# archibate/ptina

Measured on AMD Instinct MI355X. Metric: Msamples/sec (pixels x spp / s), 512x512x32spp cornell-monkey (978 tri), higher is better.
Workload: dtype f32; 1 GPU; s978: 978-tri synthetic cornell + bumpy sphere, 512x512, 32 spp, unidirectional MIS path tracer, depth<=5; step = 32 x render() + get_image() (resolve + D2H), exams/benchmark.py:29-36; spp=32, mode=fast, parallelism=single GPU

## Files before the change

### ptina_amd/csrc/miptina.cpp

```cpp

#include "miptina_ctx.h"
#include <chrono>

static int g_hwq = 0;
static bool g_hwq_late = false;
__attribute__((constructor)) static void mpt_want_hw_queues() {
    if (!getenv("GPU_MAX_HW_QUEUES")) {
        setenv("GPU_MAX_HW_QUEUES", "12", 0);
        const char *pre = getenv("LD_PRELOAD");
        if ((pre && strstr(pre, "rocprof")) || getenv("ROCP_TOOL_LIBRARIES")) {
            g_hwq_late = true;
            fprintf(stderr, "libmiptina: GPU_MAX_HW_QUEUES=12 requested after a preloaded profiler tool may have initialised HIP: "
                            "streams may fold onto the default 4 hardware queues (results unchanged; export the variable "
                            "before starting the profiler)\n");
        }
    }
    const char *v = getenv("GPU_MAX_HW_QUEUES");
    g_hwq = v ? atoi(v) : 0;
}

static thread_local std::string g_err;

int fail(const char *fmt, ...) {
    char buf[1024];
    va_list ap;
    va_start(ap, fmt);
    vsnprintf(buf, sizeof buf, fmt, ap);
    va_end(ap);
    g_err = buf;
    return 1;
}


extern "C" const char *mpt_last_error(void) { return g_err.c_str(); }
extern "C" int mpt_version(void) { return 100; }

extern "C" int mpt_device_count(void) {
    int n = 0;
    if (hipGetDeviceCount(&n) != hipSuccess) return 0;
    return n;
}

int use_ro(mpt_ctx *c) {
    if (!c) return fail("null context");
    HIP_TRY(hipSetDevice(c->device));
    return 0;
}

int use(mpt_ctx *c) {
    if (use_ro(c)) return 1;
    if (mpt_flush(c)) return 1;
    c->main_dirty = true;
    c->spec_valid = false;
    return 0;
}


static void default_light(mpt_ctx *c) {
    MptLight L{};
    L.color_size = { 32.f, 32.f, 32.f, 0.5f };
    L.pos_type = { 1.f, 2.f, 3.f, 0.f };
    int t = MPT_LIGHT_POINT;
    memcpy(&L.pos_type.w, &t, 4);
    c->h_lights.assign(1, L);
}

static int upload_lights(mpt_ctx *c) {
    if (!c->h_lights.empty())
        HIP_TRY(hipMemcpyAsync(c->lights, c->h_lights.data(), c->h_lights.size() * sizeof(MptLight),
                               hipMemcpyHostToDevice, c->stream));
    HIP_TRY(hipStreamSynchronize(c->stream));
    return 0;
}

static int make_render_streams(mpt_ctx *c) {
    for (int k = 0; k < MPT_MAX_PIPE; k++)
        if (!c->rstream[k]) HIP_TRY(hipStreamCreateWithFlags(&c->rstream[k], hipStreamNonBlocking));
    return 0;
}

extern "C" mpt_ctx *mpt_create(const mpt_caps *caps, int device) {
    int ndev = 0;
    hipError_t e = hipGetDeviceCount(&ndev);
    if (e != hipSuccess || ndev == 0) {
        fail("no HIP device available (%s): the MI355X path has no CPU fallback",
             e == hipSuccess ? "device count 0" : hipGetErrorString(e));
        return nullptr;
    }
    if (device < 0 || device >= ndev) { fail("device %d out of range (%d devices)", device, ndev); return nullptr; }
    mpt_ctx *c = new mpt_ctx();
    c->device = device;
    mpt_caps d = { 1 << 21, 1 << 22, 1 << 6, 1 << 6, 1 << 6, 1 << 21, 3 };
    c->caps = caps ? *caps : d;
    if (c->caps.max_lights > MPT_MAX_LIGHTS) c->caps.max_lights = MPT_MAX_LIGHTS;
    if (c->caps.max_filmpasses < 3) c->caps.max_filmpasses = 3;
    auto bail = [&](const char *what) -> mpt_ctx * {
        std::string m = g_err;
        fail("mpt_create: %s: %s", what, m.c_str());
        delete c;
        return nullptr;
    };
    if (hipSetDevice(device) != hipSuccess) return bail("hipSetDevice");
    if (hipStreamCreateWithFlags(&c->stream, hipStreamNonBlocking) != hipSuccess) return bail("stream");
    if (dev_alloc(&c->mats, (size_t)c->caps.max_materials + 1)) return bail("materials");
    if (dev_alloc(&c->images, c->caps.max_textures)) return bail("images");
    if (dev_alloc(&c->lights, MPT_MAX_LIGHTS)) return bail("lights");
    if (dev_alloc(&c->d_counters, MPT_COUNTER_WORDS)) return bail("counters");
    if (dev_alloc(&c->d_scratch, 2)) return bail("scratch");
    if (dev_alloc(&c->d_work, MPT_QUEUE_WORDS)) return bail("work counters");
    for (int k = 0; k < MPT_MAX_PIPE; k++) {
        if (hipEventCreateWithFlags(&c->ev_sobol2[k], hipEventDisableTiming) != hipSuccess) return bail("event");
        if (hipEventCreateWithFlags(&c->ev_render[k], hipEventDisableTiming) != hipSuccess) return bail("event");
        if (hipEventCreateWithFlags(&c->ev_free[k], hipEventDisableTiming) != hipSuccess) return bail("event");
        if (dev_alloc(&c->d_work2[k], MPT_QUEUE_WORDS)) return bail("work counters");
        hipMemsetAsync(c->d_work2[k], 0, MPT_QUEUE_WORDS * sizeof(unsigned int), c->stream);
    }
    if (hipStreamCreateWithFlags(&c->aux, hipStreamNonBlocking) != hipSuccess) return bail("aux stream");
    if (hipEventCreateWithFlags(&c->ev_main, hipEventDisableTiming) != hipSuccess) return bail("event");
    if (hipEventCreateWithFlags(&c->ev_film, hipEventDisableTiming) != hipSuccess) return bail("event");
    {
        hipDeviceProp_t prop;
        if (hipGetDeviceProperties(&prop, device) == hipSuccess) {
            if (prop.multiProcessorCount > 0) c->num_cus = prop.multiProcessorCount;
            c->clock_khz = prop.clockRate;
        }
    }
    if (make_render_streams(c)) return bail("render streams");
    {
        void *dp = nullptr;
        if (hipHostMalloc((void **)&c->h_watchdog, sizeof(unsigned int), hipHostMallocMapped) != hipSuccess ||
            hipHostGetDevicePointer(&dp, c->h_watchdog, 0) != hipSuccess) return bail("pinned watchdog flag");
        *c->h_watchdog = 0;
        c->d_watchdog = (unsigned int *)dp;
        void *dm = nullptr;
        if (hipHostMalloc((void **)&c->h_sahmeta, 32 * sizeof(int), hipHostMallocMapped) != hipSuccess ||
            hipHostGetDevicePointer(&dm, c->h_sahmeta, 0) != hipSuccess) return bail("pinned build mailbox");
        c->d_sahmeta = (int *)dm;
        memset(c->h_sahmeta, 0, 32 * sizeof(int));
    }
    hipMemsetAsync(c->d_counters, 0, MPT_COUNTER_WORDS * sizeof(unsigned long long), c->stream);
    hipMemsetAsync(c->d_work, 0, MPT_QUEUE_WORDS * sizeof(unsigned int), c->stream);
    {
        std::vector<MptMaterial> z((size_t)c->caps.max_materials + 1);
        for (auto &m : z) { memset(&m, 0, sizeof m); for (int k = 0; k < 12; k++) m.tex[k] = -1; }
        const float dflt[14] = { 0.8f, 0.8f, 0.8f, 0.0f, 0.4f, 0.5f, 0.4f, 0.0f, 0.0f, 0.4f, 0.0f, 0.5f, 0.0f, 1.45f };
        memcpy(z.back().p, dflt, sizeof dflt);
        hipMemcpyAsync(c->mats, z.data(), z.size() * sizeof(MptMaterial), hipMemcpyHostToDevice, c->stream);
        mpt_launch_derive_materials(c->mats, (int)z.size(), c->stream);
        hipStreamSynchronize(c->stream);
    }
    for (int i = 0; i < 16; i++) c->v2w[i] = c->w2v[i] = (i % 5 == 0) ? 1.f : 0.f;
    default_light(c);
    if (upload_lights(c)) return bail("lights upload");
    return c;
}

extern "C" void mpt_destroy(mpt_ctx *c) {
    if (!c) return;
    hipSetDevice(c->device);
    for (int k = 0; k < MPT_MAX_PIPE; k++) if (c->rstream[k]) hipStreamSynchronize(c->rstream[k]);
    if (c->aux) { hipStreamSynchronize(c->aux); }
    hipStreamSynchronize(c->stream);
    mpt_comm_release(c);
    if (c->aux) hipStreamDestroy(c->aux);
    if (c->probe_stream) hipStreamDestroy(c->probe_stream);
    if (c->stress_stream) { hipStreamSynchronize(c->stress_stream); hipStreamDestroy(c->stress_stream); }
    hipFree(c->stress_buf);
    for (int k = 0; k < MPT_MAX_PIPE; k++) {
        if (c->rstream[k]) hipStreamDestroy(c->rstream[k]);
        if (c->ev_render[k]) hipEventDestroy(c->ev_render[k]);
        if (c->ev_free[k]) hipEventDestroy(c->ev_free[k]);
        if (c->ev_sobol2[k]) hipEventDestroy(c->ev_sobol2[k]);
        hipFree(c->partial2[k]); hipFree(c->sP2[k]); hipFree(c->d_work2[k]);
    }
    if (c->ev_main) hipEventDestroy(c->ev_main);
    if (c->ev_film) hipEventDestroy(c->ev_film);
    for (auto &pr : c->events) { hipEventDestroy(pr.first); hipEventDestroy(pr.second); }
    for (auto &ev : c->event_pool) hipEventDestroy(ev);
    for (auto &ev : c->mlt_events) hipEventDestroy(ev);
    for (auto &ev : c->brute_events) hipEventDestroy(ev);
    hipFree(c->mlt_X); hipFree(c->mlt_L); hipFree(c->mlt_bit); hipFree(c->mlt_keys); hipFree(c->mlt_keys2);
    hipFree(c->mlt_vals); hipFree(c->mlt_vals2); hipFree(c->mlt_tmp); hipFree(c->mlt_runs);
    for (int p = 0; p < 3; p++) hipFree(c->film[p]);
    hipFree(c->resolved); hipFree(c->exported);
    hipFree(c->snode); hipFree(c->fnode); hipFree(c->tgeo); hipFree(c->tshade); hipFree(c->wnode); hipFree(c->qnode); hipFree(c->tfast);
    for (int k = 0; k < MPT_MAX_PIPE; k++) hipFree(c->stack_spill2[k]);
    hipFree(c->mats); hipFree(c->images); hipFree(c->texels); hipFree(c->lights);
    hipFree(c->sV); hipFree(c->sX); hipFree(c->sX_spec); hipFree(c->sP);
    hipFree(c->gather_buf); hipFree(c->d_pieces); hipFree(c->sah_ws);
    hipFree(c->wb_bin_of); hipFree(c->wb_ncount); hipFree(c->wb_offset); hipFree(c->wb_scan); hipFree(c->wb_area);
    hipFree(c->d_counters); hipFree(c->d_scratch); hipFree(c->d_work); hipFree(c->d_timeline);
    if (c->h_watchdog) hipHostFree(c->h_watchdog);
    if (c->h_sahmeta) hipHostFree(c->h_sahmeta);
    if (c->h_stage) hipHostFree(c->h_stage);
    hipFree(c->d_verts); hipFree(c->d_mtlids); hipFree(c->d_cen); hipFree(c->d_bounds); hipFree(c->d_depth);
    hipFree(c->d_keys_in); hipFree(c->d_keys_out); hipFree(c->d_sort_tmp);
    hipFree(c->d_child); hipFree(c->d_parent); hipFree(c->d_leaf); hipFree(c->d_mc);
    hipFree(c->d_bmin); hipFree(c->d_bmax); hipFree(c->d_arrive);
    hipStreamDestroy(c->stream);
    delete c;
}

static std::mutex g_host_mu;
static std::map<uintptr_t, size_t> g_host_bufs;

extern "C" void *mpt_host_alloc(size_t bytes) {
    void *p = nullptr;
    if (hipHostMalloc(&p, std::max<size_t>(bytes, 1), hipHostMallocDefault) != hipSuccess) {
        fail("hipHostMalloc(%zu) failed", bytes);
        return nullptr;
    }
    std::lock_guard<std::mutex> lk(g_host_mu);
    g_host_bufs[(uintptr_t)p] = bytes;
    return p;
}

extern "C" void mpt_host_free(void *p) {
    if (!p) return;
    {
        std::lock_guard<std::mutex> lk(g_host_mu);
        g_host_bufs.erase((uintptr_t)p);
    }
    hipHostFree(p);
}

static bool is_locked_range(const void *p, size_t bytes) {
    std::lock_guard<std::mutex> lk(g_host_mu);
    auto it = g_host_bufs.upper_bound((uintptr_t)p);
    if (it == g_host_bufs.begin()) return false;
    --it;
    return (uintptr_t)p + bytes <= it->first + it->second;
}

static int read_back(mpt_ctx *c, void *out, const void *dev, size_t bytes) {
    if (is_locked_range(out, bytes)) {
        HIP_TRY(hipMemcpyAsync(out, dev, bytes, hipMemcpyDeviceToHost, c->stream));
        HIP_TRY(hipStreamSynchronize(c->stream));
        return 0;
    }
    if (bytes > c->h_stage_bytes) {
        if (c->h_stage) hipHostFree(c->h_stage);
        c->h_stage = nullptr; c->h_stage_bytes = 0;
        HIP_TRY(hipHostMalloc(&c->h_stage, bytes, hipHostMallocDefault));
        c->h_stage_bytes = bytes;
    }
    HIP_TRY(hipMemcpyAsync(c->h_stage, dev, bytes, hipMemcpyDeviceToHost, c->stream));
    HIP_TRY(hipStreamSynchronize(c->stream));
    memcpy(out, c->h_stage, bytes);
    return 0;
}

extern "C" int mpt_set_option(mpt_ctx *c, const char *key, int value) {
    if (use(c)) return 1;
    std::string k = key ? key : "";
    if (k == "mode") {
        if (value != MPT_MODE_FAST && value != MPT_MODE_STRICT) return fail("mode must be 0 (fast) or 1 (strict)");
        c->mode = value;
    } else if (k == "batch") {
        if (value < 1 || value > MPT_MAX_BATCH) return fail("batch must be in 1..%d", MPT_MAX_BATCH);
        c->batch = value;
    } else if (k == "chunk") {
        if (value < 0) return fail("chunk must be >= 0");
        c->chunk = value;
    } else if (k == "count") {
        c->count = value ? 1 : 0;
    } else if (k == "lds") {
        c->use_lds = value ? 1 : 0;
    } else if (k == "lds_wide") {
        if (value != 0 && value != 1) return fail("lds_wide must be 0 or 1");
        c->lds_wide = value;
    } else if (k == "zero_copy") {
        c->zero_copy = value ? 1 : 0;
    } else if (k == "skip_dark") {
        if (value < -1 || value > 1) return fail("skip_dark must be -1 (auto), 0 or 1");
        c->skip_dark = value;
    } else if (k == "spin_us") {
        if (value < 0) return fail("spin_us must be >= 0");
        c->spin_us = value;
    } else if (k == "finalise") {
        if (value < 0 || value > 2) return fail("finalise must be 0 (combine pass), 1 (tail finalisation) or 2 (the same without the early image: A/B)");
        c->finalise = value;
    } else if (k == "launch_seq") {
        if (value < 0) return fail("launch_seq must be >= 0");
        if (mpt_flush(c)) return 1;
        c->launch_seq = (unsigned)value;
        c->tag_epoch = 0xffffffffu;
    } else if (k == "timeline") {
        c->timeline = value ? 1 : 0;
    } else if (k == "pipe_depth") {
        if (value != 0 && (value < 2 || value > MPT_MAX_PIPE)) return fail("pipe_depth must be 0 (auto) or 2..%d", MPT_MAX_PIPE);
        c->pipe_depth = value;
    } else if (k == "grid_div") {
        if (value < 0 || value > 8) return fail("grid_div must be 0 (auto) or 1..8");
        c->grid_div = value;
    } else if (k == "lds_block") {
        if (value != 0 && value != 256 && value != 512 && value != 768 && value != 1024)
            return fail("lds_block must be 0 (auto), 256, 512, 768 or 1024");
        c->lds_block = value;
    } else if (k == "reserve_cus") {
        if (value < 0 || value >= c->num_cus) return fail("reserve_cus must be in 0..%d", c->num_cus - 1);
        c->reserve_cus = value;
    } else if (k == "wide") {
        c->use_wide = value ? 1 : 0;
    } else if (k == "sah_exact_max") {
        if (value < 2) return fail("sah_exact_max must be >= 2");
        c->sah_exact_max = value; c->tree_valid = false;
    } else if (k == "sah_build") {
        if (value < -1 || value > 1) return fail("sah_build must be -1 (auto), 0 (host) or 1 (device)");
        if (value != c->sah_build) { c->sah_build = value; c->tree_valid = false; }
    } else if (k == "wide_build") {
        if ((value ? 1 : 0) != c->wide_build) { c->wide_build = value ? 1 : 0; c->tree_valid = false; }
    } else if (k == "wide_quant") {
        c->use_quant = value ? 1 : 0;
    } else if (k == "tree") {
        if (value != 0 && value != 1) return fail("tree must be 0 (LBVH) or 1 (SAH)");
        if (value != c->tree_kind) { c->tree_kind = value; c->tree_valid = false; }
    } else if (k == "tile_w_shift" || k == "tile_h_shift") {
        if (value < 0 || value > 3) return fail("%s must be in 0..3", k.c_str());
        (k == "tile_w_shift" ? c->tile_w_shift : c->tile_h_shift) = value;
    } else if (k == "gpu_build") {
        if ((value ? 1 : 0) != c->gpu_build) { c->gpu_build = value ? 1 : 0; c->tree_valid = false; }
    } else if (k == "sah_inject_fail") {
        c->sah_inject_fail = value != 0; c->tree_valid = false;
    } else if (k == "build_phases") {
        c->build_phases = value ? 1 : 0;
    } else if (k == "lane_hist") {
        c->lane_hist = value ? 1 : 0;
    } else if (k == "sah_max") {
        c->sah_max = value; c->tree_valid = false;
    } else {
        return fail("unknown option '%s'", k.c_str());
    }
    return 0;
}

extern "C" int mpt_get_option(mpt_ctx *c, const char *key, int *value) {
    if (!c || !value) return fail("null argument");
    std::string k = key ? key : "";
    if (k == "mode") *value = c->mode;
    else if (k == "batch") *value = c->batch;
    else if (k == "chunk") *value = c->chunk;
    else if (k == "count") *value = c->count;
    else if (k == "tree_depth") *value = c->tree_depth;
    else if (k == "fast_depth") *value = c->fast_depth;
    else if (k == "tree") *value = c->tree_kind;
    else if (k == "gpu_build") *value = c->gpu_build;
    else if (k == "pending") *value = c->pending;
    else if (k == "lds") *value = c->use_lds;
    else if (k == "lds_wide") *value = c->lds_wide;
    else if (k == "lds_block") *value = c->lds_block;
    else if (k == "zero_copy") *value = c->zero_copy;
    else if (k == "spin_us") *value = c->spin_us;
    else if (k == "finalise") *value = c->finalise;
    else if (k == "last_finalised") *value = c->last_finalised;
    else if (k == "launch_seq") *value = (int)(c->launch_seq & 0x7fffffffu);
    else if (k == "tag_wraps") *value = (int)c->tag_wraps;
    else if (k == "skip_dark") *value = c->skip_dark;
    else if (k == "pipe_depth") *value = c->pipe_depth;
    else if (k == "grid_div") *value = c->grid_div;
    else if (k == "cur_depth") *value = c->cur_depth;
    else if (k == "cur_div") *value = c->cur_div;
    else if (k == "last_div") *value = c->last_div;
    else if (k == "last_kernel") *value = c->last_kernel;
    else if (k == "num_cus") *value = c->num_cus;
    else if (k == "reserve_cus") *value = c->reserve_cus;
    else if (k == "wide") *value = c->use_wide;
    else if (k == "wide_quant") *value = c->use_quant;
    else if (k == "wide_build") *value = c->wide_build;
    else if (k == "sah_build") *value = c->sah_build;
    else if (k == "sah_fallback") *value = c->sah_fallback;
    else if (k == "build_phases") *value = c->build_phases;
    else if (k == "lane_hist") *value = c->lane_hist;
    else if (k == "sah_levels") *value = c->sah_stats.levels;
    else if (k == "sah_kelems") *value = (int)(c->sah_stats.elems / 1000);
    else if (k == "sah_chunks") *value = (int)c->sah_stats.chunks;
    else if (k == "sah_segments") *value = (int)c->sah_stats.segments;
    else if (k == "sah_part_kwords") *value = (int)(c->sah_stats.part_words / 1000);
    else if (k == "sah_tasks_small") *value = c->sah_stats.tasks_small;
    else if (k == "sah_tasks_big") *value = c->sah_stats.tasks_big;
    else if (k == "sah_t_sort_k") *value = c->sah_stats.t_sort_k;
    else if (k == "sah_t_loop_k") *value = c->sah_stats.t_loop_k;
    else if (k == "sah_t_max_k") *value = c->sah_stats.t_max_k;
    else if (k == "sah_task_levels") *value = c->sah_stats.task_levels;
    else if (k == "sah_task_levels_max") *value = c->sah_stats.task_levels_max;
    else if (k.rfind("build_phase_us_", 0) == 0 && k.size() == 16 && k[15] >= '0' && k[15] <= '5') *value = (int)(c->build_phase_us[k[15] - '0'] + 0.5);
    else if (k == "wide_nodes") *value = c->wide_nodes;
    else if (k == "wide_stack") *value = c->wide_stack;
    else if (k == "wide_ratio_permille") *value = (int)(c->wide_ratio * 1000.f + 0.5f);
    else if (k == "wide_depth") *value = c->wide_depth;
    else if (k == "nranks") *value = c->nranks;
    else if (k == "rank") *value = c->rank;
    else if (k == "device") *value = c->device;
    else if (k == "clock_khz") *value = c->clock_khz;
    else if (k == "hw_queues") *value = g_hwq_late ? -g_hwq : g_hwq;
    else return fail("unknown option '%s'", k.c_str());
    return 0;
}

extern "C" int mpt_set_size(mpt_ctx *c, int nx, int ny) {
    if (use(c)) return 1;
    if (nx <= 0 || ny <= 0) return fail("film size must be positive, got %dx%d", nx, ny);
    size_t npix = (size_t)nx * ny;
    if (npix > (size_t)c->caps.max_filmsize)
        return fail("film %dx%d exceeds max_filmsize=%d (init_things(max_filmsize=...))", nx, ny, c->caps.max_filmsize);
    if (npix > c->film_cap) {
        HIP_TRY(hipStreamSynchronize(c->stream));
        for (int p = 0; p < 3; p++) { hipFree(c->film[p]); c->film[p] = nullptr; }
        hipFree(c->resolved); c->resolved = nullptr;
        hipFree(c->exported); c->exported = nullptr;
        for (int p = 0; p < 3; p++) {
            if (dev_alloc(&c->film[p], npix)) return 1;
            HIP_TRY(hipMemsetAsync(c->film[p], 0, npix * sizeof(MptVec4), c->stream));
        }
        if (dev_alloc(&c->resolved, npix)) return 1;
        if (dev_alloc(&c->exported, npix * 3)) return 1;
        c->film_cap = npix;
    }
    c->nx = nx; c->ny = ny; c->x0 = 0; c->x1 = nx; c->stripe_w = 0; c->stripe_idx = 0; c->stripe_mod = 1;
    c->film_version++;
    return 0;
}

extern "C" int mpt_get_size(mpt_ctx *c, int *nx, int *ny) {
    if (!c) return fail("null context");
    if (nx) *nx = c->nx;
    if (ny) *ny = c->ny;
    return 0;
}

extern "C" int mpt_set_slab(mpt_ctx *c, int x0, int x1) {
    if (use(c)) return 1;
    if (x0 < 0 || x1 > c->nx || x0 > x1) return fail("slab [%d,%d) outside film width %d", x0, x1, c->nx);
    c->x0 = x0; c->x1 = x1;
    c->stripe_w = 0; c->stripe_idx = 0; c->stripe_mod = 1;
    return 0;
}

extern "C" int mpt_set_stripes(mpt_ctx *c, int width, int index, int modulo) {
    if (use(c)) return 1;
    if (c->nx <= 0) return fail("film size not set: call set_size() first");
    if (width <= 0 || width % MPT_TILE != 0) return fail("stripe width must be a positive multiple of %d", MPT_TILE);
    if (modulo < 1 || index < 0 || index >= modulo) return fail("stripe index %d outside [0, %d)", index, modulo);
    if ((long long)width * modulo > (1 << 30)) return fail("stripe pitch too large");
    c->stripe_w = width; c->stripe_idx = index; c->stripe_mod = modulo;
    c->x0 = std::min((long long)index * width, (long long)c->nx); c->x1 = c->nx;
    return 0;
}

static void share_extent(const mpt_ctx *c, int tile, long long *cols, int *tile_cols) {
    long long n = 0; int t = 0;
    if (c->stripe_w == 0) {
        n = c->x1 - c->x0; t = (c->x1 - c->x0 + tile - 1) / tile;
    } else {
        for (long long x = (long long)c->stripe_idx * c->stripe_w; x < c->nx; x += (long long)c->stripe_w * c->stripe_mod) {
            int w = (int)std::min<long long>(c->stripe_w, c->nx - x);
            n += w; t += (w + tile - 1) / tile;
        }
    }
    if (cols) *cols = n;
    if (tile_cols) *tile_cols = t;
}

extern "C" int mpt_load_model(mpt_ctx *c, const float *verts, const int32_t *mtlids, int n) {
    if (use(c)) return 1;
    if (n < 0 || (n > 0 && !verts)) return fail("bad model arguments");
    if (n >= c->caps.max_faces) return fail("too many faces");
    c->nfaces = n;
    c->verts.assign(verts, verts + (size_t)n * 24);
    if (mtlids) c->mtlids.assign(mtlids, mtlids + n);
    else c->mtlids.assign(n, -1);
    c->max_mtlid = -1;
    for (int i = 0; i < n; i++) {
        if (c->mtlids[i] < -1 || c->mtlids[i] >= c->caps.max_materials)
            return fail("material id %d of face %d outside [-1, %d)", c->mtlids[i], i, c->caps.max_materials);
        c->max_mtlid = std::max(c->max_mtlid, (int)c->mtlids[i]);
    }
    {
        double lo[3] = { 1e300, 1e300, 1e300 }, hi[3] = { -1e300, -1e300, -1e300 };
        for (size_t v = 0; v < (size_t)n * 3; v++)
            for (int k = 0; k < 3; k++) {
                const double x = c->verts[v * 8 + k];
                if (x < lo[k]) lo[k] = x;
                if (x > hi[k]) hi[k] = x;
            }
        double r2 = 0;
        for (int k = 0; k < 3; k++) { c->scene_cen[k] = n ? 0.5 * (lo[k] + hi[k]) : 0.0; r2 += n ? 0.25 * (hi[k] - lo[k]) * (hi[k] - lo[k]) : 0.0; }
        c->scene_rad = std::sqrt(r2);
        if (!std::isfinite(c->scene_rad)) c->scene_rad = 1e30;
    }
    c->tree_valid = false;
    c->d_model_stale = true;
    return 0;
}

extern "C" int mpt_load_materials(mpt_ctx *c, const float *fac, const int32_t *tex, int m) {
    if (use(c)) return 1;
    if (m < 0 || m > c->caps.max_materials) return fail("%d materials exceed max_materials=%d", m, c->caps.max_materials);
    std::vector<MptMaterial> h(std::max(m, 1));
    int max_tex = -1;
    for (int i = 0; i < m; i++) {
        MptMaterial &M = h[i];
        memset(&M, 0, sizeof M);
        const float *f = fac + (size_t)i * 48;
        M.p[0] = f[0]; M.p[1] = f[1]; M.p[2] = f[2];
        for (int k = 1; k < 12; k++) M.p[2 + k] = f[k * 4];
        M.any_tex = 0;
        for (int k = 0; k < 12; k++) {
            int t = tex ? tex[(size_t)i * 12 + k] : -1;
            if (t < -1 || t >= c->caps.max_textures) return fail("texture id %d outside [-1, %d)", t, c->caps.max_textures);
            M.tex[k] = t;
            if (t != -1) M.any_tex = 1;
            max_tex = std::max(max_tex, t);
        }
    }
    c->max_mat_tex = max_tex;
    c->nmats = m;
    if (m) HIP_TRY(hipMemcpyAsync(c->mats, h.data(), (size_t)m * sizeof(MptMaterial), hipMemcpyHostToDevice, c->stream));
    HIP_TRY(mpt_launch_derive_materials(c->mats, m, c->stream));
    HIP_TRY(hipStreamSynchronize(c->stream));
    return 0;
}

extern "C" int mpt_reset_images(mpt_ctx *c) {
    if (use(c)) return 1;
    c->h_images.clear();
    c->texels_used = 0;
    return 0;
}

extern "C" int mpt_load_image(mpt_ctx *c, const float *rgba, int nx, int ny, int *id) {
    if (use(c)) return 1;
    if ((int)c->h_images.size() >= c->caps.max_textures) return fail("Out of ID!");
    size_t need = (size_t)nx * ny;
    if (c->texels_used + need > (size_t)c->caps.max_texels) return fail("Out of memory!");
    if (!c->texels) { if (dev_alloc(&c->texels, (size_t)c->caps.max_texels)) return 1; }
    HIP_TRY(hipMemcpyAsync(c->texels + c->texels_used, rgba, need * sizeof(MptVec4), hipMemcpyHostToDevice, c->stream));
    MptImage im = { nx, ny, (int32_t)c->texels_used, 0 };
    c->h_images.push_back(im);
    c->texels_used += need;
    HIP_TRY(hipMemcpyAsync(c->images, c->h_images.data(), c->h_images.size() * sizeof(MptImage),
                           hipMemcpyHostToDevice, c->stream));
    HIP_TRY(hipStreamSynchronize(c->stream));
    if (id) *id = (int)c->h_images.size() - 1;
    return 0;
}

extern "C" int mpt_set_camera(mpt_ctx *c, const float v2w[16], const float w2v[16]) {
    if (use(c)) return 1;
    memcpy(c->v2w, v2w, sizeof c->v2w);
    if (w2v) memcpy(c->w2v, w2v, sizeof c->w2v);
    return 0;
}

extern "C" int mpt_clear_lights(mpt_ctx *c) {
    if (use(c)) return 1;
    c->h_lights.clear();
    return 0;
}

extern "C" int mpt_add_light(mpt_ctx *c, int type, const float color[3], const float pos[3], const float axes[9],
                             float size, int *index) {
    if (use(c)) return 1;
    if (type != MPT_LIGHT_POINT && type != MPT_LIGHT_AREA) return fail("unknown light type %d", type);
    if ((int)c->h_lights.size() >= c->caps.max_lights) return fail("too many lights (max_lights=%d)", c->caps.max_lights);
    MptLight L{};
    L.color_size = { color[0], color[1], color[2], size };
    L.pos_type = { pos[0], pos[1], pos[2], 0.f };
    memcpy(&L.pos_type.w, &type, 4);
    L.ax0 = { axes[0], axes[1], axes[2], 0.f };
    L.ax1 = { axes[3], axes[4], axes[5], 0.f };
    L.ax2 = { axes[6], axes[7], axes[8], 0.f };
    c->h_lights.push_back(L);
    if (index) *index = (int)c->h_lights.size() - 1;
    return upload_lights(c);
}

extern "C" int mpt_set_world_light(mpt_ctx *c, const float fac[4], int tex) {
    if (use(c)) return 1;
    memcpy(c->world_fac, fac, sizeof c->world_fac);
    c->world_tex = tex;
    return 0;
}

extern "C" int mpt_sobol_init(mpt_ctx *c, const int32_t *V, int rows, int dim) {
    if (use(c)) return 1;
    if (rows < 2 || dim < 1 || !V) return fail("bad sobol grid %dx%d", rows, dim);
    HIP_TRY(hipStreamSynchronize(c->stream));
    hipFree(c->sV); hipFree(c->sX); hipFree(c->sX_spec); hipFree(c->sP);
    c->sV = c->sX = c->sX_spec = nullptr; c->sP = nullptr;
    HIP_TRY(hipStreamSynchronize(c->aux));
    for (int k = 0; k < MPT_MAX_PIPE; k++) { HIP_TRY(hipStreamSynchronize(c->rstream[k])); hipFree(c->sP2[k]); c->sP2[k] = nullptr; }
    if (dev_alloc(&c->sV, (size_t)rows * dim) || dev_alloc(&c->sX, (size_t)dim) || dev_alloc(&c->sX_spec, (size_t)dim) ||
        dev_alloc(&c->sP, (size_t)MPT_MAX_BATCH * dim)) return 1;
    for (int k = 0; k < MPT_MAX_PIPE; k++)
        if (dev_alloc(&c->sP2[k], (size_t)MPT_MAX_BATCH * dim)) return 1;
    HIP_TRY(hipMemcpyAsync(c->sV, V, (size_t)rows * dim * sizeof(int32_t), hipMemcpyHostToDevice, c->stream));
    HIP_TRY(hipMemsetAsync(c->sX, 0, (size_t)dim * sizeof(int), c->stream));
    HIP_TRY(hipStreamSynchronize(c->stream));
    c->sdim = dim; c->srows = rows; c->stime = 0;
    return 0;
}

static int sobol_advance(mpt_ctx *c, int count, int keep, hipStream_t stream = nullptr, float *P = nullptr) {
    if (!stream) stream = c->stream;
    if (!P) P = c->sP;
    while (count > 0) {
        int step = count;
        int k = std::min(keep, step);
        HIP_TRY(mpt_launch_sobol_update(c->sX, c->sX, c->sV, P, c->sdim, c->srows, c->stime, step, k, 1, stream));
        c->stime = (int32_t)((uint32_t)c->stime + (uint32_t)step);
        count -= step;
    }
    return 0;
}

extern "C" int mpt_sobol_reset(mpt_ctx *c, int skip) {
    if (use(c)) return 1;
    if (!c->sV) return fail("sobol sampler not initialised");
    c->stime = 0;
    HIP_TRY(hipMemsetAsync(c->sX, 0, (size_t)c->sdim * sizeof(int), c->stream));
    return sobol_advance(c, skip, 0);
}

extern "C" int mpt_sobol_update(mpt_ctx *c, int count) {
    if (use(c)) return 1;
    if (!c->sV) return fail("sobol sampler not initialised");
    return sobol_advance(c, count, 0);
}

extern "C" int mpt_sobol_get(mpt_ctx *c, int32_t *X, float *P, int32_t *time) {
    if (use(c)) return 1;
    if (!c->sV) return fail("sobol sampler not initialised");
    std::vector<int32_t> x(c->sdim);
    HIP_TRY(hipMemcpyAsync(x.data(), c->sX, (size_t)c->sdim * sizeof(int32_t), hipMemcpyDeviceToHost, c->stream));
    HIP_TRY(hipStreamSynchronize(c->stream));
    if (X) memcpy(X, x.data(), (size_t)c->sdim * sizeof(int32_t));
    if (P)
        for (int j = 0; j < c->sdim; j++) {
            float ret = 0.f, term = 0.5f;
            for (uint32_t v = (uint32_t)x[j]; v; v <<= 1, term *= 0.5f)
                if (v & 0x80000000u) ret += term;
            P[j] = ret;
        }
    if (time) *time = c->stime;
    return 0;
}

static int fill_scene_params(mpt_ctx *c, MptRenderParams &p) {
    p.nlights = (int)c->h_lights.size(); p.world_tex = c->world_tex;
    memcpy(p.world_fac, c->world_fac, sizeof p.world_fac);
    memcpy(p.v2w, c->v2w, sizeof p.v2w);
    p.default_mtl = c->caps.max_materials;
    p.mats = c->mats; p.lights = c->lights; p.images = c->images; p.texels = c->texels;
    if (p.world_tex != -1 && (p.world_tex < 0 || p.world_tex >= (int)c->h_images.size()))
        return fail("world light texture %d is not a loaded image", p.world_tex);
    return 0;
}

static int fill_params(mpt_ctx *c, MptRenderParams &p, int nframes) {
    if (c->nx <= 0) return fail("film size not set: call set_size() first");
    if (!c->sV) return fail("sobol sampler not initialised");
    if (!c->tree_valid) return fail("BVH not built: call build_tree() after load_model()");
    if ((long long)nframes * c->sdim >= (1ll << 30) || nframes >= (1 << 24) || c->sdim >= (1 << 24))
        return fail("%d frames of %d Sobol dimensions in one launch exceed the kernels' 32-bit row offsets", nframes, c->sdim);
    if (c->nfaces >= (1 << 26)) return fail("%d faces exceed the kernels' 32-bit record offsets", c->nfaces);
    memset(&p, 0, sizeof p);
    p.nx = c->nx; p.ny = c->ny; p.x0 = c->x0; p.x1 = c->x1;
    p.nframes = nframes; p.n = c->nfaces;
// ... 73 lines not shown
        if (c->main_dirty) {
            HIP_TRY(hipEventRecord(c->ev_main, c->stream));
            c->main_dirty = false;
        }
        HIP_TRY(hipStreamWaitEvent(ss, c->ev_main, 0));
        HIP_TRY(hipStreamWaitEvent(ss, c->ev_render[k], 0));
        HIP_TRY(hipStreamWaitEvent(rs, c->ev_main, 0));
        p.P = c->sP2[k];
    }
    const bool use_spec = fast && p.ntiles != 0 && c->spec_valid && c->spec_slot == k && c->spec_B == B &&
                          c->spec_time == c->stime;
    c->spec_valid = false;
    if (p.ntiles == 0) {
        if (sobol_advance(c, B, 0, ss, fast ? c->sP2[k] : nullptr)) return 1;
        if (fast) { HIP_TRY(hipEventRecord(c->ev_sobol2[k], ss)); HIP_TRY(hipStreamWaitEvent(c->stream, c->ev_sobol2[k], 0)); }
        return 0;
    }
    if (use_spec) {
        std::swap(c->sX, c->sX_spec);
        c->stime = (int32_t)((uint32_t)c->stime + (uint32_t)B);
    } else if (sobol_advance(c, B, B, ss, fast ? c->sP2[k] : nullptr)) return 1;

    const int stack = ((c->mode == MPT_MODE_STRICT ? c->tree_depth : c->fast_depth) + 2 <= 32) ? 32 : 64;
    const int lds_stack = c->fast_depth + 1;
    const size_t lds_bytes = ((((size_t)(c->nfaces - 1) * MPT_LDS_NODE_STRIDE + 15) >> 4) + (size_t)c->nfaces * 3 + (size_t)(c->caps.max_materials + 1) * 6) * sizeof(MptVec4) +
                             (((size_t)c->nfaces + 15) & ~(size_t)15) + (size_t)lds_stack * 1024 * sizeof(short);
    const int lds4_nmats = c->max_mtlid + 1;
    const size_t lds4_bytes = ((size_t)c->wide_nodes * (MPT_LDS4_NODE_STRIDE / 16) + ((size_t)c->nfaces + 1) * 3 + (size_t)(lds4_nmats + 1) * 6) * sizeof(MptVec4) +
                              (((size_t)c->nfaces + 15) & ~(size_t)15) + (size_t)c->wide_stack * 1024 * sizeof(short);
    const bool lds4_kernel = fast && c->use_lds && c->lds_wide && c->use_wide && c->wide_nodes > 0 && c->wide_stack > 0 && c->wnode &&
                             c->nfaces >= 2 && c->nfaces < 4095 && lds4_nmats < 255 && lds4_bytes <= 160 * 1024 &&
                             (size_t)c->wide_nodes * MPT_LDS4_NODE_STRIDE < 65536;
    const bool lds_kernel = lds4_kernel ||
                            (fast && c->use_lds && c->nfaces >= 2 && c->nfaces < 32768 && c->caps.max_materials < 256 &&
                             lds_bytes <= 160 * 1024 &&
                             (size_t)(c->nfaces - 1) * (MPT_LDS_NODE_STRIDE / 8) < 32768);
    p.lds_nmats = lds4_nmats;
    int chunk = B, nchunks = 1;
    const int tw = 1 << c->tile_w_shift, th = 1 << c->tile_h_shift;
    int tile_cols = 0;
    share_extent(c, tw, nullptr, &tile_cols);
    const int tiles8 = tile_cols * ((c->ny + th - 1) / th);
    if (fast) {
        chunk = c->chunk;
        if (chunk <= 0) {
            chunk = 1;
        }
        chunk = std::min(chunk, B);
        nchunks = (B + chunk - 1) / chunk;
    }
    p.chunk = chunk; p.nchunks = nchunks;
    p.nitems = tiles8 * nchunks;
    p.tile_w_shift = c->tile_w_shift; p.tile_h_shift = c->tile_h_shift;
    if (fast) {
        const int ccols = tile_cols * tw;
        p.partial_stride = ccols * c->ny;
        size_t need = (size_t)B * (size_t)ccols * c->ny;
        bool zeroed = false;
        for (int q = 0; q < c->cur_depth; q++)
            if (need > c->partial2_cap[q]) {
                HIP_TRY(hipDeviceSynchronize());
                hipFree(c->partial2[q]); c->partial2[q] = nullptr; c->partial2_cap[q] = 0;
                if (dev_alloc(&c->partial2[q], need)) return 1;
                c->partial2_cap[q] = need;
                HIP_TRY(hipMemsetAsync(c->partial2[q], 0, need * sizeof(MptVec4), c->stream));
                zeroed = true;
            }
        if (zeroed) HIP_TRY(hipStreamSynchronize(c->stream));
        p.partial = c->partial2[k];
        p.work_counter = c->d_work2[k];
        if (!use_spec) {
            HIP_TRY(hipMemsetAsync(c->d_work2[k], 0, MPT_QUEUE_WORDS * sizeof(unsigned int), ss));
            HIP_TRY(hipEventRecord(c->ev_sobol2[k], ss));
        }
        HIP_TRY(hipStreamWaitEvent(rs, c->ev_sobol2[k], 0));
        HIP_TRY(hipStreamWaitEvent(rs, c->ev_free[k], 0));
    }
    const int reserve = std::max(c->reserve_cus, 0);
    const int usable_cus = std::max(c->num_cus - reserve, 1);
    int launch_div = std::max(c->cur_div, 1);
    bool ring_idle = fast;
    if (fast && ((launch_div > 1 && c->grid_div <= 0) || c->finalise)) {
        for (int q = 0; q < c->cur_depth && ring_idle; q++) {
            hipError_t st = hipEventQuery(c->ev_render[q]);
            if (st == hipErrorNotReady) ring_idle = false;
            else if (st != hipSuccess) HIP_TRY(st);
        }
    }
    if (fast && launch_div > 1 && c->grid_div <= 0 && ring_idle) launch_div = 1;
    c->last_div = launch_div;
    const int launch_cus = std::max(usable_cus / launch_div, 1);
    const bool wide_pays = c->use_wide != 0;
    const bool wide_kernel = fast && !lds_kernel && wide_pays && c->wide_nodes > 0;
    int wide_blocks = 0;
    if (wide_kernel) {
        HIP_TRY(mpt_wide_blocks(launch_cus, c->count, c->use_quant, &wide_blocks));
        const size_t need_spill = (size_t)wide_blocks * MPT_BLOCK * 128;
        for (int q = 0; q < c->cur_depth; q++)
            if (need_spill > c->stack_spill2_cap[q]) {
                HIP_TRY(hipDeviceSynchronize());
                hipFree(c->stack_spill2[q]); c->stack_spill2[q] = nullptr; c->stack_spill2_cap[q] = 0;
                if (dev_alloc(&c->stack_spill2[q], need_spill)) return 1;
                c->stack_spill2_cap[q] = need_spill;
            }
        p.stack_spill = c->stack_spill2[k];
    }
    int lds_block_used = c->lds_block ? c->lds_block : 1024;
    if (lds_kernel && !lds4_kernel && c->lds_block == 0 &&
        ((long long)p.nitems * chunk << (c->tile_w_shift + c->tile_h_shift)) < 6ll * launch_cus * 1024) lds_block_used = 768;
    p.timeline = nullptr;
    if (c->timeline && lds_kernel) {
        const int block = lds_block_used;
        const int waves = launch_cus * (block / 64);
        if (waves != c->timeline_waves) {
            HIP_TRY(hipDeviceSynchronize());
            hipFree(c->d_timeline); c->d_timeline = nullptr;
            if (dev_alloc(&c->d_timeline, (size_t)waves * MPT_TIMELINE_WORDS)) return 1;
            HIP_TRY(hipMemsetAsync(c->d_timeline, 0, (size_t)waves * MPT_TIMELINE_WORDS * sizeof(unsigned long long), c->stream));
            HIP_TRY(hipStreamSynchronize(c->stream));
            c->timeline_waves = waves;
        }
        p.timeline = c->d_timeline;
    }
    const bool fin = fast && c->finalise && ring_idle && p.nitems > 0;
    c->launch_seq++;
    p.fin_counter = nullptr; p.image_out = nullptr; p.slab_tag = MPT_TAG_COMBINE;
    c->film_version++;
    if (fin) {
        const unsigned phase = c->launch_seq % (unsigned)MPT_TAG_PERIOD, epoch = c->launch_seq / (unsigned)MPT_TAG_PERIOD;
        if (epoch != c->tag_epoch) {
            c->tag_epoch = epoch;
            HIP_TRY(hipStreamSynchronize(c->stream));
            for (int q = 0; q < MPT_MAX_PIPE; q++)
                if (c->partial2[q]) HIP_TRY(hipMemsetAsync(c->partial2[q], 0, c->partial2_cap[q] * sizeof(MptVec4), rs));
            HIP_TRY(hipStreamSynchronize(rs));
            c->tag_wraps++;
        }
        p.fin_counter = c->d_work2[k] + 8 * MPT_QUEUE_STRIDE;
        p.slab_tag = (unsigned)MPT_TAG_FIRST + phase;
        const hipError_t main_busy = hipStreamQuery(c->stream);
        if (main_busy == hipErrorNotReady) {
            HIP_TRY(hipEventRecord(c->ev_film, c->stream));
            HIP_TRY(hipStreamWaitEvent(rs, c->ev_film, 0));
        } else if (main_busy != hipSuccess) HIP_TRY(main_busy);
        const size_t img_bytes = (size_t)c->nx * c->ny * sizeof(MptVec4);
        void *mapped = nullptr;
        if (c->hint_image && c->finalise == 1 && c->zero_copy && c->x0 == 0 && c->x1 == c->nx && c->stripe_w == 0 && is_locked_range(c->hint_image, img_bytes) &&
            hipHostGetDevicePointer(&mapped, c->hint_image, 0) == hipSuccess && mapped) {
            p.image_out = (MptVec4 *)mapped;
            c->early_ptr = c->hint_image; c->early_version = c->film_version; c->early_stream = rs;
        }
    }
    c->last_finalised = fin ? 1 : 0;
    hipEvent_t e0 = get_event(c), e1 = get_event(c);
    HIP_TRY(hipEventRecord(e0, rs));
    if (!fast) HIP_TRY(mpt_launch_render_strict(&p, p.ntiles, stack, c->count, rs));
    else if (lds4_kernel) HIP_TRY(mpt_launch_render_lds4(&p, launch_cus, lds_block_used, lds4_bytes, c->count, rs));
    else if (lds_kernel) HIP_TRY(mpt_launch_render_lds(&p, launch_cus, lds_block_used, lds_bytes, c->count, rs));
    else if (wide_kernel) HIP_TRY(mpt_launch_render_wide(&p, wide_blocks, c->count, c->use_quant, rs));
    else HIP_TRY(mpt_launch_render_fast(&p, launch_cus, stack, c->count, rs));
    c->last_kernel = lds4_kernel ? 5 : lds_kernel ? 1 : wide_kernel ? 2 : 0;
    HIP_TRY(hipEventRecord(e1, rs));
    c->events.push_back({ e0, e1 });
    if (c->events.size() > 4096) {
        for (size_t q = 0; q < 2048; q++) { c->event_pool.push_back(c->events[q].first); c->event_pool.push_back(c->events[q].second); }
        c->events.erase(c->events.begin(), c->events.begin() + 2048);
    }
    if (fast) {
        HIP_TRY(hipEventRecord(c->ev_render[k], rs));
        HIP_TRY(hipStreamWaitEvent(c->stream, c->ev_render[k], 0));
        if (!fin)
            HIP_TRY(mpt_launch_combine(c->film[0], c->partial2[k], c->ny, c->x0, c->x1, p.stripe_w, p.stripe_pitch,
                                       p.partial_stride / std::max(c->ny, 1), B, c->stream));
        HIP_TRY(hipEventRecord(c->ev_free[k], c->stream));
        const int k2 = c->flip % c->cur_depth;
        if (k2 != k) {
            HIP_TRY(hipStreamWaitEvent(ss, c->ev_render[k2], 0));
            HIP_TRY(mpt_launch_sobol_update(c->sX, c->sX_spec, c->sV, c->sP2[k2], c->sdim, c->srows, c->stime, B, B, 1, ss));
            HIP_TRY(hipMemsetAsync(c->d_work2[k2], 0, MPT_QUEUE_WORDS * sizeof(unsigned int), ss));
            HIP_TRY(hipEventRecord(c->ev_sobol2[k2], ss));
            c->spec_valid = true; c->spec_slot = k2; c->spec_B = B; c->spec_time = c->stime;
        }
    }
    return 0;
}

extern "C" int mpt_render(mpt_ctx *c, int nframes) {
    if (!c) return fail("null context");
    if (nframes < 0) return fail("nframes must be >= 0");
    if (c->nx <= 0) return fail("film size not set: call set_size() first");
    if (!c->sV) return fail("sobol sampler not initialised");
    if (!c->tree_valid) return fail("BVH not built: call build_tree() after load_model()");
    if (c->mlt_pending && mlt_flush(c)) return 1;
    while (nframes > 0) {
        int room = c->batch - c->pending;
        int take = std::min(room, nframes);
        c->pending += take;
        nframes -= take;
        if (c->pending >= c->batch && mpt_flush(c)) return 1;
    }
    return 0;
}

extern "C" int mpt_render_preview(mpt_ctx *c, int nframes) {
    if (use(c)) return 1;
    while (nframes > 0) {
        int B = std::min(nframes, MPT_MAX_BATCH);
        MptRenderParams p;
        if (fill_params(c, p, B)) return 1;
        if (sobol_advance(c, B, B)) return 1;
        p.chunk = B; p.nchunks = 1;
        const int stack = ((c->mode == MPT_MODE_STRICT ? c->tree_depth : c->fast_depth) + 2 <= 32) ? 32 : 64;
        if (p.ntiles) {
            if (c->mode == MPT_MODE_STRICT) HIP_TRY(mpt_launch_preview_strict(&p, p.ntiles, stack, c->stream));
            else HIP_TRY(mpt_launch_preview_fast(&p, p.ntiles, stack, c->stream));
        }
        nframes -= B;
    }
    return 0;
}

enum { MPT_MLT_SLAB_RECORDS = 1 << 24 };

static int mlt_check(mpt_ctx *c) {
    if (c->mlt_n <= 0) return fail("Metropolis engine not reset: call mpt_mlt_reset first");
    return 0;
}

static int mlt_stack(const mpt_ctx *c) {
    return ((c->mode == MPT_MODE_STRICT ? c->tree_depth : c->fast_depth) + 2 <= 32) ? 32 : 64;
}

static int mlt_flush(mpt_ctx *c) {
    int n = c->mlt_pending;
    c->mlt_pending = 0;
    if (n <= 0) return 0;
    HIP_TRY(hipSetDevice(c->device));
    MptRenderParams p;
    if (fill_params(c, p, 1)) return 1;
    const int nch = c->mlt_n;
    const int kmax = std::max(1, (int)(MPT_MLT_SLAB_RECORDS / nch));
    const int K0 = std::min(n, kmax);
    const size_t recs = (size_t)K0 * nch, npix = (size_t)c->nx * c->ny;
    if (recs > c->mlt_cap || npix > c->mlt_runs_cap) {
        HIP_TRY(hipStreamSynchronize(c->stream));
        const size_t cap = std::max(recs, c->mlt_cap), rcap = std::max(npix, c->mlt_runs_cap);
        size_t tmp = 0;
        HIP_TRY(mpt_mlt_sort_bytes((int)cap, (int)rcap, &tmp));
        hipFree(c->mlt_keys); hipFree(c->mlt_keys2); hipFree(c->mlt_vals); hipFree(c->mlt_vals2); hipFree(c->mlt_tmp); hipFree(c->mlt_runs);
        c->mlt_keys = c->mlt_keys2 = nullptr; c->mlt_vals = c->mlt_vals2 = nullptr; c->mlt_tmp = nullptr; c->mlt_runs = nullptr;
        c->mlt_cap = c->mlt_runs_cap = 0;
        HIP_TRY(hipMalloc(&c->mlt_keys, cap * sizeof(uint32_t)));
        HIP_TRY(hipMalloc(&c->mlt_keys2, cap * sizeof(uint32_t)));
        HIP_TRY(hipMalloc(&c->mlt_vals, cap * sizeof(MptVec4)));
        HIP_TRY(hipMalloc(&c->mlt_vals2, cap * sizeof(MptVec4)));
        HIP_TRY(hipMalloc(&c->mlt_tmp, std::max(tmp, (size_t)16)));
        HIP_TRY(hipMalloc(&c->mlt_runs, rcap * 2 * sizeof(uint32_t)));
        c->mlt_cap = cap; c->mlt_runs_cap = rcap; c->mlt_tmp_bytes = std::max(tmp, (size_t)16);
    }
    const int stack = mlt_stack(c);
    while (n > 0) {
        const int K = std::min(n, kmax);
        MptMltArgs a;
        a.X = c->mlt_X; a.L = c->mlt_L; a.bit = c->mlt_bit; a.keys = c->mlt_keys; a.vals = c->mlt_vals;
        a.nchains = nch; a.t0 = c->mlt_iter; a.K = K; a.seed = c->mlt_seed; a.lsp = c->mlt_lsp; a.sigma = c->mlt_sigma;
        hipEvent_t e0 = get_event(c), e1 = get_event(c), e2 = get_event(c);
        HIP_TRY(hipEventRecord(e0, c->stream));
        if (c->mode == MPT_MODE_STRICT) HIP_TRY(mpt_launch_mlt_chain_strict(&p, &a, stack, c->stream));
        else HIP_TRY(mpt_launch_mlt_chain_fast(&p, &a, stack, c->stream));
        HIP_TRY(hipEventRecord(e1, c->stream));
        HIP_TRY(mpt_launch_mlt_splat(c->film[0], c->mlt_keys, c->mlt_vals, c->mlt_keys2, c->mlt_vals2, c->mlt_tmp, c->mlt_tmp_bytes,
                                     c->mlt_runs, K * nch, (int)npix, c->stream));
        HIP_TRY(hipEventRecord(e2, c->stream));
        c->mlt_events.push_back(e0); c->mlt_events.push_back(e1); c->mlt_events.push_back(e2);
        if (c->mlt_events.size() > 3 * 4096) {
            for (size_t q = 0; q < 3 * 2048; q++) c->event_pool.push_back(c->mlt_events[q]);
            c->mlt_events.erase(c->mlt_events.begin(), c->mlt_events.begin() + 3 * 2048);
        }
        c->mlt_iter += K;
        n -= K;
    }
    c->film_version++;
    c->main_dirty = true;
    return 0;
}

extern "C" int mpt_mlt_reset(mpt_ctx *c, int nchains, uint32_t seed) {
    if (use(c)) return 1;
    if (nchains <= 0 || nchains > (1 << 24)) return fail("nchains %d outside [1, 2^24]", nchains);
    if (nchains != c->mlt_n) {
        HIP_TRY(hipStreamSynchronize(c->stream));
        hipFree(c->mlt_X); hipFree(c->mlt_L); hipFree(c->mlt_bit);
        c->mlt_X = c->mlt_L = nullptr; c->mlt_bit = nullptr; c->mlt_n = 0;
        HIP_TRY(hipMalloc(&c->mlt_X, (size_t)nchains * 2 * 32 * sizeof(float)));
        HIP_TRY(hipMalloc(&c->mlt_L, (size_t)nchains * 3 * sizeof(float)));
        HIP_TRY(hipMalloc(&c->mlt_bit, (size_t)nchains * sizeof(int32_t)));
        c->mlt_n = nchains;
    }
    c->mlt_seed = seed; c->mlt_iter = 0; c->mlt_pending = 0;
    HIP_TRY(mpt_launch_mlt_reset(c->mlt_X, c->mlt_L, c->mlt_bit, nchains, seed, c->stream));
    return 0;
}

extern "C" int mpt_mlt_set_param(mpt_ctx *c, float lsp, float sigma) {
    if (use(c)) return 1;
    c->mlt_lsp = lsp; c->mlt_sigma = sigma;
    return 0;
}

extern "C" int mpt_mlt_render(mpt_ctx *c, int iterations) {
    if (!c) return fail("null context");
    if (iterations < 0) return fail("iterations must be >= 0");
    if (mlt_check(c)) return 1;
// ... 392 lines not shown
```

### ptina_amd/csrc/miptina_ctx.h

```cpp
#pragma once

#include "../../include/miptina.h"
#include "mpt_types.h"
#include <hip/hip_runtime_api.h>
#include <rccl/rccl.h>
#include <dlfcn.h>
#include <algorithm>
#include <cmath>
#include <cstdarg>
#include <cstdio>
#include <chrono>
#include <cstring>
#include <map>
#include <mutex>
#include <string>
#include <vector>

MPT_KERNEL_API hipError_t mpt_launch_render_fast(const MptRenderParams *, int grid, int stack, int count, hipStream_t);
MPT_KERNEL_API hipError_t mpt_launch_render_strict(const MptRenderParams *, int grid, int stack, int count, hipStream_t);
MPT_KERNEL_API hipError_t mpt_launch_derive_materials(MptMaterial *mats, int count, hipStream_t);
MPT_KERNEL_API hipError_t mpt_launch_derive_tfast(const MptVec4 *tgeo, MptVec4 *tfast, int n, hipStream_t);
MPT_KERNEL_API hipError_t mpt_wide_blocks(int grid, int count, int quant, int *blocks);
MPT_KERNEL_API hipError_t mpt_launch_render_wide(const MptRenderParams *, int blocks, int count, int quant, hipStream_t);
MPT_KERNEL_API hipError_t mpt_launch_render_lds(const MptRenderParams *, int grid, int block, size_t lds_bytes, int count, hipStream_t);
MPT_KERNEL_API hipError_t mpt_launch_render_lds4(const MptRenderParams *, int grid, int block, size_t lds_bytes, int count, hipStream_t);
MPT_KERNEL_API hipError_t mpt_launch_mlt_chain_fast(const MptRenderParams *, const MptMltArgs *, int stack, hipStream_t);
MPT_KERNEL_API hipError_t mpt_launch_mlt_chain_strict(const MptRenderParams *, const MptMltArgs *, int stack, hipStream_t);
MPT_KERNEL_API hipError_t mpt_launch_mlt_trace_fast(const MptRenderParams *, const float *X, float *rgb, int n, int stack, hipStream_t);
MPT_KERNEL_API hipError_t mpt_launch_mlt_trace_strict(const MptRenderParams *, const float *X, float *rgb, int n, int stack, hipStream_t);
MPT_KERNEL_API hipError_t mpt_launch_mlt_reset(float *X, float *L, int *bit, int nchains, unsigned seed, hipStream_t);
MPT_KERNEL_API hipError_t mpt_mlt_sort_bytes(int n, int npix, size_t *bytes);
MPT_KERNEL_API hipError_t mpt_launch_mlt_splat(MptVec4 *film, const unsigned *keys, const MptVec4 *vals, unsigned *keys2, MptVec4 *vals2,
                                               void *tmp, size_t tmp_bytes, unsigned *runs, int n, int npix, hipStream_t);
MPT_KERNEL_API hipError_t mpt_launch_brute_fast(const MptRenderParams *, int grid, int stack, hipStream_t);
MPT_KERNEL_API hipError_t mpt_launch_brute_strict(const MptRenderParams *, int grid, int stack, hipStream_t);
MPT_KERNEL_API hipError_t mpt_launch_preview_fast(const MptRenderParams *, int grid, int stack, hipStream_t);
MPT_KERNEL_API hipError_t mpt_launch_preview_strict(const MptRenderParams *, int grid, int stack, hipStream_t);
MPT_KERNEL_API hipError_t mpt_launch_sobol_update(const int *X, int *Xout, const int *V, float *P, int dim, int rows, int time0,
                                              int count, int keep, int write_x, hipStream_t stream);
MPT_KERNEL_API hipError_t mpt_launch_combine(MptVec4 *film, const MptVec4 *partial, int ny, int x0, int x1,
                                         int stripe_w, int stripe_pitch, int ccols, int nframes, hipStream_t);
MPT_KERNEL_API hipError_t mpt_launch_resolve(const MptVec4 *film, MptVec4 *out, size_t npix, hipStream_t);
MPT_KERNEL_API hipError_t mpt_launch_probe(double *out, int threads, size_t lds_bytes, hipStream_t);
MPT_KERNEL_API hipError_t mpt_launch_unit_eval_fast(const MptRenderParams *, int kind, const float *in, int in_cols, float *out, int out_cols, int n, hipStream_t);
MPT_KERNEL_API hipError_t mpt_launch_unit_eval_strict(const MptRenderParams *, int kind, const float *in, int in_cols, float *out, int out_cols, int n, hipStream_t);
MPT_KERNEL_API hipError_t mpt_launch_copy_pieces(const MptVec4 *src, MptVec4 *dst, const MptPiece *tab, int npieces,
                                             long long max_count, hipStream_t);
MPT_KERNEL_API hipError_t mpt_launch_export(const MptVec4 *film, float *out, int nx, int ny, hipStream_t);

struct MptLbvhBuffers {
    const float *verts; const int *mtlids; int n;
    float *cen; int *bounds;
    unsigned long long *keys_in, *keys_out;
    void *sort_tmp; size_t sort_tmp_bytes;
    int *child, *parent, *leaf, *mc;
    float *bmin, *bmax;
    unsigned *arrive;
    int *depth;
    MptVec4 *snode, *fnode, *tgeo, *tshade;
};
MPT_KERNEL_API size_t mpt_sah_seg_capacity(int n);
MPT_KERNEL_API size_t mpt_sah_chunk_capacity(int n);
MPT_KERNEL_API size_t mpt_sah_task_capacity(int n);
MPT_KERNEL_API size_t mpt_sah_part_words(int n);
MPT_KERNEL_API size_t mpt_sah_segbin_words(int n);
MPT_KERNEL_API size_t mpt_sah_level_words(int n, size_t nseg, int *nb_out);
MPT_KERNEL_API int mpt_sah_task_max(void);
MPT_KERNEL_API hipError_t mpt_sah_build(const MptSahBuffers *B, int *depth, hipStream_t stream);
MPT_KERNEL_API hipError_t mpt_wide_scan_bytes(int ni, size_t *bytes);
MPT_KERNEL_API hipError_t mpt_wide_build(const MptVec4 *fnode, int n, MptVec4 *wnode, MptVec4 *qnode, int *bin_of, int *ncount,
                                     int *offset, void *scan_tmp, size_t scan_bytes, double *d_area, int *nwide, int *depth,
                                     double area[2], hipStream_t stream, volatile int *mail_host, int *mail_dev);
MPT_KERNEL_API hipError_t mpt_lbvh_sort_bytes(int n, size_t *bytes);
MPT_KERNEL_API hipError_t mpt_lbvh_build(const MptLbvhBuffers *b, hipStream_t stream);

#define MPT_INTERNAL __attribute__((visibility("hidden")))
MPT_INTERNAL int fail(const char *fmt, ...);

#define HIP_TRY(expr)                                                                     \
    do {                                                                                  \
        hipError_t e_ = (expr);                                                           \
        if (e_ != hipSuccess) return fail("%s failed: %s", #expr, hipGetErrorString(e_)); \
    } while (0)

enum { MPT_MAX_PIPE = 6 };

struct mpt_ctx {
    int device = 0;
    hipStream_t stream = nullptr;
    mpt_caps caps{};

    int mode = MPT_MODE_FAST, batch = 32, chunk = 0, count = 0, use_lds = 1, lds_block = 0, zero_copy = 1;
    int lds_wide = 1;
    int skip_dark = -1;
    int max_mtlid = -1;
    int num_cus = 256;
    int clock_khz = 0;
    int tile_w_shift = 3, tile_h_shift = 3;
    int last_div = 1;
    int last_kernel = 0;

    int nx = 0, ny = 0, x0 = 0, x1 = 0;
    int stripe_w = 0, stripe_idx = 0, stripe_mod = 1;
    MptVec4 *film[3] = { nullptr, nullptr, nullptr };
    size_t film_cap = 0;
    MptVec4 *resolved = nullptr;
    float *exported = nullptr;

    int nfaces = 0;
    std::vector<float> verts;
    double scene_cen[3] = { 0, 0, 0 }, scene_rad = 0;
    std::vector<int32_t> mtlids;
    bool tree_valid = false;
    int tree_depth = 0;
    int fast_depth = 0;
    int tree_kind = 1;
    int gpu_build = 1;
    int sah_max = 1 << 22;
    bool host_tree_valid = false;
    float *d_verts = nullptr; int *d_mtlids = nullptr; size_t d_model_cap = 0;
    float *d_cen = nullptr; int *d_bounds = nullptr; int *d_depth = nullptr;
    unsigned long long *d_keys_in = nullptr, *d_keys_out = nullptr;
    void *d_sort_tmp = nullptr; size_t d_sort_bytes = 0;
    int *d_child = nullptr, *d_parent = nullptr, *d_leaf = nullptr, *d_mc = nullptr;
    float *d_bmin = nullptr, *d_bmax = nullptr;
    unsigned *d_arrive = nullptr;
    size_t d_build_cap = 0;
    std::vector<int32_t> h_child, h_leaf, h_mc;
    std::vector<float> h_bmin, h_bmax;
    MptVec4 *snode = nullptr, *fnode = nullptr, *tgeo = nullptr, *tshade = nullptr;
    MptVec4 *tfast = nullptr; size_t tfast_cap = 0;
    MptVec4 *qnode = nullptr; size_t qnode_cap = 0;
    int use_quant = 1;
    MptVec4 *wnode = nullptr; size_t wnode_cap = 0;
    int wide_nodes = 0, wide_depth = 0;
    int wide_stack = 0;
    float wide_ratio = 1.f;
    int sah_exact_max = 8192;
    int sah_inject_fail = 0;
    int *h_sahmeta = nullptr, *d_sahmeta = nullptr;
    MptSahStats sah_stats{};
    bool d_model_stale = true;
    int lane_hist = 0;
    int build_phases = 0;
    double build_phase_us[6] = { 0, 0, 0, 0, 0, 0 };
    int sah_fallback = 0;
    int sah_build = -1;
    void *sah_ws = nullptr; size_t sah_ws_bytes = 0;
    int wide_build = 1;
    int *wb_bin_of = nullptr, *wb_ncount = nullptr, *wb_offset = nullptr; void *wb_scan = nullptr; size_t wb_scan_bytes = 0;
    double *wb_area = nullptr; size_t wb_cap = 0;
    int use_wide = 1;
    int *stack_spill2[MPT_MAX_PIPE] = {}; size_t stack_spill2_cap[MPT_MAX_PIPE] = {};
    size_t node_cap = 0, tri_cap = 0;

    MptMaterial *mats = nullptr;
    int nmats = 0;
    int max_mat_tex = -1;
    MptImage *images = nullptr;
    std::vector<MptImage> h_images;
    MptVec4 *texels = nullptr;
    size_t texels_used = 0;
    MptLight *lights = nullptr;
    std::vector<MptLight> h_lights;
    float world_fac[4] = { 0.1f, 0.1f, 0.1f, 0.1f };
    int world_tex = -1;
    float v2w[16], w2v[16];

    int sdim = 0, srows = 0;
    int32_t stime = 0;
    int *sV = nullptr, *sX = nullptr;
    int *sX_spec = nullptr;
    float *sP = nullptr;

    int mlt_n = 0, mlt_iter = 0, mlt_pending = 0;
    uint32_t mlt_seed = 0;
    float mlt_lsp = 0.25f, mlt_sigma = 0.01f;
    float *mlt_X = nullptr, *mlt_L = nullptr;
    int32_t *mlt_bit = nullptr;
    size_t mlt_cap = 0, mlt_tmp_bytes = 0, mlt_runs_cap = 0;
    uint32_t *mlt_keys = nullptr, *mlt_keys2 = nullptr;
    MptVec4 *mlt_vals = nullptr, *mlt_vals2 = nullptr;
    void *mlt_tmp = nullptr;
    uint32_t *mlt_runs = nullptr;
    std::vector<hipEvent_t> mlt_events;
    std::vector<hipEvent_t> brute_events;
    int pending = 0;

    hipStream_t rstream[MPT_MAX_PIPE] = {};
    hipEvent_t ev_render[MPT_MAX_PIPE] = {};
    hipEvent_t ev_free[MPT_MAX_PIPE] = {};
    hipStream_t probe_stream = nullptr;
    hipStream_t stress_stream = nullptr;
    char *stress_buf = nullptr;
    size_t stress_bytes = 0;
    hipStream_t aux = nullptr;
    hipEvent_t ev_sobol2[MPT_MAX_PIPE] = {};
    int pipe_depth = 0;
    int reserve_cus = 0;
    int grid_div = 0;
    int cur_depth = 2, cur_div = 1;
    hipEvent_t ev_film = nullptr;
    int finalise = 1;
    int spin_us = 20000;
    unsigned launch_seq = 0;
    unsigned tag_epoch = 0;
    unsigned tag_wraps = 0;
    unsigned long long film_version = 0;
    float *hint_image = nullptr;
    float *early_ptr = nullptr;
    hipStream_t early_stream = nullptr;
    unsigned long long early_version = 0;
    int last_finalised = 0;
    hipEvent_t ev_main = nullptr;
    bool main_dirty = true;
    int flip = 0;
    bool spec_valid = false;
    int spec_slot = -1, spec_B = 0;
    int32_t spec_time = 0;
    MptVec4 *partial2[MPT_MAX_PIPE] = {};
    size_t partial2_cap[MPT_MAX_PIPE] = {};
    float *sP2[MPT_MAX_PIPE] = {};
    unsigned int *d_work2[MPT_MAX_PIPE] = {};

    int timeline = 0;
    unsigned long long *d_timeline = nullptr;
    int timeline_waves = 0;
    unsigned long long *d_counters = nullptr;
    unsigned int *d_work = nullptr;
    unsigned int *h_watchdog = nullptr, *d_watchdog = nullptr;
    void *h_stage = nullptr; size_t h_stage_bytes = 0;
    std::vector<std::pair<hipEvent_t, hipEvent_t>> events;
    std::vector<hipEvent_t> event_pool;

    ncclComm_t comm = nullptr;
    int nranks = 1, rank = 0;
    double *d_scratch = nullptr;
    MptVec4 *gather_buf = nullptr; size_t gather_cap = 0;
    MptPiece *d_pieces = nullptr; size_t pieces_cap = 0;
    int plan_key[6] = { -1, -1, -1, -1, -1, -1 };
    int plan_npieces = 0; long long plan_max_count = 0;
};

MPT_INTERNAL int use_ro(mpt_ctx *c);
MPT_INTERNAL int use(mpt_ctx *c);
MPT_INTERNAL int check_pass(mpt_ctx *c, int pass);
MPT_INTERNAL int check_watchdog(mpt_ctx *c);

template <class T>
static int dev_alloc(T **p, size_t count) {
    HIP_TRY(hipMalloc((void **)p, std::max<size_t>(count, 1) * sizeof(T)));
    return 0;
}

MPT_INTERNAL void mpt_comm_release(mpt_ctx *c);
```

### ptina_amd/csrc/pt_device.h

```cpp
#pragma once

#include <hip/hip_runtime.h>
#include "mpt_types.h"

#ifndef MPT_STRICT
#define MPT_STRICT 0
#endif

#define MPT_EPS 1e-6f
#define MPT_INF 1e6f
#define MPT_PI 3.14159265358979323846f
#define MPT_TAU 6.28318530717958647692f
#define MPT_INV_PI 0.31830988618379067154f

#define DEV __device__ __forceinline__

#if MPT_STRICT
DEV float m_div(float a, float b) { return a / b; }
DEV float m_rcp(float a) { return 1.0f / a; }
DEV float m_sqrt(float a) { return sqrtf(a); }
DEV float m_rnorm(float sumsq) { return 1.0f / sqrtf(sumsq); }
DEV void m_sincos_turn(float p, float *s, float *c) { *c = cosf(p * MPT_TAU); *s = sinf(p * MPT_TAU); }
DEV float m_pow5(float x) { return powf(x, 5.0f); }
DEV float m_pow(float a, float b) { return powf(a, b); }
DEV float m_log(float a) { return logf(a); }
#else
DEV float m_div(float a, float b) { return a * __builtin_amdgcn_rcpf(b); }
DEV float m_rcp(float a) { return __builtin_amdgcn_rcpf(a); }
DEV float m_sqrt(float a) { return __builtin_amdgcn_sqrtf(a); }
DEV float m_rnorm(float sumsq) { return __builtin_amdgcn_rsqf(sumsq); }
DEV void m_sincos_turn(float p, float *s, float *c) { *c = __builtin_amdgcn_cosf(p); *s = __builtin_amdgcn_sinf(p); }
DEV float m_pow5(float x) { float x2 = x * x; return x2 * x2 * x; }
DEV float m_pow(float a, float b) { return __builtin_amdgcn_exp2f(b * __builtin_amdgcn_logf(a)); }
DEV float m_log(float a) { return __builtin_amdgcn_logf(a) * 0.69314718055994530942f; }
#endif

struct V3 { float x, y, z; };
DEV V3 v3(float x, float y, float z) { V3 r; r.x = x; r.y = y; r.z = z; return r; }
DEV V3 v3s(float s) { return v3(s, s, s); }
DEV V3 operator+(V3 a, V3 b) { return v3(a.x + b.x, a.y + b.y, a.z + b.z); }
DEV V3 operator-(V3 a, V3 b) { return v3(a.x - b.x, a.y - b.y, a.z - b.z); }
DEV V3 operator*(V3 a, V3 b) { return v3(a.x * b.x, a.y * b.y, a.z * b.z); }
DEV V3 operator*(V3 a, float s) { return v3(a.x * s, a.y * s, a.z * s); }
DEV V3 operator-(V3 a) { return v3(-a.x, -a.y, -a.z); }
DEV V3 vdivs(V3 a, float s) { return v3(m_div(a.x, s), m_div(a.y, s), m_div(a.z, s)); }
DEV float dot(V3 a, V3 b) { return a.x * b.x + a.y * b.y + a.z * b.z; }
DEV V3 cross(V3 a, V3 b) { return v3(a.y * b.z - a.z * b.y, a.z * b.x - a.x * b.z, a.x * b.y - a.y * b.x); }
DEV float norm_sqr(V3 a) { return a.x * a.x + a.y * a.y + a.z * a.z; }
DEV V3 normalized(V3 a) { return a * m_rnorm(norm_sqr(a)); }
DEV V3 normalized_unfused(V3 a) {
#pragma clang fp contract(off)
    const float xx = a.x * a.x, yy = a.y * a.y, zz = a.z * a.z;
    const float s = xx + yy + zz;
    return a * m_rnorm(s);
}
#if MPT_STRICT
DEV float vavg(V3 a) { return m_div(a.x + a.y + a.z, 3.0f); }
#else
DEV float vavg(V3 a) { return (a.x + a.y + a.z) * 0.33333334f; }
#endif
DEV bool any_gt0(V3 a) { return a.x > 0.0f || a.y > 0.0f || a.z > 0.0f; }
DEV bool any_ne0(V3 a) { return a.x != 0.0f || a.y != 0.0f || a.z != 0.0f; }
DEV float clampf(float x, float lo, float hi) { return fminf(hi, fmaxf(lo, x)); }
DEV float dot_or_zero(V3 a, V3 b) { return fmaxf(0.0f, dot(a, b)); }
DEV float lerpf(float f, float src, float dst) { return src * (1.0f - f) + dst * f; }
DEV V3 lerpv(float f, V3 src, V3 dst) { return src * (1.0f - f) + dst * f; }
DEV V3 reflectv(V3 I, V3 N) { return I - N * (2.0f * dot(N, I)); }

DEV bool refractv(V3 I, V3 N, float eta, V3 *T) {
    bool has_r = false;
    *T = v3s(0.0f);
    float NoI = dot(N, I);
    float discr = 1.0f - eta * eta * (1.0f - NoI * NoI);
    if (discr > 0.0f) {
        has_r = true;
        *T = normalized(I * eta - N * (eta * NoI + m_sqrt(discr)));
    }
    return has_r;
}

DEV V3 spherical(float h, float p) {
    float s, c;
    m_sincos_turn(p, &s, &c);
    float r = m_sqrt(fmaxf(0.0f, 1.0f - h * h));
    return v3(r * c, r * s, h);
}

struct TanSpace { V3 tan, bitan, nrm; };
DEV TanSpace tanspace(V3 nrm) {
    TanSpace t;
    V3 up = v3(233.0f, 666.0f, 512.0f);
    t.bitan = normalized(cross(nrm, up));
    t.tan = cross(t.bitan, nrm);
    t.nrm = nrm;
    return t;
}
DEV V3 tanspace_mul(const TanSpace &t, V3 v) {
    return v3(t.tan.x * v.x + t.bitan.x * v.y + t.nrm.x * v.z,
              t.tan.y * v.x + t.bitan.y * v.y + t.nrm.y * v.z,
              t.tan.z * v.x + t.bitan.z * v.y + t.nrm.z * v.z);
}

DEV int wanghash(int x) {
    unsigned v = (unsigned)x;
    v = (v ^ 61u) ^ (v >> 16);
    v *= 9u;
    v ^= v << 4;
    v *= 0x27d4eb2du;
    v ^= v >> 15;
    return (int)v;
}
DEV int wanghash2(int x, int y) { return wanghash(y ^ wanghash(x)); }

struct Rng { const float *P; int i; int dim; };
DEV float rng_random(Rng &r) {
    int k = r.i % r.dim;
    if (k < 0) k += r.dim;
    float v = r.P[k];
    r.i = (int)((unsigned)r.i + 1u);
    return v;
}
DEV V3 random3(Rng &r) { float a = rng_random(r), b = rng_random(r), c = rng_random(r); return v3(a, b, c); }

struct Cnt { unsigned rays, n_box, n_tri, n_shade, n_draws, bounces, n_node, samples, it_node, it_leaf, it_shade, it_new;
             unsigned pl_local, pl_batches, pl_batch_lanes, pl_prim, pl_tidle, pl_sidle, pl_trips, pl_taken; };

struct Hit { int hit; float depth; int index; float u, v; };

DEV V3 ld3(const MptVec4 &a) { return v3(a.x, a.y, a.z); }

DEV bool tri_test(MptVec4 g0, MptVec4 g1, MptVec4 g2, MptVec4 g3, V3 ro, V3 rd, float *depth, float *s_, float *t_) {
    V3 v0 = ld3(g0), u = ld3(g1), v = ld3(g2), norm = ld3(g3);
    float D = g0.w, uu = g1.w, uv = g2.w, vv = g3.w;
    float b = dot(norm, rd);
#if !MPT_STRICT
    {
        V3 w0 = ro - v0;
        float a = -dot(norm, w0);
        float r = m_div(a, b);
        V3 ip = ro + rd * r;
        V3 w = ip - v0;
        float wu = dot(w, u);
        float wv = dot(w, v);
        float rD = m_rcp(D);
        float s = (uv * wv - vv * wu) * rD;
        float t = (uv * wu - uu * wv) * rD;
        bool ok = fabsf(b) >= MPT_EPS && r > 0.0f && 0.0f <= s && s <= 1.0f && 0.0f <= t && s + t <= 1.0f;
        *depth = r; *s_ = s; *t_ = t;
        return ok;
    }
#else
    bool hit = false;
    if (fabsf(b) >= MPT_EPS) {
        V3 w0 = ro - v0;
        float a = -dot(norm, w0);
        float r = m_div(a, b);
// ... 382 lines not shown
            bool swap = tn1 < tn0;
            st.push(swap ? id0 : id1);
            curr = swap ? id1 : id0;
        } else if (h0) {
            curr = id0;
        } else if (h1) {
            curr = id1;
        } else {
            if (st.sp == 0) break;
            curr = st.pop();
        }
    }
    return ret;
}

template <class SCENE, class STACK>
struct Tracer {
    SCENE sc;
    STACK st;
    int n;
    template <bool COUNT>
    DEV Hit closest(V3 ro, V3 rd, int avoid, Cnt &cnt) const {
        Hit h = bvh_walk<false, COUNT>(sc, n, st, ro, rd, avoid, MPT_INF, cnt);
        if (!h.hit) h.depth = MPT_INF;
        return h;
    }
    template <bool COUNT>
    DEV bool occluded(V3 ro, V3 rd, int avoid, float dis, Cnt &cnt) const {
        return bvh_walk<true, COUNT>(sc, n, st, ro, rd, avoid, dis, cnt).hit != 0;
    }
};
#endif

DEV float sphere_intersect(V3 pos, float rad2, V3 ro, V3 rd) {
    float ret = 0.0f;
    V3 op = pos - ro;
    float b = dot(op, rd);
    float det = b * b + rad2 - norm_sqr(op);
    if (det >= 0.0f) {
        det = m_sqrt(det);
        float t = b - det;
        if (t > MPT_EPS) {
            ret = t;
        } else {
            t = b + det;
            if (t > MPT_EPS) ret = t;
        }
    }
    return ret;
}

DEV bool area_intersect(V3 pos, V3 dirx, V3 diry, V3 ro, V3 rd, float *depth, float *u_ = nullptr, float *v_ = nullptr) {
    bool hit = false;
    V3 nrm = normalized(cross(dirx, diry));
    float NoD = dot(nrm, rd);
    if (NoD > MPT_EPS) {
        float t = m_div(dot(nrm, pos - ro), NoD);
        V3 hitdisp = ro + rd * t - pos;
        float u = m_div(dot(hitdisp, dirx), norm_sqr(dirx));
        float v = m_div(dot(hitdisp, diry), norm_sqr(diry));
        *depth = t;
        if (u_) *u_ = u;
        if (v_) *v_ = v;
        if (-1.0f < u && u < 1.0f && -1.0f < v && v < 1.0f) hit = true;
    }
    return hit;
}

DEV int pymod(int a, int b) { int r = a % b; return r < 0 ? r + b : r; }

DEV MptVec4 image_texel(const MptRenderParams &p, MptImage im, int x, int y) {
    x = pymod(x, im.nx);
    y = pymod(y, im.ny);
    return p.texels[(size_t)im.base + (size_t)x * im.ny + y];
}

DEV MptVec4 image_sample(const MptRenderParams &p, int id, float x, float y) {
    MptImage im = p.images[id];
    float px = x * (float)(im.nx - 1), py = y * (float)(im.ny - 1);
    float fx = floorf(px), fy = floorf(py);
    int Ix = (int)fx, Iy = (int)fy;
    float x0 = px - fx, x1 = py - fy;
    float y0 = 1.0f - x0, y1 = 1.0f - x1;
    MptVec4 t11 = image_texel(p, im, Ix + 1, Iy + 1), t10 = image_texel(p, im, Ix + 1, Iy);
    MptVec4 t00 = image_texel(p, im, Ix, Iy), t01 = image_texel(p, im, Ix, Iy + 1);
    MptVec4 r;
    r.x = t11.x * x0 * x1 + t10.x * x0 * y1 + t00.x * y0 * y1 + t01.x * y0 * x1;
    r.y = t11.y * x0 * x1 + t10.y * x0 * y1 + t00.y * y0 * y1 + t01.y * y0 * x1;
    r.z = t11.z * x0 * x1 + t10.z * x0 * y1 + t00.z * y0 * y1 + t01.z * y0 * x1;
    r.w = t11.w * x0 * x1 + t10.w * x0 * y1 + t00.w * y0 * y1 + t01.w * y0 * x1;
    return r;
}

DEV float schlickFresnel(float cost) { return m_pow5(clampf(1.0f - cost, 0.0f, 1.0f)); }

DEV float dielectricFresnel(float etai, float etao, float cosi) {
    float sini = m_sqrt(fmaxf(0.0f, 1.0f - cosi * cosi));
    float sint = m_div(etao, etai) * sini;
    float ret = 1.0f;
    if (sint < 1.0f) {
        float cost = m_sqrt(fmaxf(0.0f, 1.0f - sint * sint));
        float a1 = etai * cosi, a2 = etao * cost;
        float b1 = etao * cosi, b2 = etai * cost;
        float para = m_div(a1 - a2, a1 + a2);
        float perp = m_div(b1 - b2, b1 + b2);
        ret = 0.5f * (para * para + perp * perp);
    }
    return ret;
}

DEV float GTR1(float cosh_, float alpha) {
    float alpha2 = alpha * alpha;
    float t = 1.0f + (alpha2 - 1.0f) * (cosh_ * cosh_);
    return m_div(alpha2 - 1.0f, MPT_PI * m_log(alpha2) * t);
}
DEV float GTR2(float cosh_, float alpha) {
    float alpha2 = alpha * alpha;
    float t = 1.0f + (alpha2 - 1.0f) * (cosh_ * cosh_);
    return m_div(alpha2, MPT_PI * (t * t));
}
DEV float smithGGX(float cosi, float alpha) {
    float a = alpha * alpha;
    float b = cosi * cosi;
    return m_rcp(cosi + m_sqrt(a + b - a * b));
}
DEV V3 sample_GTR1(float u, float v, float alpha) {
    u = m_div(m_sqrt(m_pow(alpha, 2.0f - 2.0f * u) - 1.0f), alpha * alpha - 1.0f);
    return spherical(u, v);
}
DEV V3 sample_GTR2(float u, float v, float alpha) {
    u = m_sqrt(m_div(1.0f - u, 1.0f - u * (1.0f - alpha * alpha)));
    return spherical(u, v);
}

struct Disney {
    V3 basecolor;
    float metallic, roughness, specular, specularTint, subsurface, sheen, sheenTint, clearcoat,
        clearcoatGloss, transmission, ior;
    V3 speccolor, sheencolor;
    float alpha, clearcoatAlpha;
};

DEV void disney_init(Disney &m) {
    V3 tint = v3s(1.0f);
    float lum = dot(m.basecolor, v3(0.3f, 0.6f, 0.1f));
    if (lum > MPT_EPS) tint = vdivs(m.basecolor, lum);
    m.speccolor = lerpv(m.metallic, lerpv(m.specularTint, v3s(1.0f), tint) * (m.specular * 0.08f), m.basecolor);
    m.sheencolor = lerpv(m.sheenTint, v3s(1.0f), tint);
    m.alpha = fmaxf(0.001f, m.roughness * m.roughness);
    m.clearcoatAlpha = lerpf(m.clearcoatGloss, 0.1f, 0.001f);
}

#if !MPT_STRICT
DEV void material_from(const MptRenderParams &p, const MptMaterial *mt, MptVec4 q0, MptVec4 q1, MptVec4 q2, MptVec4 q3,
                       MptVec4 d0, MptVec4 d1, float tu, float tv, Disney &m) {
    float v[14] = { q0.x, q0.y, q0.z, q0.w, q1.x, q1.y, q1.z, q1.w, q2.x, q2.y, q2.z, q2.w, q3.x, q3.y };
    const bool textured = __float_as_int(q3.z) != 0;
    if (textured) {
#pragma unroll 1
        for (int k = 0; k < 12; k++) {
            int texid = mt->tex[k];
            if (texid != -1) {
                MptVec4 t = image_sample(p, texid, tu, tv);
                if (k == 0) { v[0] *= t.x; v[1] *= t.y; v[2] *= t.z; }
                else {
                    switch (k) {
                    case 1: v[3] *= t.x; break; case 2: v[4] *= t.x; break; case 3: v[5] *= t.x; break;
                    case 4: v[6] *= t.x; break; case 5: v[7] *= t.x; break; case 6: v[8] *= t.x; break;
                    case 7: v[9] *= t.x; break; case 8: v[10] *= t.x; break; case 9: v[11] *= t.x; break;
                    case 10: v[12] *= t.x; break; default: v[13] *= t.x; break;
                    }
                }
            }
        }
    }
    m.basecolor = v3(v[0], v[1], v[2]);
    m.metallic = v[3]; m.roughness = v[4]; m.specular = v[5]; m.specularTint = v[6];
    m.subsurface = v[7]; m.sheen = v[8]; m.sheenTint = v[9]; m.clearcoat = v[10];
    m.clearcoatGloss = v[11]; m.transmission = v[12]; m.ior = v[13];
    if (textured) disney_init(m);
    else {
        m.speccolor = v3(d0.x, d0.y, d0.z); m.sheencolor = v3(d0.w, d1.x, d1.y);
        m.alpha = d1.z; m.clearcoatAlpha = d1.w;
    }
}
DEV void material_get(const MptRenderParams &p, int mtlid, float tu, float tv, Disney &m) {
    const MptMaterial *mt = p.mats + (mtlid == -1 ? p.default_mtl : mtlid);
    const MptVec4 *q = (const MptVec4 *)mt;
    material_from(p, mt, q[0], q[1], q[2], q[3], q[8], q[9], tu, tv, m);
}
#else
DEV void material_get(const MptRenderParams &p, int mtlid, float tu, float tv, Disney &m) {
    if (mtlid == -1) {
        m.basecolor = v3s(0.8f);
        m.metallic = 0.0f; m.roughness = 0.4f; m.specular = 0.5f; m.specularTint = 0.4f;
        m.subsurface = 0.0f; m.sheen = 0.0f; m.sheenTint = 0.4f; m.clearcoat = 0.0f;
        m.clearcoatGloss = 0.5f; m.transmission = 0.0f; m.ior = 1.45f;
    } else {
        const MptVec4 *q = (const MptVec4 *)(p.mats + mtlid);
        MptVec4 q0 = q[0], q1 = q[1], q2 = q[2], q3 = q[3];
        float v[14] = { q0.x, q0.y, q0.z, q0.w, q1.x, q1.y, q1.z, q1.w, q2.x, q2.y, q2.z, q2.w, q3.x, q3.y };
        const MptMaterial *mt = p.mats + mtlid;
        if (mt->any_tex) {
#pragma unroll 1
            for (int k = 0; k < 12; k++) {
                int texid = mt->tex[k];
                if (texid != -1) {
                    MptVec4 t = image_sample(p, texid, tu, tv);
                    if (k == 0) { v[0] *= t.x; v[1] *= t.y; v[2] *= t.z; }
                    else {
                        switch (k) {
                        case 1: v[3] *= t.x; break; case 2: v[4] *= t.x; break; case 3: v[5] *= t.x; break;
                        case 4: v[6] *= t.x; break; case 5: v[7] *= t.x; break; case 6: v[8] *= t.x; break;
                        case 7: v[9] *= t.x; break; case 8: v[10] *= t.x; break; case 9: v[11] *= t.x; break;
                        case 10: v[12] *= t.x; break; default: v[13] *= t.x; break;
                        }
                    }
                }
            }
        }
        m.basecolor = v3(v[0], v[1], v[2]);
        m.metallic = v[3]; m.roughness = v[4]; m.specular = v[5]; m.specularTint = v[6];
        m.subsurface = v[7]; m.sheen = v[8]; m.sheenTint = v[9]; m.clearcoat = v[10];
        m.clearcoatGloss = v[11]; m.transmission = v[12]; m.ior = v[13];
    }
    disney_init(m);
}
#endif

DEV V3 disney_brdf(const Disney &m, V3 normal, float sign, V3 indir, V3 outdir) {
    float etai = 1.0f, etao = m.ior;
    if (sign < 0.0f) { etai = m.ior; etao = 1.0f; }

    V3 halfdir = normalized(indir + outdir);
    float cosi = dot(indir, normal);
    float coso = dot(outdir, normal);
    float cosh_ = dot_or_zero(halfdir, normal);
    float cosoh = dot_or_zero(halfdir, outdir);

    V3 result = v3s(0.0f);
    if (coso < 0.0f) {
        if (cosi >= 0.0f) {
            float Ds = GTR2(cosh_, m.alpha);
            float fdf = dielectricFresnel(etao, etai, cosoh);
            V3 transmit = m.basecolor * MPT_INV_PI * (1.0f - fdf) * Ds;
            result = transmit * (1.0f - m.metallic) * m.transmission;
        }
    } else {
        float Fi = schlickFresnel(cosi);
        float Fo = schlickFresnel(coso);
        float Fd90 = 0.5f + 2.0f * (cosoh * cosoh) * m.roughness;
        float Fd = lerpf(Fi, 1.0f, Fd90) * lerpf(Fo, 1.0f, Fd90);

        float Fss90 = (cosoh * cosoh) * m.roughness;
        float Fss = lerpf(Fi, 1.0f, Fss90) * lerpf(Fo, 1.0f, Fss90);
        float ss = 1.25f * (Fss * (m_rcp(cosi + coso) - 0.5f) + 0.5f);

        float Foh = schlickFresnel(cosoh);
        V3 Fsheen = m.sheencolor * (Foh * m.sheen);

        float Ds = GTR2(cosh_, m.alpha);
        V3 Fs = lerpv(Foh, m.speccolor, v3s(1.0f));
        float Gs = smithGGX(cosi, m.alpha) * smithGGX(coso, m.alpha);
        V3 diffuse = m.basecolor * (MPT_INV_PI * lerpf(m.subsurface, Fd, ss)) + Fsheen;
#if MPT_STRICT
        float fdf = dielectricFresnel(etao, etai, cosoh);
        float Dr = GTR1(cosh_, m.clearcoatAlpha);
        float Gr = smithGGX(cosi, 0.25f) * smithGGX(coso, 0.25f);
        float Fr = lerpf(Foh, 0.04f, 1.0f);
        V3 specular = Fs * Gs * Ds + v3s(0.25f * m.clearcoat * Gr * Fr * Dr);
        V3 transmit = m.basecolor * (MPT_INV_PI * fdf * Ds);
#else
        float coat = 0.0f;
        if (m.clearcoat != 0.0f) {
            float Dr = GTR1(cosh_, m.clearcoatAlpha);
            float Gr = smithGGX(cosi, 0.25f) * smithGGX(coso, 0.25f);
            float Fr = lerpf(Foh, 0.04f, 1.0f);
            coat = 0.25f * m.clearcoat * Gr * Fr * Dr;
        }
        V3 specular = Fs * Gs * Ds + v3s(coat);
        V3 transmit = v3s(0.0f);
        if (m.transmission != 0.0f) transmit = m.basecolor * (MPT_INV_PI * dielectricFresnel(etao, etai, cosoh) * Ds);
#endif

        result = diffuse * (1.0f - m.metallic) * (1.0f - m.transmission);
        result = result + transmit * (1.0f - m.metallic) * m.transmission;
        result = result + specular * (1.0f - m.transmission);
    }
    return result;
}

struct BsdfSample { V3 outdir; float pdf; V3 color; };

struct Choice {
    float pdf, w;
    DEV bool operator()(float r) {
        bool ret;
        if (w < r) {
            w = m_div(w, r);
            pdf *= r;
            ret = true;
        } else {
            w = m_div(w - r, 1.0f - r);
            pdf *= 1.0f - r;
            ret = false;
        }
        return ret;
    }
};

DEV BsdfSample disney_bounce(const Disney &m, V3 normal, float sign, V3 indir, V3 samp) {
    BsdfSample result;
    result.outdir = v3s(0.0f); result.pdf = 0.0f; result.color = v3s(0.0f);

    float etai = 1.0f, etao = m.ior;
    if (sign < 0.0f) { etai = m.ior; etao = 1.0f; }
#if MPT_STRICT
    float eta = m_div(etai, etao);
#endif

    float cosi = dot(indir, normal);
    float Fi = schlickFresnel(cosi);
    V3 Fs = lerpv(Fi, m.speccolor, v3s(1.0f));

    const TanSpace ts = tanspace(normal);
    Choice choice; choice.pdf = 1.0f; choice.w = samp.z;
    float specrate = lerpf(m.transmission, lerpf(m.metallic, vavg(Fs), 1.0f), 1.0f);
    float coatrate = 0.04f * m.clearcoat;

    specrate = lerpf(specrate, 0.1f, 1.0f);
    if (coatrate != 0.0f) coatrate = lerpf(coatrate, 0.1f, 1.0f);

#if MPT_STRICT
    const bool coat = choice(coatrate);
    if (coat) {
        float alpha = m.clearcoatAlpha;
        V3 halfdir = tanspace_mul(ts, sample_GTR1(samp.x, samp.y, alpha));
        V3 outdir = reflectv(-indir, halfdir);

        float coso = dot(outdir, normal);
        float cosh_ = dot_or_zero(halfdir, normal);
        float cosoh = dot_or_zero(halfdir, outdir);
        if (cosoh > 0.0f) {
            float Dr = GTR1(cosh_, alpha);
            float Foh = schlickFresnel(cosoh);
            float Fr = lerpf(Foh, 0.04f, 1.0f);

            result.outdir = outdir;
            float partial = m_div(m.clearcoat * Fr * coso, cosoh);
            result.pdf = Dr * partial;
            result.color = v3s(m_div(partial, choice.pdf));
        }
    } else if (choice(specrate)) {
        float alpha = m.alpha;
        V3 halfdir = tanspace_mul(ts, sample_GTR2(samp.x, samp.y, alpha));
        V3 outdir = reflectv(-indir, halfdir);

        float coso = dot_or_zero(outdir, normal);
        float cosh_ = dot_or_zero(halfdir, normal);
        float cosoh = dot_or_zero(halfdir, outdir);
        if (cosoh > 0.0f && coso > 0.0f && cosh_ > 0.0f) {
            float Ds = GTR2(cosh_, alpha);

            if (choice(m.transmission)) {
                float fdf = dielectricFresnel(etao, etai, cosoh);
                float reflrate = lerpf(fdf, 0.2f, 1.0f);

                if (choice(reflrate)) {
                    result.outdir = outdir;
                    result.pdf = Ds * fdf;
                    result.color = vdivs(m.basecolor * fdf * m.transmission, choice.pdf);
                } else {
                    V3 T;
                    if (refractv(-indir, halfdir, eta, &T)) {
                        result.outdir = T;
                        result.pdf = Ds * (1.0f - fdf);
                        result.color = vdivs(m.basecolor * (1.0f - fdf) * m.transmission, choice.pdf);
                    }
                }
            } else {
                float Foh = schlickFresnel(cosoh);
                V3 Fs2 = lerpv(Foh, m.speccolor, v3s(1.0f));

                result.outdir = outdir;
                float partial = m_div(0.5f, cosoh * smithGGX(coso, alpha));
                result.pdf = Ds * vavg(Fs2) * partial;
                result.color = vdivs(Fs2 * partial * (1.0f - m.transmission), choice.pdf);
            }
        }
    } else {
        V3 outdir = tanspace_mul(ts, spherical(m_sqrt(samp.x), samp.y));

        V3 halfdir = normalized(indir + outdir);
        float cosi2 = cosi;
        float coso = dot(outdir, normal);
        float cosoh = dot_or_zero(halfdir, outdir);

        float Fi2 = Fi;
        float Fo = schlickFresnel(coso);
        float Fd90 = 0.5f + 2.0f * (cosoh * cosoh) * m.roughness;
        float Fd = lerpf(Fi2, 1.0f, Fd90) * lerpf(Fo, 1.0f, Fd90);

        float Fss90 = (cosoh * cosoh) * m.roughness;
        float Fss = lerpf(Fi2, 1.0f, Fss90) * lerpf(Fo, 1.0f, Fss90);
        float ss = 1.25f * (Fss * (m_rcp(cosi2 + coso) - 0.5f) + 0.5f);

        float Foh = schlickFresnel(cosoh);
        V3 Fsheen = m.sheencolor * (Foh * m.sheen);

        V3 diffuse = m.basecolor * (MPT_INV_PI * lerpf(m.subsurface, Fd, ss)) + Fsheen;

        result.outdir = outdir;
        result.pdf = MPT_INV_PI;
        result.color = vdivs(diffuse * MPT_PI * (1.0f - m.metallic) * (1.0f - m.transmission), choice.pdf);
    }
#else
    const bool coat = coatrate != 0.0f && choice(coatrate);
    const bool spec = !coat && choice(specrate);
    float hz;
    if (coat) {
        float a = m.clearcoatAlpha;
        hz = m_div(m_sqrt(m_pow(a, 2.0f - 2.0f * samp.x) - 1.0f), a * a - 1.0f);
    } else if (spec) {
        hz = m_sqrt(m_div(1.0f - samp.x, 1.0f - samp.x * (1.0f - m.alpha * m.alpha)));
    } else {
        hz = m_sqrt(samp.x);
    }
    const V3 sdir = tanspace_mul(ts, spherical(hz, samp.y));
    V3 halfdir, outdir;
    if (coat || spec) { halfdir = sdir; outdir = reflectv(-indir, halfdir); }
    else { outdir = sdir; halfdir = normalized(indir + outdir); }
    const float coso_raw = dot(outdir, normal);
    const float cosh_ = dot_or_zero(halfdir, normal);
    const float cosoh = dot_or_zero(halfdir, outdir);
    const float Foh = schlickFresnel(cosoh);
    if (coat) {
        if (cosoh > 0.0f) {
            float Dr = GTR1(cosh_, m.clearcoatAlpha);
            float Fr = lerpf(Foh, 0.04f, 1.0f);
            result.outdir = outdir;
            float partial = m_div(m.clearcoat * Fr * coso_raw, cosoh);
            result.pdf = Dr * partial;
            result.color = v3s(m_div(partial, choice.pdf));
        }
    } else if (spec) {
        const float coso = fmaxf(0.0f, coso_raw);
        if (cosoh > 0.0f && coso > 0.0f && cosh_ > 0.0f) {
            float Ds = GTR2(cosh_, m.alpha);
            if (choice(m.transmission)) {
                float fdf = dielectricFresnel(etao, etai, cosoh);
                float reflrate = lerpf(fdf, 0.2f, 1.0f);
                if (choice(reflrate)) {
                    result.outdir = outdir;
                    result.pdf = Ds * fdf;
                    result.color = vdivs(m.basecolor * fdf * m.transmission, choice.pdf);
                } else {
                    V3 T;
                    const float eta = m_div(etai, etao);
                    if (refractv(-indir, halfdir, eta, &T)) {
                        result.outdir = T;
                        result.pdf = Ds * (1.0f - fdf);
                        result.color = vdivs(m.basecolor * (1.0f - fdf) * m.transmission, choice.pdf);
                    }
                }
            } else {
                V3 Fs2 = lerpv(Foh, m.speccolor, v3s(1.0f));
                result.outdir = outdir;
                float partial = m_div(0.5f, cosoh * smithGGX(coso, m.alpha));
                result.pdf = Ds * vavg(Fs2) * partial;
                result.color = vdivs(Fs2 * partial * (1.0f - m.transmission), choice.pdf);
            }
        }
    } else {
        const float coso = coso_raw;
        float Fo = schlickFresnel(coso);
        float Fd90 = 0.5f + 2.0f * (cosoh * cosoh) * m.roughness;
        float Fd = lerpf(Fi, 1.0f, Fd90) * lerpf(Fo, 1.0f, Fd90);
        float Fss90 = (cosoh * cosoh) * m.roughness;
        float Fss = lerpf(Fi, 1.0f, Fss90) * lerpf(Fo, 1.0f, Fss90);
        float ss = 1.25f * (Fss * (m_rcp(cosi + coso) - 0.5f) + 0.5f);
        V3 Fsheen = m.sheencolor * (Foh * m.sheen);
        V3 diffuse = m.basecolor * (MPT_INV_PI * lerpf(m.subsurface, Fd, ss)) + Fsheen;
        result.outdir = outdir;
        result.pdf = MPT_INV_PI;
        result.color = vdivs(diffuse * MPT_PI * (1.0f - m.metallic) * (1.0f - m.transmission), choice.pdf);
    }
#endif
    return result;
}

DEV float power_heuristic(float a, float b) {
    a = clampf(a, MPT_EPS, MPT_INF); a = a * a;
    b = clampf(b, MPT_EPS, MPT_INF); b = b * b;
    return m_div(a, a + b);
}

#if !MPT_STRICT && defined(__HIP_DEVICE_COMPILE__)
typedef const __attribute__((address_space(4))) MptLight *LightPtr;
DEV LightPtr lights_const(const MptLight *g) {
    LightPtr q = (LightPtr)(const void *)g;
    asm("" : "+s"(q));
    return q;
}
#define MPT_LIGHTS(p) lights_const((p).lights)
#else
#define MPT_LIGHTS(p) ((p).lights)
#endif
DEV V3 axes_mul(const MptLight &L, V3 v) {
    return v3(L.ax0.x * v.x + L.ax0.y * v.y + L.ax0.z * v.z,
              L.ax1.x * v.x + L.ax1.y * v.y + L.ax1.z * v.z,
              L.ax2.x * v.x + L.ax2.y * v.y + L.ax2.z * v.z);
}

struct LightHit { bool hit; float dis, pdf; V3 color; };

DEV LightHit lights_hit(const MptRenderParams &p, V3 ro, V3 rd) {
    LightHit ret; ret.hit = false; ret.dis = MPT_INF; ret.pdf = 0.0f; ret.color = v3s(0.0f);
    for (int i = 0; i < p.nlights; i++) {
        MptLight L = MPT_LIGHTS(p)[i];
        int type = __float_as_int(L.pos_type.w);
        V3 pos = ld3(L.pos_type);
        float size = L.color_size.w;
        float t = 0.0f, area = 0.0f;
        if (type == 1) {
            t = sphere_intersect(pos, size * size, ro, rd);
            area = MPT_PI * (size * size);
        } else if (type == 2) {
            V3 dirx = axes_mul(L, v3(size, 0.0f, 0.0f));
            V3 diry = axes_mul(L, v3(0.0f, size, 0.0f));
            float d;
            if (area_intersect(pos, dirx, diry, ro, rd, &d)) {
                t = d;
                area = 4.0f * (size * size);
            }
        }
        if (0.0f < t && t < ret.dis) {
            ret.dis = t;
            ret.pdf = m_div(ret.dis * ret.dis, area);
            ret.color = ld3(L.color_size);
            ret.hit = true;
            break;
        }
    }
    return ret;
}

struct LightSample { float dis; V3 dir; float pdf; V3 color; };

DEV LightSample light_sample_one(const MptLight &L, V3 hitpos, V3 samp) {
    LightSample ret;
    int type = __float_as_int(L.pos_type.w);
    V3 color = ld3(L.color_size);
    V3 pos = ld3(L.pos_type);
    float size = L.color_size.w;

    V3 litpos = v3s(MPT_INF);
    V3 norm = v3s(0.0f);
    float area = 0.0f;
    if (type == 1) {
        V3 disp = spherical(samp.x, samp.y);
        litpos = pos + disp * size;
        area = MPT_PI * (size * size);
    } else if (type == 2) {
        V3 disp = axes_mul(L, v3(samp.x * 2.0f - 1.0f, samp.y * 2.0f - 1.0f, 0.0f));
        norm = axes_mul(L, v3(0.0f, 0.0f, 1.0f));
        litpos = pos + disp * size;
        area = 4.0f * (size * size);
    }
    V3 toli = litpos - hitpos;
    float d2 = norm_sqr(toli);
#if MPT_STRICT
    float dis = sqrtf(d2);
    V3 dir = vdivs(toli, dis);
    float pdf = dis * dis / area;
#else
    float rdis = __builtin_amdgcn_rsqf(d2);
    float dis = d2 * rdis;
    V3 dir = toli * rdis;
    float pdf = dis * dis * __builtin_amdgcn_rcpf(area);
#endif
    color = vdivs(color, pdf);
    if (any_ne0(norm)) color = color * dot_or_zero(norm, dir);
    ret.dis = dis; ret.dir = dir; ret.pdf = pdf; ret.color = color;
    return ret;
}

DEV LightSample lights_sample(const MptRenderParams &p, V3 hitpos, V3 samp) {
    LightSample ret; ret.dis = MPT_INF; ret.dir = v3s(0.0f); ret.pdf = 0.0f; ret.color = v3s(0.0f);
#if !MPT_STRICT
    if (p.nlights == 1) {
        const MptLight L = MPT_LIGHTS(p)[0];
        return light_sample_one(L, hitpos, samp);
    }
#endif
    if (p.nlights != 0) {
        int i = (int)floorf(samp.z * (float)p.nlights);
        i = min(max(i, 0), min(p.nlights, MPT_MAX_LIGHTS - 1));
        const MptLight L = MPT_LIGHTS(p)[i];
        ret = light_sample_one(L, hitpos, samp);
    }
    return ret;
}

DEV void dir2tex(V3 dir, float *s, float *t) {
    V3 dn = normalized(dir);
    *s = atan2f(dn.z, dn.x) / MPT_PI * 0.5f + 0.5f;
    *t = atan2f(dn.y, sqrtf(dn.x * dn.x + dn.z * dn.z)) / MPT_PI + 0.5f;
}

DEV V3 world_at(const MptRenderParams &p, V3 dir) {
    V3 fac = v3(p.world_fac[0], p.world_fac[1], p.world_fac[2]);
    if (p.world_tex != -1) {
        V3 d2 = v3(dir.x, dir.z, -dir.y);
        float s, t;
        dir2tex(d2, &s, &t);
        MptVec4 tx = image_sample(p, p.world_tex, s, t);
        fac = fac * v3(tx.x, tx.y, tx.z);
    }
    return fac;
}

DEV void camera_generate(const MptRenderParams &p, float x, float y, V3 *ro, V3 *rd) {
    const float *M = p.v2w;
    float a0 = M[0] * x + M[1] * y + M[2] * -1.0f + M[3] * 1.0f;
    float a1 = M[4] * x + M[5] * y + M[6] * -1.0f + M[7] * 1.0f;
    float a2 = M[8] * x + M[9] * y + M[10] * -1.0f + M[11] * 1.0f;
    float a3 = M[12] * x + M[13] * y + M[14] * -1.0f + M[15] * 1.0f;
    float b0 = M[0] * x + M[1] * y + M[2] * 1.0f + M[3] * 1.0f;
    float b1 = M[4] * x + M[5] * y + M[6] * 1.0f + M[7] * 1.0f;
    float b2 = M[8] * x + M[9] * y + M[10] * 1.0f + M[11] * 1.0f;
    float b3 = M[12] * x + M[13] * y + M[14] * 1.0f + M[15] * 1.0f;
    V3 o = v3(m_div(a0, a3), m_div(a1, a3), m_div(a2, a3));
    V3 o1 = v3(m_div(b0, b3), m_div(b1, b3), m_div(b2, b3));
    *ro = o;
    *rd = normalized(o1 - o);
}

DEV void face_shading(MptVec4 s0, MptVec4 s1, MptVec4 s2, MptVec4 s3, float u, float v, V3 *nrm, float *tu, float *tv) {
    float wx = 1.0f - u - v, wy = u, wz = v;
    V3 vn0 = v3(s0.x, s0.y, s0.z), vn1 = v3(s0.w, s1.x, s1.y), vn2 = v3(s1.z, s1.w, s2.x);
    *nrm = normalized(vn0 * wx + vn1 * wy + vn2 * wz);
    *tu = wx * s2.y + wy * s2.w + wz * s3.y;
    *tv = wx * s2.z + wy * s3.x + wz * s3.z;
}

DEV void get_geometries(const MptRenderParams &p, const Hit &hit, V3 ro, V3 rd, V3 *hitpos, V3 *normal, Disney &mat) {
    const MptVec4 *s = p.tshade + (size_t)hit.index * 4;
    MptVec4 s0 = s[0], s1 = s[1], s2 = s[2], s3 = s[3];
    V3 nrm; float tu, tv;
    face_shading(s0, s1, s2, s3, hit.u, hit.v, &nrm, &tu, &tv);
    *hitpos = ro + rd * hit.depth;
    float sign = -dot(rd, nrm);
    if (sign < 0.0f) nrm = -nrm;
    *normal = nrm;
    material_get(p, __float_as_int(s3.w), tu, tv, mat);
}

#if !MPT_STRICT
struct ShadeRec { MptVec4 s0, s1, s2, s3; };
template <bool OFF32>
DEV ShadeRec shade_rec_load(const MptRenderParams &p, int slot) {
    const MptVec4 *s = OFF32 ? (const MptVec4 *)((const char *)p.tshade + ((unsigned)slot << 6)) : p.tshade + (size_t)slot * 4;
    ShadeRec r; r.s0 = s[0]; r.s1 = s[1]; r.s2 = s[2]; r.s3 = s[3];
    return r;
}
template <class SCENE>
DEV void get_geometries_rec(const MptRenderParams &p, const SCENE &sc, const ShadeRec &r, const Hit &hit, V3 ro, V3 rd,
                            V3 *hitpos, V3 *normal, Disney &mat) {
    const MptVec4 s0 = r.s0, s1 = r.s1, s2 = r.s2, s3 = r.s3;
    V3 nrm; float tu, tv;
    face_shading(s0, s1, s2, s3, hit.u, hit.v, &nrm, &tu, &tv);
    *hitpos = ro + rd * hit.depth;
    float sign = -dot(rd, nrm);
    if (sign < 0.0f) nrm = -nrm;
    *normal = nrm;
    if constexpr (SCENE::LDS_MATS) {
        const int rec = sc.mtl[hit.index];
        LdsVec4Ptr q = sc.mats + rec * MPT_LDS_MAT_VEC4;
        MptVec4 q0 = lds_ld(q), q1 = lds_ld(q + 1), q2 = lds_ld(q + 2), q3 = lds_ld(q + 3), d0 = lds_ld(q + 4), d1 = lds_ld(q + 5);
        material_from(p, p.mats + (rec == sc.mat_last ? sc.mat_default : rec), q0, q1, q2, q3, d0, d1, tu, tv, mat);
    } else {
        material_get(p, __float_as_int(s3.w), tu, tv, mat);
    }
}
#endif
```

### ptina_amd/csrc/render_kernel.hip

```cpp

#include "pt_device.h"
#include "film_ops.h"
#include <atomic>

#if MPT_STRICT
#define MPT_SUFFIX(x) x##_strict
#else
#define MPT_SUFFIX(x) x##_fast
#endif

#include "path_common.h"

template <bool COUNT>
DEV void flush_counters(const MptRenderParams &p, const Cnt &c) {
    if (!COUNT) return;
    unsigned v[20] = { c.samples, c.rays, c.n_box, c.n_tri, c.n_shade, c.n_draws, c.bounces, c.n_node,
                       c.it_node, c.it_leaf, c.it_shade, c.it_new,
                       c.pl_local, c.pl_batches, c.pl_batch_lanes, c.pl_prim, c.pl_tidle, c.pl_sidle, c.pl_trips, c.pl_taken };
#pragma unroll
    for (int k = 0; k < 20; k++) {
        unsigned x = v[k];
#pragma unroll
        for (int off = 32; off > 0; off >>= 1) x += __shfl_xor(x, off);
        if ((threadIdx.x & 63) == 0 && x) atomicAdd(p.counters + k, (unsigned long long)x);
// ... 202 lines not shown
    asm("v_min3_f32 %0, %1, %2, %3" : "=v"(r) : "v"(a), "v"(b), "v"(m));
    return r;
}
DEV float exit_min(float a, float b, float c, float tbest) { return exit_min_asm(a, b, c, tbest); }

template <bool COUNT, class SCENE, class STACK>
DEV void stage_node4(const SCENE &sc, STACK &stk, LaneState &L, Cnt &cnt) {
    int id0, id1, id2, id3;
    float t0, t1, t2, t3;
    bool h0, h1, h2, h3;
    if (COUNT) { cnt.n_node++; cnt.n_box += 4; }
    int spec = 0;
    if constexpr (STACK::SP_ADDR) spec = STACK::ld(L.sp - STACK::SP_STEP + STACK::SP_BIAS);
    if constexpr (SCENE::QUANT) {
        MptVec4 ra, rb, rc, idv;
        sc.node4q(L.curr, ra, rb, rc, idv);
        id0 = __float_as_int(idv.x); id1 = __float_as_int(idv.y); id2 = __float_as_int(idv.z); id3 = __float_as_int(idv.w);
        const float sx = ra.w * L.inv.x, sy = rb.x * L.inv.y, sz = rb.y * L.inv.z;
        const float bx = __builtin_fmaf(ra.x, L.inv.x, -L.oinv.x), by = __builtin_fmaf(ra.y, L.inv.y, -L.oinv.y),
                    bz = __builtin_fmaf(ra.z, L.inv.z, -L.oinv.z);
        const unsigned lox = (unsigned)__float_as_int(rb.z), hix = (unsigned)__float_as_int(rb.w);
        const unsigned loy = (unsigned)__float_as_int(rc.x), hiy = (unsigned)__float_as_int(rc.y);
        const unsigned loz = (unsigned)__float_as_int(rc.z), hiz = (unsigned)__float_as_int(rc.w);
        const bool dnx = __float_as_int(L.inv.x) < 0, dny = __float_as_int(L.inv.y) < 0, dnz = __float_as_int(L.inv.z) < 0;
        const unsigned nxq = dnx ? hix : lox, fxq = dnx ? lox : hix;
        const unsigned nyq = dny ? hiy : loy, fyq = dny ? loy : hiy;
        const unsigned nzq = dnz ? hiz : loz, fzq = dnz ? loz : hiz;
#define MPT_UB(w, c) ((float)(((w) >> (8 * (c))) & 0xffu))
#define MPT_QSLAB(c, tn, h)                                                                                            \
        tn = fmaxf(fmaxf(__builtin_fmaf(MPT_UB(nxq, c), sx, bx), __builtin_fmaf(MPT_UB(nyq, c), sy, by)),               \
                   fmaxf(__builtin_fmaf(MPT_UB(nzq, c), sz, bz), 0.0f));                                                 \
        h = tn <= fminf(fminf(__builtin_fmaf(MPT_UB(fxq, c), sx, bx), __builtin_fmaf(MPT_UB(fyq, c), sy, by)),          \
                        fminf(__builtin_fmaf(MPT_UB(fzq, c), sz, bz), L.tbest));
        MPT_QSLAB(0, t0, h0) MPT_QSLAB(1, t1, h1) MPT_QSLAB(2, t2, h2) MPT_QSLAB(3, t3, h3)
#undef MPT_QSLAB
#undef MPT_UB
    } else {
        MptVec4 nx, fx, ny, fy, nz, fz, idv;
        sc.node4(L.curr, __float_as_int(L.inv.x) < 0 ? 16 : 0, __float_as_int(L.inv.y) < 0 ? 16 : 0, __float_as_int(L.inv.z) < 0 ? 16 : 0,
                 nx, fx, ny, fy, nz, fz, idv);
        id0 = __float_as_int(idv.x); id1 = __float_as_int(idv.y); id2 = __float_as_int(idv.z); id3 = __float_as_int(idv.w);
#define MPT_SLAB(c, tn, h)                                                                                              \
        tn = fmaxf(fmaxf(__builtin_fmaf(nx.c, L.inv.x, -L.oinv.x), __builtin_fmaf(ny.c, L.inv.y, -L.oinv.y)),            \
                   STACK::T_SCALED ? __builtin_amdgcn_fmed3f(__builtin_fmaf(nz.c, L.inv.z, -L.oinv.z), 0.0f, 1.0f)       \
                                   : fmaxf(__builtin_fmaf(nz.c, L.inv.z, -L.oinv.z), 0.0f));                             \
        h = tn <= exit_min(__builtin_fmaf(fx.c, L.inv.x, -L.oinv.x), __builtin_fmaf(fy.c, L.inv.y, -L.oinv.y),          \
                           __builtin_fmaf(fz.c, L.inv.z, -L.oinv.z), L.tbest);
        MPT_SLAB(x, t0, h0) MPT_SLAB(y, t1, h1) MPT_SLAB(z, t2, h2) MPT_SLAB(w, t3, h3)
#undef MPT_SLAB
    }
    const unsigned MISS = 0xffffffffu;
    unsigned k0, k1, k2, k3;
    if constexpr (sizeof(typename STACK::entry_t) == 2) {
        k0 = h0 ? __builtin_amdgcn_perm((unsigned)__float_as_int(t0), (unsigned)id0, 0x07060100u) : MISS;
        k1 = h1 ? __builtin_amdgcn_perm((unsigned)__float_as_int(t1), (unsigned)id1, 0x07060100u) : MISS;
        k2 = h2 ? __builtin_amdgcn_perm((unsigned)__float_as_int(t2), (unsigned)id2, 0x07060100u) : MISS;
        k3 = h3 ? __builtin_amdgcn_perm((unsigned)__float_as_int(t3), (unsigned)id3, 0x07060100u) : MISS;
        const unsigned a0 = min(k0, k1), a1 = max(k0, k1), b0 = min(k2, k3), b1 = max(k2, k3);
        const unsigned m0 = max(a0, b0), m1 = min(a1, b1);
        k0 = min(a0, b0); k3 = max(a1, b1); k1 = min(m0, m1); k2 = max(m0, m1);
        id0 = STACK::ODD_IDS ? (int)(k0 & 0xffffu) : (int)(short)(k0 & 0xffffu);
        id1 = (int)k1; id2 = (int)k2; id3 = (int)k3;
    } else {
        k0 = h0 ? (unsigned)__float_as_int(t0) : MISS;
        k1 = h1 ? (unsigned)__float_as_int(t1) : MISS;
        k2 = h2 ? (unsigned)__float_as_int(t2) : MISS;
        k3 = h3 ? (unsigned)__float_as_int(t3) : MISS;
#define MPT_CSWAP(ka, ia, kb, ib) { bool sw = kb < ka; unsigned tk = sw ? kb : ka; kb = sw ? ka : kb; ka = tk; \
                                    int ti_ = sw ? ib : ia; ib = sw ? ia : ib; ia = ti_; }
        MPT_CSWAP(k0, id0, k1, id1) MPT_CSWAP(k2, id2, k3, id3) MPT_CSWAP(k0, id0, k2, id2) MPT_CSWAP(k1, id1, k3, id3)
        MPT_CSWAP(k1, id1, k2, id2)
#undef MPT_CSWAP
    }
    int next = id0;
    if (STACK::NO_SPILL || __ballot(L.sp > STACK::CAP - 3) == 0ull) {
        typedef typename STACK::entry_t entry_t;
        int sp = L.sp;
        if constexpr (STACK::SP_ADDR) {
            STACK::st(sp + STACK::SP_BIAS, id3); sp += k3 != MISS ? STACK::SP_STEP : 0;
            STACK::st(sp + STACK::SP_BIAS, id2); sp += k2 != MISS ? STACK::SP_STEP : 0;
            STACK::st(sp + STACK::SP_BIAS, id1); sp += k1 != MISS ? STACK::SP_STEP : 0;
            if (k0 == MISS) { sp -= STACK::SP_STEP; next = spec; }
        } else {
            stk.base[sp * STACK::STRIDE] = (entry_t)id3; sp += k3 != MISS ? 1 : 0;
            stk.base[sp * STACK::STRIDE] = (entry_t)id2; sp += k2 != MISS ? 1 : 0;
            stk.base[sp * STACK::STRIDE] = (entry_t)id1; sp += k1 != MISS ? 1 : 0;
            if (k0 == MISS) { sp--; next = (int)stk.base[sp * STACK::STRIDE]; }
        }
        L.sp = sp;
    } else {
        stk.sp = L.sp;
        if (k3 != MISS) stk.push(id3);
        if (k2 != MISS) stk.push(id2);
        if (k1 != MISS) stk.push(id1);
        if (k0 == MISS) next = stk.pop();
        L.sp = stk.sp;
    }
    L.curr = next;
    L.st = classify<STACK>(next);
}

template <bool COUNT, class SCENE, class STACK>
DEV void stage_leaf(const SCENE &sc, STACK &stk, LaneState &L, Cnt &cnt) {
    int slot = SCENE::ODD_IDS ? L.curr : ~L.curr;
    bool stop = false;
    if (COUNT) cnt.n_tri += (SCENE::AVOID_IN_LEAF && L.curr == L.navoid) ? 0u : 1u;
    int spec = 0;
    if constexpr (STACK::SP_ADDR) spec = STACK::ld(L.sp - STACK::SP_STEP + STACK::SP_BIAS);
    else if constexpr (STACK::PEEK) spec = stk.peek(L.sp - 1);
    MptVec4 g0, g1, g2;
    sc.tri(slot, g0, g1, g2);
    float dd, su, sv;
    bool hit = tri_test_fast(g0, g1, g2, L.to, L.td, &dd, &su, &sv);
    if constexpr (STACK::T_SCALED) dd *= stk.ts;
    if constexpr (SCENE::AVOID_IN_LEAF) hit = hit && L.curr != L.navoid;
    if constexpr (STACK::ONE_TEST) {
        if (hit && dd < L.tbest) {
            L.tbest = dd; L.hidx = slot; L.hu = su; L.hv = sv;
            stop = L.shadow != 0;
        }
    } else if (hit) {
        if (L.shadow) {
            if (dd <= L.tbest) { L.hidx = slot; stop = true; }
        } else if (dd < L.tbest) {
            L.tbest = dd; L.hidx = slot; L.hu = su; L.hv = sv;
        }
    }
    int next;
    if constexpr (STACK::PEEK) {
#if MPT_X_LEAFPAIRS
        if (COUNT) { cnt.pl_trips++; if (classify<STACK>(spec) == ST_LEAF && !stop) cnt.pl_local++; }
#endif
        next = spec; L.sp = L.sp - (STACK::SP_ADDR ? STACK::SP_STEP : 1);
    } else {
        stk.sp = L.sp;
        next = stk.pop();
        L.sp = stk.sp;
    }
    L.curr = next;
    L.st = stop ? ST_DONE : classify<STACK>(next);
}

enum { SH_END = 0, SH_BOUNCE = 1, SH_SHADOW = 2 };
#if MPT_X_STAMPS == 2
#define MPT_SEG_BEGIN unsigned long long seg_t = 0; if (COUNT) { __builtin_amdgcn_sched_barrier(0); seg_t = __builtin_amdgcn_s_memtime(); __builtin_amdgcn_sched_barrier(0); }
#define MPT_SEG(field) if (COUNT) { __builtin_amdgcn_sched_barrier(0); const unsigned long long seg_n = __builtin_amdgcn_s_memtime(); \
        const unsigned long long seg_m = __ballot(true); \
        const bool seg_first = __builtin_amdgcn_mbcnt_hi((unsigned)(seg_m >> 32), __builtin_amdgcn_mbcnt_lo((unsigned)seg_m, 0u)) == 0; \
        cnt.field += seg_first ? (unsigned)((seg_n - seg_t) >> 4) : 0u; seg_t = seg_n; __builtin_amdgcn_sched_barrier(0); }
#else
#define MPT_SEG_BEGIN
#define MPT_SEG(field)
#endif
template <bool COUNT, class SCENE>
DEV int shade_core(const MptRenderParams &p, const SCENE &sc, LaneState &L, Cnt &cnt, V3 &hitpos, V3 &sdir, float &sdis) {
    V3 ro = L.to, rd = L.prd;
    const bool was_hit = L.hidx >= 0;
    float hdepth = was_hit ? (SCENE::T_SCALED ? L.tbest * p.t_unscale : L.tbest) : MPT_INF;
    ShadeRec rec;
    float u[6];
    if constexpr (!SCENE::LDS_MATS) { rec = ShadeRec{}; for (int k = 0; k < 6; k++) u[k] = 0.0f; }
    MPT_SEG_BEGIN
    const int hslot = SCENE::ODD_IDS ? (L.hidx >> 4) : L.hidx;
    if (was_hit) {
        rec = shade_rec_load<SCENE::LDS_MATS>(p, hslot);
        lane_draws<6, SCENE::LDS_MATS>(p, L, u);
    }
    MPT_SEG(pl_trips)
    LightHit lit = lights_hit(p, ro, rd);
    if (lit.hit && (!was_hit || lit.dis < hdepth)) {
        float mis = power_heuristic(L.last_brdf_pdf, lit.pdf);
        L.result = L.result + L.throughput * (lit.color * mis);
    }
    hitpos = ro; sdir = v3s(0.0f); sdis = 0.0f;
    MPT_SEG(pl_local)
    if (!was_hit) {
        L.result = L.result + L.throughput * world_at(p, rd);
        L.depth = 5;
        return SH_END;
    }
    L.navoid = SCENE::ODD_IDS ? L.hidx : ~L.hidx;
    Hit hit; hit.hit = 1; hit.depth = hdepth; hit.index = hslot; hit.u = L.hu; hit.v = L.hv;
    V3 normal; Disney mat;
    get_geometries_rec(p, sc, rec, hit, ro, rd, &hitpos, &normal, mat);
    if (COUNT) { cnt.n_shade++; cnt.n_draws += 6; }
    float sign = -dot(rd, normal);
    if (sign < 0.0f) normal = -normal;
    MPT_SEG(pl_batches)

    LightSample li = lights_sample(p, hitpos, v3(u[0], u[1], u[2]));
    bool want_shadow = any_gt0(li.color);
    MPT_SEG(pl_batch_lanes)
    L.direct = v3s(0.0f);
    if (want_shadow) {
        V3 brdf_clr = disney_brdf(mat, normal, sign, -rd, li.dir);
        float brdf_pdf = vavg(brdf_clr);
        float mis = power_heuristic(li.pdf, brdf_pdf);
        V3 direct_li = li.color * mis * brdf_clr * dot_or_zero(normal, li.dir);
        L.direct = L.throughput * direct_li;
    }
    MPT_SEG(pl_prim)
    BsdfSample brdf = disney_bounce(mat, normal, sign, -rd, v3(u[3], u[4], u[5]));
    L.throughput = L.throughput * brdf.color;
    L.prd = brdf.outdir;
    L.last_brdf_pdf = brdf.pdf;
    MPT_SEG(pl_tidle)
    if (want_shadow && p.n >= 2 && (p.skip_dark == 0 || any_ne0(L.direct))) {
        sdir = li.dir; sdis = li.dis;
        return SH_SHADOW;
    }
    if (want_shadow && p.n < 2) { L.result = L.result + L.direct; if (COUNT) cnt.rays++; }
    return SH_BOUNCE;
}

struct PrimaryPool {
    V3 ro, rd;
    int rng_i, rng_k;
};
DEV void pool_prepare(const MptRenderParams &p, PrimaryPool &pp, bool inside, int i, int j, int frame) {
    pp.ro = v3s(0.0f); pp.rd = v3s(0.0f); pp.rng_i = 0; pp.rng_k = -1;
    if (inside) {
        LaneState T;
        T.frame = frame;
        T.rng_i = wanghash2(i, j);
        T.rng_k = reduce_mod_dim(T.rng_i, p.sobol_dim, p.sobol_inv_dim);
        float jit[2];
        lane_draws<2>(p, T, jit);
        float x = m_div((float)i + jit[0], (float)p.nx) * 2.0f - 1.0f;
        float y = m_div((float)j + jit[1], (float)p.ny) * 2.0f - 1.0f;
        camera_generate(p, x, y, &pp.ro, &pp.rd);
        pp.rng_i = T.rng_i; pp.rng_k = T.rng_k;
    }
}
DEV float lane_from(float v, int byte_lane) { return __int_as_float(__builtin_amdgcn_ds_bpermute(byte_lane, __float_as_int(v))); }
DEV int lane_from(int v, int byte_lane) { return __builtin_amdgcn_ds_bpermute(byte_lane, v); }

#ifndef MPT_PREF_NODE
#define MPT_PREF_NODE 1
#define MPT_PREF_LEAF 1
#endif
#ifndef MPT_LEAVE_A
#define MPT_LEAVE_A 2
#define MPT_LEAVE_B 1
#endif
#if MPT_X_STAMPS
#define MPT_STAMP_BEGIN unsigned long long stamp_t0 = 0; if (COUNT) { __builtin_amdgcn_sched_barrier(0); stamp_t0 = __builtin_amdgcn_s_memtime(); __builtin_amdgcn_sched_barrier(0); }
#define MPT_STAMP_END(acc) if (COUNT) { __builtin_amdgcn_sched_barrier(0); acc += __builtin_amdgcn_s_memtime() - stamp_t0; __builtin_amdgcn_sched_barrier(0); }
#else
#define MPT_STAMP_BEGIN
#define MPT_STAMP_END(acc)
#endif
DEV void lane_hist_add(const MptRenderParams &p, int stage, bool part, int depth, int shadow) {
    unsigned long long *h = p.counters + MPT_HIST_BASE;
    const bool l0 = (threadIdx.x & 63) == 0;
    const int n = (int)__builtin_popcountll(__ballot(part));
    if (l0) atomicAdd(h + stage * 65 + n, 1ull);
    for (int d = 0; d < 6; d++)
        for (int k = 0; k < 2; k++) {
            const int c = (int)__builtin_popcountll(__ballot(part && min(depth, 5) == d && (shadow != 0) == (k != 0)));
            if (l0 && c) atomicAdd(h + 3 * 65 + (stage * 6 + d) * 2 + k, (unsigned long long)c);
        }
}
DEV void node_id_hist_add(const MptRenderParams &p, bool part, int id) {
    unsigned long long *h = p.counters + MPT_HIST_BASE + 3 * 65 + 3 * 6 * 2;
    const int b = id <= 0 ? 0 : 32 - __builtin_clz((unsigned)id);
    for (int k = 0; k < 24; k++) {
        const int c = (int)__builtin_popcountll(__ballot(part && b == k));
        if ((threadIdx.x & 63) == 0 && c) atomicAdd(h + k, (unsigned long long)c);
    }
}
DEV int wave_count(bool pred) { return (int)__builtin_popcountll(__ballot(pred)); }
DEV int wave_count32(bool pred) {
    unsigned long long m = __ballot(pred);
    int n;
    asm("s_bcnt1_i32_b64 %0, %1" : "=s"(n) : "s"(m) : "scc");
    return n;
}

struct WorkQueue {
    unsigned int *ctr;
    int nitems, q0, qoff;
    DEV int pull() {
        const int lane = threadIdx.x & 63;
        while (qoff < 8) {
            int q = (q0 + qoff) & 7;
            int lo = (int)(((long long)nitems * q) >> 3), hi = (int)(((long long)nitems * (q + 1)) >> 3);
            int k = 0;
            if (lane == 0) k = (int)atomicAdd(ctr + q * MPT_QUEUE_STRIDE, 1u);
            k = __builtin_amdgcn_readfirstlane(k);
            if (lo + k < hi) return lo + k;
            qoff++;
        }
        return -1;
    }
};

template <bool COUNT, class SCENE, class STACK>
DEV void trace_stream(const MptRenderParams &p, const SCENE &sc, STACK stk, WorkQueue wq, Cnt &cnt,
                      unsigned long long *tl = nullptr) {
    const int tws = p.tile_w_shift, ths = p.tile_h_shift, tps = tws + ths;
    const int t8y = (p.ny + (1 << ths) - 1) >> ths;
    int S = 0, next = 0;
    int ti = 0, tj = 0, f0 = 0, tx_cur = 0;
    int ndead = 0;
    int deferred = 0;
    bool more = true;
    PrimaryPool pool;
    pool.ro = v3s(0.0f); pool.rd = v3s(0.0f); pool.rng_i = 0; pool.rng_k = -1;
    int pool_base = -64;
#if MPT_X_TIMELINE2
    int tl_items = 0, tl_passes = 0;
    unsigned long long tl_lastpull = 0;
#endif
#if MPT_X_STAMPS
    unsigned long long acc_node = 0, acc_leaf = 0, acc_sdone = 0, acc_shade = 0, acc_new = 0;
    const unsigned long long stamp_start = __builtin_amdgcn_s_memtime();
#endif
    LaneState L;
    L.st = ST_NEW;
    L.sp = 0; L.curr = 0; L.shadow = 0;
    L.result = v3s(0.0f); L.throughput = v3s(0.0f); L.prd = v3s(0.0f); L.direct = v3s(0.0f);
    L.to = v3s(0.0f); L.td = v3s(0.0f); L.inv = v3s(0.0f); L.oinv = v3s(0.0f);
    L.offx = 0; L.offy = 0; L.offz = 0;
    L.tbest = 0.0f; L.hidx = -1; L.hu = 0.0f; L.hv = 0.0f; L.last_brdf_pdf = 0.0f;
    L.navoid = 0; L.depth = 0; L.rng_i = 0; L.rng_k = 0; L.pix = 0; L.frame = 0;
    for (unsigned guard = 0;; guard++) {
        if (guard > (1u << 26)) {
            if ((threadIdx.x & 63) == 0) __hip_atomic_store(p.watchdog, 1u, __ATOMIC_RELAXED, __HIP_MEMORY_SCOPE_SYSTEM);
            break;
        }
        for (;;) {
            const int cn = wave_count32(L.st == ST_NODE);
            const int cl = wave_count32(L.st == ST_LEAF);
            const int trav = cn + cl;
            if (trav == 0) break;
            if (trav * MPT_LEAVE_A < (64 - ndead - trav - deferred) * MPT_LEAVE_B) break;
            MPT_STAMP_BEGIN
#if MPT_X_PAIRS
            const unsigned long long mn = __ballot(L.st == ST_NODE), ml = __ballot(L.st == ST_LEAF);
            if (COUNT && (threadIdx.x & 63) == 0) {
                if (cn * MPT_PREF_NODE >= cl * MPT_PREF_LEAF) { cnt.pl_local += (unsigned)__builtin_popcount((unsigned)mn | (unsigned)(mn >> 32)); cnt.pl_prim += (unsigned)__builtin_popcountll(mn); cnt.pl_trips++; }
                else { cnt.pl_batches += (unsigned)__builtin_popcount((unsigned)ml | (unsigned)(ml >> 32)); cnt.pl_tidle += (unsigned)__builtin_popcountll(ml); cnt.pl_taken++; }
            }
#endif
            if (cn * MPT_PREF_NODE >= cl * MPT_PREF_LEAF) {
                if (COUNT && (threadIdx.x & 63) == 0) cnt.it_node++;
                if (COUNT && p.lane_hist) lane_hist_add(p, 0, L.st == ST_NODE, L.depth, L.shadow);
                if constexpr (!STACK::ODD_IDS) { if (COUNT && p.lane_hist) node_id_hist_add(p, L.st == ST_NODE, L.curr); }
                if (L.st == ST_NODE) {
                    if constexpr (SCENE::WIDE) stage_node4<COUNT>(sc, stk, L, cnt);
                    else stage_node<COUNT>(sc, stk, L, cnt);
                }
#pragma unroll
                for (int rep = 0; rep < SCENE::NODE_REP; rep++) {
                    if (__ballot(L.st == ST_NODE) == 0ull) break;
                    if (COUNT && (threadIdx.x & 63) == 0) cnt.it_node++;
                    if (COUNT && p.lane_hist) lane_hist_add(p, 0, L.st == ST_NODE, L.depth, L.shadow);
                    if constexpr (!STACK::ODD_IDS) { if (COUNT && p.lane_hist) node_id_hist_add(p, L.st == ST_NODE, L.curr); }
                    if (L.st == ST_NODE) {
                        if constexpr (SCENE::WIDE) stage_node4<COUNT>(sc, stk, L, cnt);
                        else stage_node<COUNT>(sc, stk, L, cnt);
                    }
                }
                MPT_STAMP_END(acc_node)
            } else {
                if (COUNT && (threadIdx.x & 63) == 0) cnt.it_leaf++;
                if (COUNT && p.lane_hist) lane_hist_add(p, 1, L.st == ST_LEAF, L.depth, L.shadow);
                if (L.st == ST_LEAF) stage_leaf<COUNT>(sc, stk, L, cnt);
#pragma unroll
                for (int rep = 0; rep < SCENE::LEAF_REP; rep++) {
                    if (__ballot(L.st == ST_LEAF) == 0ull) break;
                    if (COUNT && (threadIdx.x & 63) == 0) cnt.it_leaf++;
                    if (COUNT && p.lane_hist) lane_hist_add(p, 1, L.st == ST_LEAF, L.depth, L.shadow);
                    if (L.st == ST_LEAF) stage_leaf<COUNT>(sc, stk, L, cnt);
                }
                MPT_STAMP_END(acc_leaf)
            }
        }
        bool shade_now = wave_count(L.st == ST_DONE && !L.shadow) != 0;
        if constexpr (SCENE::SHADE_MIN > 0) {
            const int ns = wave_count(L.st == ST_DONE && !L.shadow);
            const int ntrav = wave_count(L.st == ST_NODE || L.st == ST_LEAF);
            shade_now = ns != 0 && (ns >= SCENE::SHADE_MIN || ns * 2 >= 64 - ndead || ntrav == 0);
            deferred = shade_now ? 0 : ns;
        }
        if (shade_now) {
#if MPT_X_PAIRS
            const unsigned long long ms = __ballot(L.st == ST_DONE && !L.shadow);
            if (COUNT && (threadIdx.x & 63) == 0) {
                cnt.pl_batch_lanes += (unsigned)__builtin_popcount((unsigned)ms | (unsigned)(ms >> 32)); cnt.pl_sidle += (unsigned)__builtin_popcountll(ms);
            }
#endif
            if (COUNT && (threadIdx.x & 63) == 0) cnt.it_shade++;
            if (COUNT && p.lane_hist) lane_hist_add(p, 2, L.st == ST_DONE && !L.shadow, L.depth, 0);
            MPT_STAMP_BEGIN
            if (L.st == ST_DONE && !L.shadow) {
                V3 hitpos, sdir;
                float sdis;
                const int nk = shade_core<COUNT>(p, sc, L, cnt, hitpos, sdir, sdis);
                L.to = hitpos;
                if (nk == SH_SHADOW) { L.td = sdir; L.tbest = sdis; L.st = ST_SHADOW; }
                else L.st = ST_BOUNCE;
            }
            MPT_STAMP_END(acc_shade)
        }
        {
            MPT_STAMP_BEGIN
            if (L.st == ST_DONE && L.shadow) {
                if (L.hidx < 0) L.result = L.result + L.direct;
                L.st = ST_BOUNCE;
            }
            if (L.st == ST_BOUNCE && !path_continues(L)) lane_store_sample(p, L);
            MPT_STAMP_END(acc_sdone)
        }
        MPT_STAMP_BEGIN
        unsigned long long m_new = __ballot(L.st == ST_NEW);
        if (m_new != 0ull) {
            if (next >= S && more) {
#if MPT_X_STAMPS == 3
                const unsigned long long tp0 = __builtin_amdgcn_s_memtime();
#endif
                int item = wq.pull();
#if MPT_X_STAMPS == 3
                if (COUNT && (threadIdx.x & 63) == 0) cnt.pl_local += (unsigned)((__builtin_amdgcn_s_memtime() - tp0) >> 4);
#endif
                if (item < 0) {
                    more = false;
                    if (tl && (threadIdx.x & 63) == 0) {
                        tl[2] = wall_clock64();
#if MPT_X_TIMELINE2
                        tl[4] = tl_lastpull; tl[5] = (unsigned long long)tl_items;
                        tl[6] = (unsigned long long)(64 - (int)__builtin_popcountll(m_new));
#endif
                    }
                } else {
#if MPT_X_TIMELINE2
                    tl_items++; tl_lastpull = wall_clock64();
#endif
                    int tile = item / p.nchunks, chunk = item - tile * p.nchunks;
                    int tx = tile / t8y, ty = tile - tx * t8y;
                    int tps_x = p.stripe_w >> tws, st = tx / tps_x;
                    ti = p.x0 + st * p.stripe_pitch + ((tx - st * tps_x) << tws); tj = ty << ths; tx_cur = tx;
                    f0 = chunk * p.chunk;
                    S = (min(f0 + p.chunk, p.nframes) - f0) << tps;
                    next = 0; pool_base = -64;
                }
            }
            if (next < S) {
                if (COUNT && (threadIdx.x & 63) == 0) cnt.it_new++;
                const int lane = threadIdx.x & 63;
                if (next >= pool_base + 64) {
                    pool_base = next;
                    const int smp = pool_base + lane;
                    const int q = smp & ((1 << tps) - 1);
                    const int i = ti + (q >> ths), j = tj + (q & ((1 << ths) - 1));
#if MPT_X_STAMPS == 3
                    __builtin_amdgcn_sched_barrier(0);
                    const unsigned long long tq0 = __builtin_amdgcn_s_memtime();
#endif
                    pool_prepare(p, pool, smp < S && i < p.x1 && j < p.ny, i, j, f0 + (smp >> tps));
#if MPT_X_STAMPS == 3
                    {
                        float sink = pool.rd.x + pool.ro.x;
                        asm volatile("" :: "v"(sink));
                        __builtin_amdgcn_sched_barrier(0);
                        if (COUNT && (threadIdx.x & 63) == 0) cnt.pl_batches += (unsigned)((__builtin_amdgcn_s_memtime() - tq0) >> 4);
                    }
#endif
                }
                const int rank = __builtin_amdgcn_mbcnt_hi((unsigned)(m_new >> 32), __builtin_amdgcn_mbcnt_lo((unsigned)m_new, 0u));
                const int smp = next + rank;
                const int pool_end = min(S, pool_base + 64);
                const int src = ((smp - pool_base) & 63) << 2;
                V3 ro = v3(lane_from(pool.ro.x, src), lane_from(pool.ro.y, src), lane_from(pool.ro.z, src));
                V3 rd = v3(lane_from(pool.rd.x, src), lane_from(pool.rd.y, src), lane_from(pool.rd.z, src));
                const int rng_i = lane_from(pool.rng_i, src), rng_k = lane_from(pool.rng_k, src);
                if (L.st == ST_NEW && smp < pool_end && rng_k >= 0) {
                    const int q = smp & ((1 << tps) - 1);
                    L.frame = f0 + (smp >> tps);
                    L.pix = ((tx_cur << tws) + (q >> ths)) * p.ny + (tj + (q & ((1 << ths) - 1)));
                    L.rng_i = rng_i; L.rng_k = rng_k; L.prd = rd;
                    L.navoid = 0; L.depth = 0;
                    L.result = v3s(0.0f); L.throughput = v3s(1.0f); L.last_brdf_pdf = 0.0f;
                    if (COUNT) { cnt.samples++; cnt.n_draws += 2; }
                    L.to = ro;
                    L.st = ST_BOUNCE;
                    if (!path_continues(L)) lane_store_sample(p, L);
                }
                next = min(next + (int)__builtin_popcountll(m_new), pool_end);
            } else if (!more) {
                if (L.st == ST_NEW) L.st = ST_DEAD;
                ndead += (int)__builtin_popcountll(m_new);
            }
        }
        MPT_STAMP_END(acc_new)
        {
            MPT_STAMP_BEGIN
            if (L.st == ST_BOUNCE || L.st == ST_SHADOW) lane_begin_ray<COUNT>(p, L, stk, cnt);
            MPT_STAMP_END(acc_sdone)
        }
#if MPT_X_TIMELINE2
        if (!more) tl_passes++;
        if (ndead == 64 && tl && (threadIdx.x & 63) == 0) tl[7] = (unsigned long long)tl_passes;
#endif
        if (ndead == 64) break;
    }
#if MPT_X_STAMPS
    if (COUNT) {
        const bool l0 = (threadIdx.x & 63) == 0;
        const unsigned long long total = __builtin_amdgcn_s_memtime() - stamp_start;
        cnt.n_box = l0 ? (unsigned)(acc_node >> 8) : 0u; cnt.n_tri = l0 ? (unsigned)(acc_leaf >> 8) : 0u;
        cnt.n_draws = l0 ? (unsigned)(acc_sdone >> 8) : 0u; cnt.n_shade = l0 ? (unsigned)(acc_shade >> 8) : 0u;
        cnt.bounces = l0 ? (unsigned)(acc_new >> 8) : 0u; cnt.n_node = l0 ? (unsigned)(total >> 8) : 0u;
    }
#endif
}

DEV mpt_u4 slab_load_sc1(const MptVec4 *frame_base, unsigned frame_bytes, unsigned byte_off) {
    const __amdgpu_buffer_rsrc_t rsrc = __builtin_amdgcn_make_buffer_rsrc((void *)frame_base, (short)0, (int)frame_bytes, 0x00020000);
#ifndef MPT_FIN_AUX
#define MPT_FIN_AUX 16
#endif
    return __builtin_amdgcn_raw_buffer_load_b128(rsrc, (int)byte_off, 0, MPT_FIN_AUX);
}

#ifndef MPT_FIN_SLEEP
#define MPT_FIN_SLEEP 32
#endif
#ifndef MPT_FIN_GROUP_LDS
#define MPT_FIN_GROUP_LDS 8
#define MPT_FIN_GROUP_GATHER 6
#endif
struct FinArgs {
    MptVec4 *partial, *film0, *image_out;
    unsigned int *fin_counter, *watchdog;
    int tile_w_shift, tile_h_shift, ny, nitems, nchunks, nframes, partial_stride, stripe_w, stripe_pitch, x0, x1;
    unsigned slab_tag;
};
DEV int uniform_i(int v) { return __builtin_amdgcn_readfirstlane(v); }
template <class T> DEV T *uniform_p(T *ptr) {
    const unsigned long long v = (unsigned long long)ptr;
    const unsigned lo = (unsigned)__builtin_amdgcn_readfirstlane((int)(unsigned)v), hi = (unsigned)__builtin_amdgcn_readfirstlane((int)(unsigned)(v >> 32));
    return (T *)(((unsigned long long)hi << 32) | lo);
}
template <int GROUP>
__device__ __attribute__((noinline)) int finalise_tiles_impl(
        MptVec4 *a_partial, MptVec4 *a_film0, MptVec4 *a_image_out, unsigned int *a_fin_counter, unsigned int *a_watchdog,
        int a_tws, int a_ths, int a_ny, int a_nitems, int a_nchunks, int a_nframes, int a_partial_stride, int a_stripe_w,
        int a_stripe_pitch, int a_x0, int a_x1, unsigned a_slab_tag) {
    FinArgs p;
    p.partial = a_partial; p.film0 = a_film0; p.image_out = a_image_out; p.fin_counter = a_fin_counter; p.watchdog = a_watchdog;
    p.tile_w_shift = a_tws; p.tile_h_shift = a_ths; p.ny = a_ny; p.nitems = a_nitems; p.nchunks = a_nchunks; p.nframes = a_nframes;
    p.partial_stride = a_partial_stride; p.stripe_w = a_stripe_w; p.stripe_pitch = a_stripe_pitch; p.x0 = a_x0; p.x1 = a_x1;
    p.slab_tag = a_slab_tag;
    p.partial = uniform_p(p.partial); p.partial_stride = uniform_i(p.partial_stride); p.nframes = uniform_i(p.nframes);
    p.tile_w_shift = uniform_i(p.tile_w_shift); p.tile_h_shift = uniform_i(p.tile_h_shift);
    const int lane = threadIdx.x & 63;
    const int tws = p.tile_w_shift, ths = p.tile_h_shift, tps = tws + ths;
    const int t8y = (p.ny + (1 << ths) - 1) >> ths;
    const int ntile = p.nitems / p.nchunks;
    const int B = p.nframes;
    const unsigned frame_bytes = (unsigned)p.partial_stride * 16u;
    const unsigned tag = p.slab_tag;
    const mpt_u4 absent = slab_pack(0.0f, 0.0f, 0.0f, tag);
    const unsigned long long t_begin = wall_clock64();
    int done = 0;
    for (;; done++) {
        int t = 0;
        if (lane == 0) t = (int)atomicAdd(p.fin_counter, 1u);
        t = __builtin_amdgcn_readfirstlane(t);
        if (t >= ntile) break;
        const int tx = t / t8y, ty = t - tx * t8y;
        const int tps_x = p.stripe_w >> tws, st = tx / tps_x;
        const int ti = p.x0 + st * p.stripe_pitch + ((tx - st * tps_x) << tws), tj = ty << ths;
        for (int q0 = 0; q0 < (1 << tps); q0 += 64) {
            const int q = q0 + lane;
            const int i = ti + (q >> ths), j = tj + (q & ((1 << ths) - 1));
            const bool inside = q < (1 << tps) && i < p.x1 && j < p.ny;
            const unsigned off = (unsigned)(((tx << tws) + (q >> ths)) * p.ny + (tj + (q & ((1 << ths) - 1)))) * 16u;
            const size_t pix = (size_t)i * p.ny + j;
            MptVec4 acc = { 0.0f, 0.0f, 0.0f, 0.0f };
            if (inside) acc = p.film0[pix];
            for (int f0 = 0; f0 < B; f0 += GROUP) {
                mpt_u4 v[GROUP];
                for (;;) {
                    bool ready = true;
#pragma unroll
                    for (int k = 0; k < GROUP; k++) {
                        v[k] = absent;
                        if (f0 + k < B && inside) v[k] = slab_load_sc1(p.partial + (size_t)(f0 + k) * (size_t)p.partial_stride, frame_bytes, off);
                        ready = ready && slab_ready(v[k], tag);
                    }
                    if (__ballot(!ready) == 0ull) break;
                    if (wall_clock64() - t_begin > 400000000ull) {
                        if (lane == 0) __hip_atomic_store(p.watchdog, 1u, __ATOMIC_RELAXED, __HIP_MEMORY_SCOPE_SYSTEM);
                        return done;
                    }
                    __builtin_amdgcn_s_sleep(MPT_FIN_SLEEP);
                }
#pragma unroll
                for (int k = 0; k < GROUP; k++)
                    if (f0 + k < B) film_add_sample(acc, slab_r(v[k]), slab_g(v[k]), slab_b(v[k]));
            }
            if (inside) {
                p.film0[pix] = acc;
                if (p.image_out) p.image_out[pix] = film_resolve(acc);
            }
        }
    }
    return done;
}

template <int GROUP>
DEV int finalise_tiles(const MptRenderParams &p) {
#ifndef MPT_FIN_YOUNG
#define MPT_FIN_YOUNG 2
#endif
    if ((blockDim.x >> 8) >= 3 && (int)((threadIdx.x >> 8) & 3) < MPT_FIN_YOUNG) return 0;
    if (p.fin_counter)
        return finalise_tiles_impl<GROUP>(p.partial, p.film0, p.image_out, p.fin_counter, p.watchdog, p.tile_w_shift, p.tile_h_shift, p.ny,
                                          p.nitems, p.nchunks, p.nframes, p.partial_stride, p.stripe_w, p.stripe_pitch, p.x0, p.x1, p.slab_tag);
    return 0;
}
#endif

#if MPT_STRICT
#define MPT_RENDER_BOUNDS __launch_bounds__(MPT_BLOCK)
#else
#define MPT_RENDER_BOUNDS __launch_bounds__(MPT_BLOCK, 4)
#endif
template <int STACK, bool COUNT>
__global__ MPT_RENDER_BOUNDS void MPT_SUFFIX(render_kernel)(const MptRenderParams p) {
    __shared__ int s_stack[STACK * MPT_BLOCK];
    BlockTracer tr = make_block_tracer(p, s_stack + threadIdx.x);
    Cnt cnt = {};
#if MPT_STRICT
    int tile = xcd_remap(blockIdx.x, gridDim.x);
    int i, j;
    if (tile_pixel(p, tile, &i, &j)) trace_pixel<COUNT>(p, tr, i, j, 0, p.nframes, cnt);
#else
    WorkQueue wq; wq.ctr = p.work_counter; wq.nitems = p.nitems; wq.q0 = blockIdx.x & 7; wq.qoff = 0;
    trace_stream<COUNT>(p, tr.sc, tr.st, wq, cnt);
    finalise_tiles<MPT_FIN_GROUP_GATHER>(p);
#endif
    flush_counters<COUNT>(p, cnt);
}

#if !MPT_STRICT
#ifndef MPT_WIDE_WAVES
#define MPT_WIDE_WAVES 5
#endif
template <bool COUNT, bool QUANT>
__global__ __launch_bounds__(MPT_BLOCK, MPT_WIDE_WAVES) void render_kernel_wide(const MptRenderParams p) {
    __shared__ int s_stack[SpillStack::CAP * MPT_BLOCK];
    SpillStack stk;
    stk.base = s_stack + threadIdx.x;
    stk.spill = p.stack_spill;
    stk.lane_off = (blockIdx.x * MPT_BLOCK + threadIdx.x) * (unsigned)SpillStack::SPILL;
    stk.sp = 0;
    Cnt cnt = {};
    WorkQueue wq; wq.ctr = p.work_counter; wq.nitems = p.nitems; wq.q0 = blockIdx.x & 7; wq.qoff = 0;
    if constexpr (QUANT) {
        QuantScene sc; sc.qnode = p.qnode; sc.tgeo = p.tfast;
        trace_stream<COUNT>(p, sc, stk, wq, cnt);
    } else {
        WideScene sc; sc.wnode = p.wnode; sc.tgeo = p.tfast;
        trace_stream<COUNT>(p, sc, stk, wq, cnt);
    }
    finalise_tiles<MPT_FIN_GROUP_GATHER>(p);
    flush_counters<COUNT>(p, cnt);
}

template <bool COUNT>
__global__ __launch_bounds__(MPT_LDS_BLOCK) void render_kernel_lds(const MptRenderParams p) {
    extern __shared__ __attribute__((aligned(16))) MptVec4 smem[];
    const int nnode4 = ((p.n - 1) * MPT_LDS_NODE_STRIDE + 15) >> 4, ntri4 = p.n * 3, nmat4 = (p.default_mtl + 1) * MPT_LDS_MAT_VEC4;
    const int nmtl4 = (p.n + 15) >> 4;
    unsigned long long *tl = p.timeline ? p.timeline + MPT_TIMELINE_WORDS * (size_t)(blockIdx.x * (blockDim.x >> 6) + (threadIdx.x >> 6)) : nullptr;
    if (tl && (threadIdx.x & 63) == 0) tl[0] = wall_clock64();
    {
        for (int k = threadIdx.x; k < (p.n - 1) * 4; k += blockDim.x) {
            MptVec4 v = p.fnode[k];
            if ((k & 3) == 3) {
                const int i0 = __float_as_int(v.x), i1 = __float_as_int(v.y);
                v.x = __int_as_float(i0 >= 0 ? i0 * (MPT_LDS_NODE_STRIDE / 8) : i0);
                v.y = __int_as_float(i1 >= 0 ? i1 * (MPT_LDS_NODE_STRIDE / 8) : i1);
            }
            float *d = (float *)((char *)smem + (k >> 2) * MPT_LDS_NODE_STRIDE + (k & 3) * 16);
            *(float2 *)d = make_float2(v.x, v.y); *(float2 *)(d + 2) = make_float2(v.z, v.w);
        }
        for (int k = threadIdx.x; k < ntri4; k += blockDim.x) smem[nnode4 + k] = p.tfast[k];
        for (int k = threadIdx.x; k < nmat4; k += blockDim.x) {
            const int rec = k / MPT_LDS_MAT_VEC4, w = k - rec * MPT_LDS_MAT_VEC4;
            smem[nnode4 + ntri4 + k] = ((const MptVec4 *)(p.mats + rec))[w < 4 ? w : w + 4];
        }
        unsigned char *mtl = (unsigned char *)(smem + nnode4 + ntri4 + nmat4);
        for (int k = threadIdx.x; k < p.n; k += blockDim.x) {
            const int id = __float_as_int(p.tshade[(size_t)k * 4 + 3].w);
            mtl[k] = (unsigned char)(id == -1 ? p.default_mtl : id);
        }
    }
    __syncthreads();
    if (tl && (threadIdx.x & 63) == 0) tl[1] = wall_clock64();

    LdsScene sc;
    sc.fnode = (LdsVec4Ptr)(void *)smem;
    sc.tgeo = (LdsVec4Ptr)(void *)(smem + nnode4);
    sc.mats = (LdsVec4Ptr)(void *)(smem + nnode4 + ntri4);
    sc.mtl = (LdsU8Ptr)(void *)(smem + nnode4 + ntri4 + nmat4);
    sc.mat_last = p.default_mtl; sc.mat_default = p.default_mtl;
    Stack16 stk;
    stk.base = (LdsShortPtr)(void *)(smem + nnode4 + ntri4 + nmat4 + nmtl4) + threadIdx.x;
    stk.sp = 0;
    Cnt cnt = {};
    WorkQueue wq; wq.ctr = p.work_counter; wq.nitems = p.nitems; wq.q0 = blockIdx.x & 7; wq.qoff = 0;
    trace_stream<COUNT>(p, sc, stk, wq, cnt, tl);
    if (tl && (threadIdx.x & 63) == 0) tl[3] = wall_clock64();
    const int fin_tiles = finalise_tiles<MPT_FIN_GROUP_LDS>(p);
#if !MPT_X_TIMELINE2
    if (tl && (threadIdx.x & 63) == 0) { tl[4] = wall_clock64(); tl[5] = (unsigned long long)fin_tiles; }
#endif
    flush_counters<COUNT>(p, cnt);
}

template <bool COUNT>
__global__ __launch_bounds__(MPT_LDS_BLOCK) void render_kernel_lds4(const MptRenderParams p) {
    extern __shared__ __attribute__((aligned(16))) MptVec4 smem[];
    const int nnode4 = p.nwide * (MPT_LDS4_NODE_STRIDE / 16), ntri4 = (p.n + 1) * 3, nmat4 = (p.lds_nmats + 1) * MPT_LDS_MAT_VEC4;
    const int nmtl4 = (p.n + 15) >> 4;
    unsigned long long *tl = p.timeline ? p.timeline + MPT_TIMELINE_WORDS * (size_t)(blockIdx.x * (blockDim.x >> 6) + (threadIdx.x >> 6)) : nullptr;
    if (tl && (threadIdx.x & 63) == 0) tl[0] = wall_clock64();
    {
        for (int k = threadIdx.x; k < p.nwide * 7; k += blockDim.x) {
            const int rec = k / 7, w = k - rec * 7;
            MptVec4 v = p.wnode[rec * 8 + w];
            if (w == 6) {
                const int i0 = __float_as_int(v.x), i1 = __float_as_int(v.y), i2 = __float_as_int(v.z), i3 = __float_as_int(v.w);
                const int scale = LdsWideScene::ODD_IDS ? MPT_LDS4_NODE_STRIDE : MPT_LDS4_NODE_STRIDE / 8;
#define MPT_LDS_ID(i) __int_as_float((i) >= 0 ? (i) * scale : (LdsWideScene::ODD_IDS ? ((~(i)) << 4) | 1 : (i)))
                v.x = MPT_LDS_ID(i0); v.y = MPT_LDS_ID(i1); v.z = MPT_LDS_ID(i2); v.w = MPT_LDS_ID(i3);
#undef MPT_LDS_ID
            }
            smem[k] = v;
        }
        for (int k = threadIdx.x; k < ntri4; k += blockDim.x) smem[nnode4 + k] = p.tfast[k];
        for (int k = threadIdx.x; k < nmat4; k += blockDim.x) {
            const int rec = k / MPT_LDS_MAT_VEC4, w = k - rec * MPT_LDS_MAT_VEC4;
            const int grec = rec == p.lds_nmats ? p.default_mtl : rec;
            smem[nnode4 + ntri4 + k] = ((const MptVec4 *)(p.mats + grec))[w < 4 ? w : w + 4];
        }
        unsigned char *mtl = (unsigned char *)(smem + nnode4 + ntri4 + nmat4);
        for (int k = threadIdx.x; k < p.n; k += blockDim.x) {
            const int id = __float_as_int(p.tshade[(size_t)k * 4 + 3].w);
            mtl[k] = (unsigned char)(id == -1 ? p.lds_nmats : id);
        }
    }
    __syncthreads();
    if (tl && (threadIdx.x & 63) == 0) tl[1] = wall_clock64();

    LdsWideScene sc;
    sc.wnode = (LdsVec4Ptr)(void *)smem;
    if (LdsWideScene::ODD_IDS && (unsigned)(unsigned long long)(LdsBytePtr)sc.wnode != 0u) {
        if (threadIdx.x == 0) __hip_atomic_store(p.watchdog, 1u, __ATOMIC_RELAXED, __HIP_MEMORY_SCOPE_SYSTEM);
        return;
    }
    sc.tgeo = (LdsVec4Ptr)(void *)(smem + nnode4);
    sc.mats = (LdsVec4Ptr)(void *)(smem + nnode4 + ntri4);
    sc.mtl = (LdsU8Ptr)(void *)(smem + nnode4 + ntri4 + nmat4);
    sc.mat_last = p.lds_nmats; sc.mat_default = p.default_mtl;
    Stack16W stk;
    stk.base = (LdsShortPtr)(void *)(smem + nnode4 + ntri4 + nmat4 + nmtl4) + threadIdx.x;
    stk.sp = 0;
    stk.ts = p.t_scale;
    Cnt cnt = {};
    WorkQueue wq; wq.ctr = p.work_counter; wq.nitems = p.nitems; wq.q0 = blockIdx.x & 7; wq.qoff = 0;
    trace_stream<COUNT>(p, sc, stk, wq, cnt, tl);
    if (tl && (threadIdx.x & 63) == 0) tl[3] = wall_clock64();
    const int fin_tiles = finalise_tiles<MPT_FIN_GROUP_LDS>(p);
#if !MPT_X_TIMELINE2
    if (tl && (threadIdx.x & 63) == 0) { tl[4] = wall_clock64(); tl[5] = (unsigned long long)fin_tiles; }
#endif
    flush_counters<COUNT>(p, cnt);
}
#endif

template <int STACK>
__global__ __launch_bounds__(MPT_BLOCK) void MPT_SUFFIX(preview_kernel)(const MptRenderParams p) {
    __shared__ int s_stack[STACK * MPT_BLOCK];
    BlockTracer tr = make_block_tracer(p, s_stack + threadIdx.x);
    int tile = xcd_remap(blockIdx.x, gridDim.x);
    int i, j;
    if (!tile_pixel(p, tile, &i, &j)) return;
    const int pix = i * p.ny + j;
    const int h = wanghash2(i, j);
    Cnt cnt = {};
    MptVec4 a1 = p.film1[pix], a2 = p.film2[pix];
    for (int f = 0; f < p.nframes; f++) {
        Rng rng; rng.dim = p.sobol_dim; rng.P = p.P + (size_t)f * p.sobol_dim; rng.i = h;
        V3 albedo = v3s(0.0f), normal = v3s(0.0f);
        float dx = rng_random(rng), dy = rng_random(rng);
        float x = m_div((float)i + dx, (float)p.nx) * 2.0f - 1.0f;
        float y = m_div((float)j + dy, (float)p.ny) * 2.0f - 1.0f;
        V3 ro, rd;
        camera_generate(p, x, y, &ro, &rd);
        Hit hit = tr.template closest<false>(ro, rd, -1, cnt);
        if (hit.hit == 1) {
            V3 hitpos; Disney material;
            get_geometries(p, hit, ro, rd, &hitpos, &normal, material);
            albedo = material.basecolor;
        }
        a1.x += albedo.x; a1.y += albedo.y; a1.z += albedo.z; a1.w += 1.0f;
        a2.x += normal.x; a2.y += normal.y; a2.z += normal.z; a2.w += 1.0f;
    }
    p.film1[pix] = a1;
    p.film2[pix] = a2;
}

template <class K>
static int blocks_per_cu(K kernel) {
    int nb = 0;
    if (hipOccupancyMaxActiveBlocksPerMultiprocessor(&nb, kernel, MPT_BLOCK, 0) != hipSuccess || nb < 1) nb = 2;
    return nb;
}

MPT_KERNEL_API hipError_t MPT_SUFFIX(mpt_launch_render)(const MptRenderParams *p, int grid, int stack, int count,
                                                     hipStream_t stream) {
#if !MPT_STRICT
    static std::atomic<int> occ_cache[MPT_MAX_DEVICES][4];
    int v = (stack <= 32 ? 0 : 2) + (count ? 1 : 0);
    int dev = 0;
    if (hipGetDevice(&dev) != hipSuccess || dev < 0 || dev >= MPT_MAX_DEVICES) return hipErrorInvalidDevice;
    int occ = occ_cache[dev][v].load(std::memory_order_relaxed);
    if (!occ) {
        occ = v == 0 ? blocks_per_cu(MPT_SUFFIX(render_kernel)<32, false>)
            : v == 1 ? blocks_per_cu(MPT_SUFFIX(render_kernel)<32, true>)
            : v == 2 ? blocks_per_cu(MPT_SUFFIX(render_kernel)<64, false>)
                     : blocks_per_cu(MPT_SUFFIX(render_kernel)<64, true>);
        occ_cache[dev][v].store(occ, std::memory_order_relaxed);
    }
    grid *= occ;
#endif
    if (stack <= 32) {
        if (count) hipLaunchKernelGGL((MPT_SUFFIX(render_kernel)<32, true>), dim3(grid), dim3(MPT_BLOCK), 0, stream, *p);
        else hipLaunchKernelGGL((MPT_SUFFIX(render_kernel)<32, false>), dim3(grid), dim3(MPT_BLOCK), 0, stream, *p);
    } else {
        if (count) hipLaunchKernelGGL((MPT_SUFFIX(render_kernel)<64, true>), dim3(grid), dim3(MPT_BLOCK), 0, stream, *p);
        else hipLaunchKernelGGL((MPT_SUFFIX(render_kernel)<64, false>), dim3(grid), dim3(MPT_BLOCK), 0, stream, *p);
    }
    return hipGetLastError();
}

#if !MPT_STRICT
template <bool COUNT>
static hipError_t launch_lds(const MptRenderParams *p, int grid, int block, size_t lds_bytes, hipStream_t stream) {
    static std::atomic<bool> configured[MPT_MAX_DEVICES];
    int dev = 0;
    if (hipGetDevice(&dev) != hipSuccess || dev < 0 || dev >= MPT_MAX_DEVICES) return hipErrorInvalidDevice;
    if (!configured[dev].load(std::memory_order_acquire)) {
        hipError_t e = hipFuncSetAttribute((const void *)render_kernel_lds<COUNT>,
                                           hipFuncAttributeMaxDynamicSharedMemorySize, 160 * 1024);
        if (e != hipSuccess) return e;
        configured[dev].store(true, std::memory_order_release);
    }
    hipLaunchKernelGGL((render_kernel_lds<COUNT>), dim3(grid), dim3(block), lds_bytes, stream, *p);
    return hipGetLastError();
}

template <bool COUNT>
static hipError_t launch_lds4(const MptRenderParams *p, int grid, int block, size_t lds_bytes, hipStream_t stream) {
    static std::atomic<bool> configured[MPT_MAX_DEVICES];
    int dev = 0;
    if (hipGetDevice(&dev) != hipSuccess || dev < 0 || dev >= MPT_MAX_DEVICES) return hipErrorInvalidDevice;
    if (!configured[dev].load(std::memory_order_acquire)) {
        hipError_t e = hipFuncSetAttribute((const void *)render_kernel_lds4<COUNT>,
                                           hipFuncAttributeMaxDynamicSharedMemorySize, 160 * 1024);
        if (e != hipSuccess) return e;
        configured[dev].store(true, std::memory_order_release);
    }
    hipLaunchKernelGGL((render_kernel_lds4<COUNT>), dim3(grid), dim3(block), lds_bytes, stream, *p);
    return hipGetLastError();
}

MPT_KERNEL_API hipError_t mpt_launch_render_lds4(const MptRenderParams *p, int grid, int block, size_t lds_bytes, int count,
                                             hipStream_t stream) {
    return count ? launch_lds4<true>(p, grid, block, lds_bytes, stream) : launch_lds4<false>(p, grid, block, lds_bytes, stream);
}

MPT_KERNEL_API hipError_t mpt_launch_render_lds(const MptRenderParams *p, int grid, int block, size_t lds_bytes, int count,
                                            hipStream_t stream) {
    return count ? launch_lds<true>(p, grid, block, lds_bytes, stream) : launch_lds<false>(p, grid, block, lds_bytes, stream);
}
#endif

#if !MPT_STRICT
__global__ void derive_materials_kernel(MptMaterial *mats, int count) {
    int i = blockIdx.x * blockDim.x + threadIdx.x;
    if (i >= count) return;
    MptMaterial *mt = mats + i;
    Disney m;
    m.basecolor = v3(mt->p[0], mt->p[1], mt->p[2]);
    m.metallic = mt->p[3]; m.roughness = mt->p[4]; m.specular = mt->p[5]; m.specularTint = mt->p[6];
    m.subsurface = mt->p[7]; m.sheen = mt->p[8]; m.sheenTint = mt->p[9]; m.clearcoat = mt->p[10];
    m.clearcoatGloss = mt->p[11]; m.transmission = mt->p[12]; m.ior = mt->p[13];
    disney_init(m);
    mt->d[0] = m.speccolor.x; mt->d[1] = m.speccolor.y; mt->d[2] = m.speccolor.z;
    mt->d[3] = m.sheencolor.x; mt->d[4] = m.sheencolor.y; mt->d[5] = m.sheencolor.z;
    mt->d[6] = m.alpha; mt->d[7] = m.clearcoatAlpha;
    mt->p[14] = __int_as_float(mt->any_tex);
}

MPT_KERNEL_API hipError_t mpt_launch_derive_materials(MptMaterial *mats, int count, hipStream_t stream) {
    if (count <= 0) return hipSuccess;
    hipLaunchKernelGGL(derive_materials_kernel, dim3((count + 63) / 64), dim3(64), 0, stream, mats, count);
    return hipGetLastError();
}

MPT_KERNEL_API hipError_t mpt_wide_blocks(int grid, int count, int quant, int *blocks) {
    static std::atomic<int> occ_cache[MPT_MAX_DEVICES][4];
    int dev = 0;
    if (hipGetDevice(&dev) != hipSuccess || dev < 0 || dev >= MPT_MAX_DEVICES) return hipErrorInvalidDevice;
    const int v = (count ? 1 : 0) + (quant ? 2 : 0);
    int occ = occ_cache[dev][v].load(std::memory_order_relaxed);
    if (!occ) {
        occ = v == 0 ? blocks_per_cu(render_kernel_wide<false, false>) : v == 1 ? blocks_per_cu(render_kernel_wide<true, false>)
            : v == 2 ? blocks_per_cu(render_kernel_wide<false, true>) : blocks_per_cu(render_kernel_wide<true, true>);
        occ_cache[dev][v].store(occ, std::memory_order_relaxed);
    }
    *blocks = grid * occ;
    return hipSuccess;
}

MPT_KERNEL_API hipError_t mpt_launch_render_wide(const MptRenderParams *p, int blocks, int count, int quant, hipStream_t stream) {
    if (quant) {
        if (count) hipLaunchKernelGGL((render_kernel_wide<true, true>), dim3(blocks), dim3(MPT_BLOCK), 0, stream, *p);
        else hipLaunchKernelGGL((render_kernel_wide<false, true>), dim3(blocks), dim3(MPT_BLOCK), 0, stream, *p);
    } else {
        if (count) hipLaunchKernelGGL((render_kernel_wide<true, false>), dim3(blocks), dim3(MPT_BLOCK), 0, stream, *p);
        else hipLaunchKernelGGL((render_kernel_wide<false, false>), dim3(blocks), dim3(MPT_BLOCK), 0, stream, *p);
    }
    return hipGetLastError();
}
#endif

MPT_KERNEL_API hipError_t MPT_SUFFIX(mpt_launch_preview)(const MptRenderParams *p, int grid, int stack,
                                                      hipStream_t stream) {
    if (stack <= 32) hipLaunchKernelGGL((MPT_SUFFIX(preview_kernel)<32>), dim3(grid), dim3(MPT_BLOCK), 0, stream, *p);
    else hipLaunchKernelGGL((MPT_SUFFIX(preview_kernel)<64>), dim3(grid), dim3(MPT_BLOCK), 0, stream, *p);
    return hipGetLastError();
}
```

### ptina_amd/csrc/unit_eval.hip

```cpp

#include "pt_device.h"
#include "tri_records.h"
#include "../../include/miptina.h"

#if MPT_STRICT
#define MPT_SUFFIX(x) x##_strict
#else
#define MPT_SUFFIX(x) x##_fast
#endif

DEV V3 ld(const float *r, int k) { return v3(r[k], r[k + 1], r[k + 2]); }
DEV void st(float *o, int k, V3 v) { o[k] = v.x; o[k + 1] = v.y; o[k + 2] = v.z; }

DEV Disney disney_from14(const float *p) {
    Disney m;
    m.basecolor = v3(p[0], p[1], p[2]);
    m.metallic = p[3]; m.roughness = p[4]; m.specular = p[5]; m.specularTint = p[6];
    m.subsurface = p[7]; m.sheen = p[8]; m.sheenTint = p[9]; m.clearcoat = p[10];
    m.clearcoatGloss = p[11]; m.transmission = p[12]; m.ior = p[13];
    disney_init(m);
    return m;
}

#if !MPT_STRICT
struct UnitScene { static constexpr bool LDS_MATS = false; };
#endif

__global__ __launch_bounds__(64) void MPT_SUFFIX(unit_eval_kernel)(const MptRenderParams p, int kind, const float *__restrict__ in,
                                                                   int in_cols, float *__restrict__ out, int out_cols, int n) {
    const int row = blockIdx.x * 64 + threadIdx.x;
    if (row >= n) return;
    const float *r = in + (size_t)row * in_cols;
    float *o = out + (size_t)row * out_cols;
    switch (kind) {
    case MPT_UNIT_SCHLICK: o[0] = schlickFresnel(r[0]); break;
    case MPT_UNIT_DIELECTRIC: o[0] = dielectricFresnel(r[0], r[1], r[2]); break;
    case MPT_UNIT_GTR1: o[0] = GTR1(r[0], r[1]); break;
    case MPT_UNIT_GTR2: o[0] = GTR2(r[0], r[1]); break;
    case MPT_UNIT_SMITHGGX: o[0] = smithGGX(r[0], r[1]); break;
    case MPT_UNIT_SAMPLE_GTR1: st(o, 0, sample_GTR1(r[0], r[1], r[2])); break;
    case MPT_UNIT_SAMPLE_GTR2: st(o, 0, sample_GTR2(r[0], r[1], r[2])); break;
    case MPT_UNIT_TANSPACE: st(o, 0, tanspace_mul(tanspace(ld(r, 0)), ld(r, 3))); break;
    case MPT_UNIT_SPHERICAL: st(o, 0, spherical(r[0], r[1])); break;
    case MPT_UNIT_DIR2TEX: dir2tex(ld(r, 0), &o[0], &o[1]); break;
    case MPT_UNIT_REFLECT: st(o, 0, reflectv(ld(r, 0), ld(r, 3))); break;
    case MPT_UNIT_REFRACT: {
        V3 T;
        o[0] = refractv(ld(r, 0), ld(r, 3), r[6], &T) ? 1.0f : 0.0f;
        st(o, 1, T);
        break;
    }
    case MPT_UNIT_BOX: {
#if MPT_STRICT
        float nearv, farv;
        o[0] = box_strict(ld(r, 0), ld(r, 3), ld(r, 6), ld(r, 9), &nearv, &farv) ? 1.0f : 0.0f;
        o[1] = nearv; o[2] = farv;
#else
        const V3 ro = ld(r, 6), rd = ld(r, 9);
        const V3 inv = v3(m_rcp(rd.x), m_rcp(rd.y), m_rcp(rd.z)), oinv = ro * inv;
        float tn;
        o[0] = box_fast(r[0], r[1], r[2], r[3], r[4], r[5], inv, oinv, MPT_INF, &tn) ? 1.0f : 0.0f;
        o[1] = tn; o[2] = -1.0f;
#endif
        break;
    }
    case MPT_UNIT_FACE: {
        MptVec4 g[4];
        tri_make_tgeo(r, r + 3, r + 6, g);
        float d = 2.0f * MPT_INF, s = 0.0f, t = 0.0f;
#if MPT_STRICT
        const bool hit = tri_test(g[0], g[1], g[2], g[3], ld(r, 9), ld(r, 12), &d, &s, &t);
#else
        MptVec4 f[3];
        tri_make_tfast(g, f);
        const bool hit = tri_test_fast(f[0], f[1], f[2], ld(r, 9), ld(r, 12), &d, &s, &t);
#endif
        o[0] = hit ? 1.0f : 0.0f; o[1] = d; o[2] = s; o[3] = t;
        const float *vn = r + 15, *vt = r + 24;
        const MptVec4 s0 = { vn[0], vn[1], vn[2], vn[3] }, s1 = { vn[4], vn[5], vn[6], vn[7] },
                      s2 = { vn[8], vt[0], vt[1], vt[2] }, s3 = { vt[3], vt[4], vt[5], 0.0f };
        V3 nrm; float tu, tv;
        face_shading(s0, s1, s2, s3, s, t, &nrm, &tu, &tv);
        st(o, 4, nrm); o[7] = tu; o[8] = tv;
        break;
    }
    case MPT_UNIT_SPHERE: o[0] = sphere_intersect(ld(r, 0), r[3], ld(r, 4), ld(r, 7)); break;
    case MPT_UNIT_AREA: {
        float d = MPT_INF, u = 0.0f, v = 0.0f;
        o[0] = area_intersect(ld(r, 0), ld(r, 3), ld(r, 6), ld(r, 9), ld(r, 12), &d, &u, &v) ? 1.0f : 0.0f;
        o[1] = d; o[2] = u; o[3] = v;
        break;
    }
    case MPT_UNIT_DISNEY_BRDF: {
        const Disney m = disney_from14(r);
        st(o, 0, disney_brdf(m, ld(r, 14), r[17], ld(r, 18), ld(r, 21)));
        break;
    }
    case MPT_UNIT_DISNEY_BOUNCE: {
        const Disney m = disney_from14(r);
        const BsdfSample b = disney_bounce(m, ld(r, 14), r[17], ld(r, 18), ld(r, 21));
        st(o, 0, b.outdir); o[3] = b.pdf; st(o, 4, b.color);
        break;
    }
    case MPT_UNIT_POWER_HEURISTIC: o[0] = power_heuristic(r[0], r[1]); break;
    case MPT_UNIT_WANGHASH: o[0] = __int_as_float(wanghash(__float_as_int(r[0]))); break;
    case MPT_UNIT_WANGHASH2: o[0] = __int_as_float(wanghash2(__float_as_int(r[0]), __float_as_int(r[1]))); break;
    case MPT_UNIT_LIGHT_HIT: {
        const LightHit h = lights_hit(p, ld(r, 0), ld(r, 3));
        o[0] = h.hit ? 1.0f : 0.0f; o[1] = h.dis; o[2] = h.pdf; st(o, 3, h.color);
        break;
    }
    case MPT_UNIT_LIGHT_SAMPLE: {
        const LightSample s = lights_sample(p, ld(r, 0), ld(r, 3));
        o[0] = s.dis; st(o, 1, s.dir); o[4] = s.pdf; st(o, 5, s.color);
        break;
    }
    case MPT_UNIT_IMAGE_SAMPLE: {
        const MptVec4 t = image_sample(p, (int)r[0], r[1], r[2]);
        o[0] = t.x; o[1] = t.y; o[2] = t.z; o[3] = t.w;
        break;
    }
    case MPT_UNIT_WORLD_AT: st(o, 0, world_at(p, ld(r, 0))); break;
    case MPT_UNIT_MATERIAL_GET: {
        Disney m;
        material_get(p, (int)r[0], r[1], r[2], m);
        st(o, 0, m.basecolor);
        o[3] = m.metallic; o[4] = m.roughness; o[5] = m.specular; o[6] = m.specularTint; o[7] = m.subsurface; o[8] = m.sheen;
        o[9] = m.sheenTint; o[10] = m.clearcoat; o[11] = m.clearcoatGloss; o[12] = m.transmission; o[13] = m.ior;
        st(o, 14, m.speccolor); st(o, 17, m.sheencolor); o[20] = m.alpha; o[21] = m.clearcoatAlpha;
        break;
    }
    case MPT_UNIT_CAMERA_GENERATE: {
        V3 ro, rd;
        camera_generate(p, r[0], r[1], &ro, &rd);
        st(o, 0, ro); st(o, 3, rd);
        break;
    }
    case MPT_UNIT_FACE_SIDE: {
        Hit hit;
        hit.index = row; hit.depth = 1.0f; hit.u = r[12]; hit.v = r[13];
        V3 hitpos, normal;
        Disney m;
#if MPT_STRICT
        get_geometries(p, hit, v3s(0.0f), ld(r, 0), &hitpos, &normal, m);
#else
        const UnitScene sc;
        get_geometries_rec(p, sc, shade_rec_load<false>(p, row), hit, v3s(0.0f), ld(r, 0), &hitpos, &normal, m);
#endif
        const MptVec4 *s = p.tshade + (size_t)row * 4;
        V3 plain; float tu, tv;
        face_shading(s[0], s[1], s[2], s[3], hit.u, hit.v, &plain, &tu, &tv);
        st(o, 0, normal); o[3] = dot(plain, normal) < 0.0f ? 1.0f : 0.0f;
        break;
    }
    default: break;
    }
}

MPT_KERNEL_API hipError_t MPT_SUFFIX(mpt_launch_unit_eval)(const MptRenderParams *p, int kind, const float *in, int in_cols, float *out,
                                                         int out_cols, int n, hipStream_t stream) {
    if (n <= 0) return hipSuccess;
    hipLaunchKernelGGL(MPT_SUFFIX(unit_eval_kernel), dim3((n + 63) / 64), dim3(64), 0, stream, *p, kind, in, in_cols, out,
                       out_cols, n);
    return hipGetLastError();
}
```

Before: 3567 Msamples/s.

## Specialise the LDS4 render kernel for plain scenes via shading feature mask

Adds a host-side feature mask built from the scene's materials, lights and world texture. When the scene uses no textured materials, a single light and no world texture, a template instantiation of the LDS4 kernel is launched with those branches compiled out. This removes runtime branches and texture-loop code from the shading path, which may lower register pressure. The cost is an extra kernel instantiation and a host scan of the material features on each render.

```diff
diff --git a/ptina_amd/csrc/miptina.cpp b/ptina_amd/csrc/miptina.cpp
--- a/ptina_amd/csrc/miptina.cpp
+++ b/ptina_amd/csrc/miptina.cpp
@@ -145,6 +145,12 @@
         for (auto &m : z) { memset(&m, 0, sizeof m); for (int k = 0; k < 12; k++) m.tex[k] = -1; }
         const float dflt[14] = { 0.8f, 0.8f, 0.8f, 0.0f, 0.4f, 0.5f, 0.4f, 0.0f, 0.0f, 0.4f, 0.0f, 0.5f, 0.0f, 1.45f };
         memcpy(z.back().p, dflt, sizeof dflt);
+        {
+            float fac[48] = {};
+            fac[0] = dflt[0]; fac[1] = dflt[1]; fac[2] = dflt[2];
+            for (int k = 1; k < 12; k++) fac[k * 4] = dflt[2 + k];
+            c->default_feat = shade_feat_material(fac, nullptr);
+        }
         hipMemcpyAsync(c->mats, z.data(), z.size() * sizeof(MptMaterial), hipMemcpyHostToDevice, c->stream);
         mpt_launch_derive_materials(c->mats, (int)z.size(), c->stream);
         hipStreamSynchronize(c->stream);
@@ -250,6 +256,8 @@
     return 0;
 }
 
+static int scene_feat_now(const mpt_ctx *c);
+
 extern "C" int mpt_set_option(mpt_ctx *c, const char *key, int value) {
     if (use(c)) return 1;
     std::string k = key ? key : "";
@@ -271,6 +279,9 @@
         c->lds_wide = value;
     } else if (k == "zero_copy") {
         c->zero_copy = value ? 1 : 0;
+    } else if (k == "shade_spec") {
+        if (value != 0 && value != 1) return fail("shade_spec must be 0 (always the generic SHADE) or 1 (the plain one for plain scenes)");
+        c->shade_spec = value;
     } else if (k == "skip_dark") {
         if (value < -1 || value > 1) return fail("skip_dark must be -1 (auto), 0 or 1");
         c->skip_dark = value;
@@ -356,6 +367,9 @@
     else if (k == "launch_seq") *value = (int)(c->launch_seq & 0x7fffffffu);
     else if (k == "tag_wraps") *value = (int)c->tag_wraps;
     else if (k == "skip_dark") *value = c->skip_dark;
+    else if (k == "shade_spec") *value = c->shade_spec;
+    else if (k == "scene_feat") *value = scene_feat_now(c);
+    else if (k == "shade_inst") *value = c->last_shade_feat;
     else if (k == "pipe_depth") *value = c->pipe_depth;
     else if (k == "grid_div") *value = c->grid_div;
     else if (k == "cur_depth") *value = c->cur_depth;
@@ -493,10 +507,15 @@
     return 0;
 }
 
+static int scene_feat_now(const mpt_ctx *c) {
+    return shade_feat_scene(c->mat_feat.data(), (int)c->mat_feat.size(), c->max_mtlid, c->default_feat, (int)c->h_lights.size(), c->world_tex);
+}
+
 extern "C" int mpt_load_materials(mpt_ctx *c, const float *fac, const int32_t *tex, int m) {
     if (use(c)) return 1;
     if (m < 0 || m > c->caps.max_materials) return fail("%d materials exceed max_materials=%d", m, c->caps.max_materials);
     std::vector<MptMaterial> h(std::max(m, 1));
+    std::vector<unsigned char> feat((size_t)m);
     int max_tex = -1;
     for (int i = 0; i < m; i++) {
         MptMaterial &M = h[i];
@@ -512,8 +531,11 @@
             if (t != -1) M.any_tex = 1;
             max_tex = std::max(max_tex, t);
         }
+        feat[i] = (unsigned char)shade_feat_material(f, M.tex);
     }
     c->max_mat_tex = max_tex;
+    if (c->mat_feat.size() < feat.size()) c->mat_feat.resize(feat.size(), 0);
+    std::copy(feat.begin(), feat.end(), c->mat_feat.begin());
     c->nmats = m;
     if (m) HIP_TRY(hipMemcpyAsync(c->mats, h.data(), (size_t)m * sizeof(MptMaterial), hipMemcpyHostToDevice, c->stream));
     HIP_TRY(mpt_launch_derive_materials(c->mats, m, c->stream));
@@ -893,13 +915,15 @@
         }
     }
     c->last_finalised = fin ? 1 : 0;
+    const int shade_feat = lds4_kernel ? shade_feat_instantiation(scene_feat_now(c), c->shade_spec) : MPT_FEAT_GENERIC;
     hipEvent_t e0 = get_event(c), e1 = get_event(c);
     HIP_TRY(hipEventRecord(e0, rs));
     if (!fast) HIP_TRY(mpt_launch_render_strict(&p, p.ntiles, stack, c->count, rs));
-    else if (lds4_kernel) HIP_TRY(mpt_launch_render_lds4(&p, launch_cus, lds_block_used, lds4_bytes, c->count, rs));
+    else if (lds4_kernel) HIP_TRY(mpt_launch_render_lds4(&p, launch_cus, lds_block_used, lds4_bytes, c->count, shade_feat, rs));
     else if (lds_kernel) HIP_TRY(mpt_launch_render_lds(&p, launch_cus, lds_block_used, lds_bytes, c->count, rs));
     else if (wide_kernel) HIP_TRY(mpt_launch_render_wide(&p, wide_blocks, c->count, c->use_quant, rs));
     else HIP_TRY(mpt_launch_render_fast(&p, launch_cus, stack, c->count, rs));
+    c->last_shade_feat = shade_feat;
     c->last_kernel = lds4_kernel ? 5 : lds_kernel ? 1 : wide_kernel ? 2 : 0;
     HIP_TRY(hipEventRecord(e1, rs));
     c->events.push_back({ e0, e1 });
diff --git a/ptina_amd/csrc/miptina_ctx.h b/ptina_amd/csrc/miptina_ctx.h
--- a/ptina_amd/csrc/miptina_ctx.h
+++ b/ptina_amd/csrc/miptina_ctx.h
@@ -2,6 +2,7 @@
 
 #include "../../include/miptina.h"
 #include "mpt_types.h"
+#include "shade_feat.h"
 #include <hip/hip_runtime_api.h>
 #include <rccl/rccl.h>
 #include <dlfcn.h>
@@ -23,7 +24,7 @@
 MPT_KERNEL_API hipError_t mpt_wide_blocks(int grid, int count, int quant, int *blocks);
 MPT_KERNEL_API hipError_t mpt_launch_render_wide(const MptRenderParams *, int blocks, int count, int quant, hipStream_t);
 MPT_KERNEL_API hipError_t mpt_launch_render_lds(const MptRenderParams *, int grid, int block, size_t lds_bytes, int count, hipStream_t);
-MPT_KERNEL_API hipError_t mpt_launch_render_lds4(const MptRenderParams *, int grid, int block, size_t lds_bytes, int count, hipStream_t);
+MPT_KERNEL_API hipError_t mpt_launch_render_lds4(const MptRenderParams *, int grid, int block, size_t lds_bytes, int count, int feat, hipStream_t);
 MPT_KERNEL_API hipError_t mpt_launch_mlt_chain_fast(const MptRenderParams *, const MptMltArgs *, int stack, hipStream_t);
 MPT_KERNEL_API hipError_t mpt_launch_mlt_chain_strict(const MptRenderParams *, const MptMltArgs *, int stack, hipStream_t);
 MPT_KERNEL_API hipError_t mpt_launch_mlt_trace_fast(const MptRenderParams *, const float *X, float *rgb, int n, int stack, hipStream_t);
@@ -99,6 +100,8 @@
     int tile_w_shift = 3, tile_h_shift = 3;
     int last_div = 1;
     int last_kernel = 0;
+    int shade_spec = 1;
+    int last_shade_feat = -1;
 
     int nx = 0, ny = 0, x0 = 0, x1 = 0;
     int stripe_w = 0, stripe_idx = 0, stripe_mod = 1;
@@ -155,6 +158,8 @@
     size_t node_cap = 0, tri_cap = 0;
 
     MptMaterial *mats = nullptr;
+    std::vector<unsigned char> mat_feat;
+    int default_feat = 0;
     int nmats = 0;
     int max_mat_tex = -1;
     MptImage *images = nullptr;
diff --git a/ptina_amd/csrc/pt_device.h b/ptina_amd/csrc/pt_device.h
--- a/ptina_amd/csrc/pt_device.h
+++ b/ptina_amd/csrc/pt_device.h
@@ -2,6 +2,7 @@
 
 #include <hip/hip_runtime.h>
 #include "mpt_types.h"
+#include "shade_feat.h"
 
 #ifndef MPT_STRICT
 #define MPT_STRICT 0
@@ -690,10 +691,12 @@
 }
 
 #if !MPT_STRICT
+template <int FEAT = MPT_FEAT_GENERIC>
 DEV void material_from(const MptRenderParams &p, const MptMaterial *mt, MptVec4 q0, MptVec4 q1, MptVec4 q2, MptVec4 q3,
                        MptVec4 d0, MptVec4 d1, float tu, float tv, Disney &m) {
     float v[14] = { q0.x, q0.y, q0.z, q0.w, q1.x, q1.y, q1.z, q1.w, q2.x, q2.y, q2.z, q2.w, q3.x, q3.y };
-    const bool textured = __float_as_int(q3.z) != 0;
+    bool textured = false;
+    if constexpr ((FEAT & MPT_FEAT_TEXTURED_MATS) != 0) textured = __float_as_int(q3.z) != 0;
     if (textured) {
 #pragma unroll 1
         for (int k = 0; k < 12; k++) {
@@ -766,7 +769,9 @@
 }
 #endif
 
+template <int FEAT = MPT_FEAT_GENERIC>
 DEV V3 disney_brdf(const Disney &m, V3 normal, float sign, V3 indir, V3 outdir) {
+    constexpr bool COAT = (FEAT & MPT_FEAT_CLEARCOAT) != 0, TRANS = (FEAT & MPT_FEAT_TRANSMISSION) != 0;
     float etai = 1.0f, etao = m.ior;
     if (sign < 0.0f) { etai = m.ior; etao = 1.0f; }
 
@@ -778,7 +783,7 @@
 
     V3 result = v3s(0.0f);
     if (coso < 0.0f) {
-        if (cosi >= 0.0f) {
+        if (TRANS && cosi >= 0.0f) {
             float Ds = GTR2(cosh_, m.alpha);
             float fdf = dielectricFresnel(etao, etai, cosoh);
             V3 transmit = m.basecolor * MPT_INV_PI * (1.0f - fdf) * Ds;
@@ -810,7 +815,7 @@
         V3 transmit = m.basecolor * (MPT_INV_PI * fdf * Ds);
 #else
         float coat = 0.0f;
-        if (m.clearcoat != 0.0f) {
+        if (COAT && m.clearcoat != 0.0f) {
             float Dr = GTR1(cosh_, m.clearcoatAlpha);
             float Gr = smithGGX(cosi, 0.25f) * smithGGX(coso, 0.25f);
             float Fr = lerpf(Foh, 0.04f, 1.0f);
@@ -818,7 +823,7 @@
         }
         V3 specular = Fs * Gs * Ds + v3s(coat);
         V3 transmit = v3s(0.0f);
-        if (m.transmission != 0.0f) transmit = m.basecolor * (MPT_INV_PI * dielectricFresnel(etao, etai, cosoh) * Ds);
+        if (TRANS && m.transmission != 0.0f) transmit = m.basecolor * (MPT_INV_PI * dielectricFresnel(etao, etai, cosoh) * Ds);
 #endif
 
         result = diffuse * (1.0f - m.metallic) * (1.0f - m.transmission);
@@ -847,7 +852,9 @@
     }
 };
 
+template <int FEAT = MPT_FEAT_GENERIC>
 DEV BsdfSample disney_bounce(const Disney &m, V3 normal, float sign, V3 indir, V3 samp) {
+    constexpr bool COAT = (FEAT & MPT_FEAT_CLEARCOAT) != 0, TRANS = (FEAT & MPT_FEAT_TRANSMISSION) != 0;
     BsdfSample result;
     result.outdir = v3s(0.0f); result.pdf = 0.0f; result.color = v3s(0.0f);
 
@@ -953,7 +960,7 @@
         result.color = vdivs(diffuse * MPT_PI * (1.0f - m.metallic) * (1.0f - m.transmission), choice.pdf);
     }
 #else
-    const bool coat = coatrate != 0.0f && choice(coatrate);
+    const bool coat = COAT && coatrate != 0.0f && choice(coatrate);
     const bool spec = !coat && choice(specrate);
     float hz;
     if (coat) {
@@ -985,7 +992,7 @@
         const float coso = fmaxf(0.0f, coso_raw);
         if (cosoh > 0.0f && coso > 0.0f && cosh_ > 0.0f) {
             float Ds = GTR2(cosh_, m.alpha);
-            if (choice(m.transmission)) {
+            if (TRANS && choice(m.transmission)) {
                 float fdf = dielectricFresnel(etao, etai, cosoh);
                 float reflrate = lerpf(fdf, 0.2f, 1.0f);
                 if (choice(reflrate)) {
@@ -1052,9 +1059,11 @@
 
 struct LightHit { bool hit; float dis, pdf; V3 color; };
 
+template <int FEAT = MPT_FEAT_GENERIC>
 DEV LightHit lights_hit(const MptRenderParams &p, V3 ro, V3 rd) {
     LightHit ret; ret.hit = false; ret.dis = MPT_INF; ret.pdf = 0.0f; ret.color = v3s(0.0f);
-    for (int i = 0; i < p.nlights; i++) {
+    const int nlights = (FEAT & MPT_FEAT_MANY_LIGHTS) != 0 ? p.nlights : 1;
+    for (int i = 0; i < nlights; i++) {
         MptLight L = MPT_LIGHTS(p)[i];
         int type = __float_as_int(L.pos_type.w);
         V3 pos = ld3(L.pos_type);
@@ -1123,15 +1132,16 @@
     return ret;
 }
 
+template <int FEAT = MPT_FEAT_GENERIC>
 DEV LightSample lights_sample(const MptRenderParams &p, V3 hitpos, V3 samp) {
     LightSample ret; ret.dis = MPT_INF; ret.dir = v3s(0.0f); ret.pdf = 0.0f; ret.color = v3s(0.0f);
 #if !MPT_STRICT
-    if (p.nlights == 1) {
+    if ((FEAT & MPT_FEAT_MANY_LIGHTS) == 0 || p.nlights == 1) {
         const MptLight L = MPT_LIGHTS(p)[0];
         return light_sample_one(L, hitpos, samp);
     }
 #endif
-    if (p.nlights != 0) {
+    if ((FEAT & MPT_FEAT_MANY_LIGHTS) != 0 && p.nlights != 0) {
         int i = (int)floorf(samp.z * (float)p.nlights);
         i = min(max(i, 0), min(p.nlights, MPT_MAX_LIGHTS - 1));
         const MptLight L = MPT_LIGHTS(p)[i];
@@ -1146,9 +1156,10 @@
     *t = atan2f(dn.y, sqrtf(dn.x * dn.x + dn.z * dn.z)) / MPT_PI + 0.5f;
 }
 
+template <int FEAT = MPT_FEAT_GENERIC>
 DEV V3 world_at(const MptRenderParams &p, V3 dir) {
     V3 fac = v3(p.world_fac[0], p.world_fac[1], p.world_fac[2]);
-    if (p.world_tex != -1) {
+    if ((FEAT & MPT_FEAT_WORLD_TEXTURE) != 0 && p.world_tex != -1) {
         V3 d2 = v3(dir.x, dir.z, -dir.y);
         float s, t;
         dir2tex(d2, &s, &t);
@@ -1202,7 +1213,7 @@
     ShadeRec r; r.s0 = s[0]; r.s1 = s[1]; r.s2 = s[2]; r.s3 = s[3];
     return r;
 }
-template <class SCENE>
+template <int FEAT, class SCENE>
 DEV void get_geometries_rec(const MptRenderParams &p, const SCENE &sc, const ShadeRec &r, const Hit &hit, V3 ro, V3 rd,
                             V3 *hitpos, V3 *normal, Disney &mat) {
     const MptVec4 s0 = r.s0, s1 = r.s1, s2 = r.s2, s3 = r.s3;
@@ -1216,8 +1227,9 @@
         const int rec = sc.mtl[hit.index];
         LdsVec4Ptr q = sc.mats + rec * MPT_LDS_MAT_VEC4;
         MptVec4 q0 = lds_ld(q), q1 = lds_ld(q + 1), q2 = lds_ld(q + 2), q3 = lds_ld(q + 3), d0 = lds_ld(q + 4), d1 = lds_ld(q + 5);
-        material_from(p, p.mats + (rec == sc.mat_last ? sc.mat_default : rec), q0, q1, q2, q3, d0, d1, tu, tv, mat);
+        material_from<FEAT>(p, p.mats + (rec == sc.mat_last ? sc.mat_default : rec), q0, q1, q2, q3, d0, d1, tu, tv, mat);
     } else {
+        static_assert(FEAT == MPT_FEAT_GENERIC, "the gather kernels are built for the generic mask only");
         material_get(p, __float_as_int(s3.w), tu, tv, mat);
     }
 }
diff --git a/ptina_amd/csrc/render_kernel.hip b/ptina_amd/csrc/render_kernel.hip
--- a/ptina_amd/csrc/render_kernel.hip
+++ b/ptina_amd/csrc/render_kernel.hip
@@ -378,7 +378,7 @@
 #define MPT_SEG_BEGIN
 #define MPT_SEG(field)
 #endif
-template <bool COUNT, class SCENE>
+template <bool COUNT, int FEAT, class SCENE>
 DEV int shade_core(const MptRenderParams &p, const SCENE &sc, LaneState &L, Cnt &cnt, V3 &hitpos, V3 &sdir, float &sdis) {
     V3 ro = L.to, rd = L.prd;
     const bool was_hit = L.hidx >= 0;
@@ -393,7 +393,7 @@
         lane_draws<6, SCENE::LDS_MATS>(p, L, u);
     }
     MPT_SEG(pl_trips)
-    LightHit lit = lights_hit(p, ro, rd);
+    LightHit lit = lights_hit<FEAT>(p, ro, rd);
     if (lit.hit && (!was_hit || lit.dis < hdepth)) {
         float mis = power_heuristic(L.last_brdf_pdf, lit.pdf);
         L.result = L.result + L.throughput * (lit.color * mis);
@@ -401,32 +401,32 @@
     hitpos = ro; sdir = v3s(0.0f); sdis = 0.0f;
     MPT_SEG(pl_local)
     if (!was_hit) {
-        L.result = L.result + L.throughput * world_at(p, rd);
+        L.result = L.result + L.throughput * world_at<FEAT>(p, rd);
         L.depth = 5;
         return SH_END;
     }
     L.navoid = SCENE::ODD_IDS ? L.hidx : ~L.hidx;
     Hit hit; hit.hit = 1; hit.depth = hdepth; hit.index = hslot; hit.u = L.hu; hit.v = L.hv;
     V3 normal; Disney mat;
-    get_geometries_rec(p, sc, rec, hit, ro, rd, &hitpos, &normal, mat);
+    get_geometries_rec<FEAT>(p, sc, rec, hit, ro, rd, &hitpos, &normal, mat);
     if (COUNT) { cnt.n_shade++; cnt.n_draws += 6; }
     float sign = -dot(rd, normal);
     if (sign < 0.0f) normal = -normal;
     MPT_SEG(pl_batches)
 
-    LightSample li = lights_sample(p, hitpos, v3(u[0], u[1], u[2]));
+    LightSample li = lights_sample<FEAT>(p, hitpos, v3(u[0], u[1], u[2]));
     bool want_shadow = any_gt0(li.color);
     MPT_SEG(pl_batch_lanes)
     L.direct = v3s(0.0f);
     if (want_shadow) {
-        V3 brdf_clr = disney_brdf(mat, normal, sign, -rd, li.dir);
+        V3 brdf_clr = disney_brdf<FEAT>(mat, normal, sign, -rd, li.dir);
         float brdf_pdf = vavg(brdf_clr);
         float mis = power_heuristic(li.pdf, brdf_pdf);
         V3 direct_li = li.color * mis * brdf_clr * dot_or_zero(normal, li.dir);
         L.direct = L.throughput * direct_li;
     }
     MPT_SEG(pl_prim)
-    BsdfSample brdf = disney_bounce(mat, normal, sign, -rd, v3(u[3], u[4], u[5]));
+    BsdfSample brdf = disney_bounce<FEAT>(mat, normal, sign, -rd, v3(u[3], u[4], u[5]));
     L.throughput = L.throughput * brdf.color;
     L.prd = brdf.outdir;
     L.last_brdf_pdf = brdf.pdf;
@@ -521,7 +521,7 @@
     }
 };
 
-template <bool COUNT, class SCENE, class STACK>
+template <bool COUNT, int FEAT, class SCENE, class STACK>
 DEV void trace_stream(const MptRenderParams &p, const SCENE &sc, STACK stk, WorkQueue wq, Cnt &cnt,
                       unsigned long long *tl = nullptr) {
     const int tws = p.tile_w_shift, ths = p.tile_h_shift, tps = tws + ths;
@@ -623,7 +623,7 @@
             if (L.st == ST_DONE && !L.shadow) {
                 V3 hitpos, sdir;
                 float sdis;
-                const int nk = shade_core<COUNT>(p, sc, L, cnt, hitpos, sdir, sdis);
+                const int nk = shade_core<COUNT, FEAT>(p, sc, L, cnt, hitpos, sdir, sdis);
                 L.to = hitpos;
                 if (nk == SH_SHADOW) { L.td = sdir; L.tbest = sdis; L.st = ST_SHADOW; }
                 else L.st = ST_BOUNCE;
@@ -866,7 +866,7 @@
     if (tile_pixel(p, tile, &i, &j)) trace_pixel<COUNT>(p, tr, i, j, 0, p.nframes, cnt);
 #else
     WorkQueue wq; wq.ctr = p.work_counter; wq.nitems = p.nitems; wq.q0 = blockIdx.x & 7; wq.qoff = 0;
-    trace_stream<COUNT>(p, tr.sc, tr.st, wq, cnt);
+    trace_stream<COUNT, MPT_FEAT_GENERIC>(p, tr.sc, tr.st, wq, cnt);
     finalise_tiles<MPT_FIN_GROUP_GATHER>(p);
 #endif
     flush_counters<COUNT>(p, cnt);
@@ -888,10 +888,10 @@
     WorkQueue wq; wq.ctr = p.work_counter; wq.nitems = p.nitems; wq.q0 = blockIdx.x & 7; wq.qoff = 0;
     if constexpr (QUANT) {
         QuantScene sc; sc.qnode = p.qnode; sc.tgeo = p.tfast;
-        trace_stream<COUNT>(p, sc, stk, wq, cnt);
+        trace_stream<COUNT, MPT_FEAT_GENERIC>(p, sc, stk, wq, cnt);
     } else {
         WideScene sc; sc.wnode = p.wnode; sc.tgeo = p.tfast;
-        trace_stream<COUNT>(p, sc, stk, wq, cnt);
+        trace_stream<COUNT, MPT_FEAT_GENERIC>(p, sc, stk, wq, cnt);
     }
     finalise_tiles<MPT_FIN_GROUP_GATHER>(p);
     flush_counters<COUNT>(p, cnt);
@@ -940,7 +940,7 @@
     stk.sp = 0;
     Cnt cnt = {};
     WorkQueue wq; wq.ctr = p.work_counter; wq.nitems = p.nitems; wq.q0 = blockIdx.x & 7; wq.qoff = 0;
-    trace_stream<COUNT>(p, sc, stk, wq, cnt, tl);
+    trace_stream<COUNT, MPT_FEAT_GENERIC>(p, sc, stk, wq, cnt, tl);
     if (tl && (threadIdx.x & 63) == 0) tl[3] = wall_clock64();
     const int fin_tiles = finalise_tiles<MPT_FIN_GROUP_LDS>(p);
 #if !MPT_X_TIMELINE2
@@ -949,7 +949,7 @@
     flush_counters<COUNT>(p, cnt);
 }
 
-template <bool COUNT>
+template <bool COUNT, int FEAT>
 __global__ __launch_bounds__(MPT_LDS_BLOCK) void render_kernel_lds4(const MptRenderParams p) {
     extern __shared__ __attribute__((aligned(16))) MptVec4 smem[];
     const int nnode4 = p.nwide * (MPT_LDS4_NODE_STRIDE / 16), ntri4 = (p.n + 1) * 3, nmat4 = (p.lds_nmats + 1) * MPT_LDS_MAT_VEC4;
@@ -1000,7 +1000,7 @@
     stk.ts = p.t_scale;
     Cnt cnt = {};
     WorkQueue wq; wq.ctr = p.work_counter; wq.nitems = p.nitems; wq.q0 = blockIdx.x & 7; wq.qoff = 0;
-    trace_stream<COUNT>(p, sc, stk, wq, cnt, tl);
+    trace_stream<COUNT, FEAT>(p, sc, stk, wq, cnt, tl);
     if (tl && (threadIdx.x & 63) == 0) tl[3] = wall_clock64();
     const int fin_tiles = finalise_tiles<MPT_FIN_GROUP_LDS>(p);
 #if !MPT_X_TIMELINE2
@@ -1092,24 +1092,29 @@
     return hipGetLastError();
 }
 
-template <bool COUNT>
+template <bool COUNT, int FEAT>
 static hipError_t launch_lds4(const MptRenderParams *p, int grid, int block, size_t lds_bytes, hipStream_t stream) {
     static std::atomic<bool> configured[MPT_MAX_DEVICES];
     int dev = 0;
     if (hipGetDevice(&dev) != hipSuccess || dev < 0 || dev >= MPT_MAX_DEVICES) return hipErrorInvalidDevice;
     if (!configured[dev].load(std::memory_order_acquire)) {
-        hipError_t e = hipFuncSetAttribute((const void *)render_kernel_lds4<COUNT>,
+        hipError_t e = hipFuncSetAttribute((const void *)render_kernel_lds4<COUNT, FEAT>,
                                            hipFuncAttributeMaxDynamicSharedMemorySize, 160 * 1024);
         if (e != hipSuccess) return e;
         configured[dev].store(true, std::memory_order_release);
     }
-    hipLaunchKernelGGL((render_kernel_lds4<COUNT>), dim3(grid), dim3(block), lds_bytes, stream, *p);
+    hipLaunchKernelGGL((render_kernel_lds4<COUNT, FEAT>), dim3(grid), dim3(block), lds_bytes, stream, *p);
     return hipGetLastError();
 }
 
-MPT_KERNEL_API hipError_t mpt_launch_render_lds4(const MptRenderParams *p, int grid, int block, size_t lds_bytes, int count,
+MPT_KERNEL_API hipError_t mpt_launch_render_lds4(const MptRenderParams *p, int grid, int block, size_t lds_bytes, int count, int feat,
                                              hipStream_t stream) {
-    return count ? launch_lds4<true>(p, grid, block, lds_bytes, stream) : launch_lds4<false>(p, grid, block, lds_bytes, stream);
+    if (feat == MPT_FEAT_PLAIN)
+        return count ? launch_lds4<true, MPT_FEAT_PLAIN_KERNEL>(p, grid, block, lds_bytes, stream)
+                     : launch_lds4<false, MPT_FEAT_PLAIN_KERNEL>(p, grid, block, lds_bytes, stream);
+    if (feat != MPT_FEAT_GENERIC) return hipErrorInvalidValue;
+    return count ? launch_lds4<true, MPT_FEAT_GENERIC>(p, grid, block, lds_bytes, stream)
+                 : launch_lds4<false, MPT_FEAT_GENERIC>(p, grid, block, lds_bytes, stream);
 }
 
 MPT_KERNEL_API hipError_t mpt_launch_render_lds(const MptRenderParams *p, int grid, int block, size_t lds_bytes, int count,
diff --git a/ptina_amd/csrc/shade_feat.h b/ptina_amd/csrc/shade_feat.h
--- /dev/null
+++ b/ptina_amd/csrc/shade_feat.h
@@ -0,0 +1,37 @@
+#pragma once
+
+#include <stdint.h>
+
+enum {
+    MPT_FEAT_TEXTURED_MATS = 1,
+    MPT_FEAT_CLEARCOAT = 2,
+    MPT_FEAT_TRANSMISSION = 4,
+    MPT_FEAT_WORLD_TEXTURE = 8,
+    MPT_FEAT_MANY_LIGHTS = 16,
+    MPT_FEAT_PLAIN = 0,
+    MPT_FEAT_GENERIC = 31,
+    MPT_FEAT_PLAIN_KERNEL = MPT_FEAT_CLEARCOAT | MPT_FEAT_TRANSMISSION
+};
+
+static inline int shade_feat_material(const float *fac, const int32_t *tex) {
+    int bits = 0;
+    if (tex)
+        for (int k = 0; k < 12; k++)
+            if (tex[k] != -1) bits |= MPT_FEAT_TEXTURED_MATS;
+    if (fac[8 * 4] != 0.0f || (tex && tex[8] != -1)) bits |= MPT_FEAT_CLEARCOAT;
+    if (fac[10 * 4] != 0.0f || (tex && tex[10] != -1)) bits |= MPT_FEAT_TRANSMISSION;
+    return bits;
+}
+
+static inline int shade_feat_scene(const unsigned char *mat_bits, int nmats, int max_mtlid, int default_bits,
+                                   int nlights, int world_tex) {
+    int bits = default_bits;
+    for (int i = 0; i < nmats && i <= max_mtlid; i++) bits |= mat_bits[i];
+    if (world_tex != -1) bits |= MPT_FEAT_WORLD_TEXTURE;
+    if (nlights != 1) bits |= MPT_FEAT_MANY_LIGHTS;
+    return bits;
+}
+
+static inline int shade_feat_instantiation(int scene_bits, int shade_spec) {
+    return (shade_spec && scene_bits == MPT_FEAT_PLAIN) ? MPT_FEAT_PLAIN : MPT_FEAT_GENERIC;
+}
diff --git a/ptina_amd/csrc/unit_eval.hip b/ptina_amd/csrc/unit_eval.hip
--- a/ptina_amd/csrc/unit_eval.hip
+++ b/ptina_amd/csrc/unit_eval.hip
@@ -145,7 +145,7 @@
         get_geometries(p, hit, v3s(0.0f), ld(r, 0), &hitpos, &normal, m);
 #else
         const UnitScene sc;
-        get_geometries_rec(p, sc, shade_rec_load<false>(p, row), hit, v3s(0.0f), ld(r, 0), &hitpos, &normal, m);
+        get_geometries_rec<MPT_FEAT_GENERIC>(p, sc, shade_rec_load<false>(p, row), hit, v3s(0.0f), ld(r, 0), &hitpos, &normal, m);
 #endif
         const MptVec4 *s = p.tshade + (size_t)row * 4;
         V3 plain; float tu, tv;
```

Measured after the change: 3636 Msamples/s (median of 6 runs). 1.9% higher.
